# pghysels/STRUMPACK

Measured on AMD Instinct MI355X. Metric: hss_compress_ulv_factor_solve_gflops, higher is better.
Workload: dtype f64

## Files before the change

include/hssk.h:

```cpp
#ifndef HSSK_H
#define HSSK_H

#ifdef __cplusplus
extern "C" {
#endif

typedef struct hssk_ctx hssk_ctx;

int hssk_ctx_create(hssk_ctx** ctx, int device);
void hssk_ctx_destroy(hssk_ctx* ctx);
void* hssk_ctx_stream(hssk_ctx* ctx);
int hssk_sync(hssk_ctx* ctx);
const char* hssk_last_error(void);
typedef struct hssk_plan hssk_plan;
int hssk_plan_begin(hssk_ctx* ctx, hssk_plan** plan);
int hssk_plan_end(hssk_ctx* ctx);
int hssk_plan_replay(hssk_ctx* ctx, hssk_plan* plan);
void hssk_plan_destroy(hssk_plan* plan);
int hssk_plan_size(const hssk_plan* plan);

void* hssk_malloc(long long bytes);
void hssk_free(void* dptr);
long long hssk_device_total_bytes(void);
int hssk_memcpy_h2d(hssk_ctx* ctx, void* dst, const void* src, long long bytes);
int hssk_memcpy_d2h(hssk_ctx* ctx, void* dst, const void* src, long long bytes);
int hssk_upload_async(hssk_ctx* ctx, void* dst, const void* src, long long bytes);
int hssk_memcpy_d2d(hssk_ctx* ctx, void* dst, const void* src, long long bytes);
int hssk_memcpy2d_h2d(hssk_ctx* ctx, void* dst, long long dpitch, const void* src, long long spitch,
                      long long width, long long height);
int hssk_memcpy2d_d2h(hssk_ctx* ctx, void* dst, long long dpitch, const void* src, long long spitch,
                      long long width, long long height);
int hssk_memset_zero(hssk_ctx* ctx, void* dst, long long bytes);
int hssk_h2d_block_async(hssk_ctx* ctx, double* dst, long long ldd, const double* src, long long lds, long long rows,
                         long long cols);
int hssk_h2d_bytes_async(hssk_ctx* ctx, void* dst, long long dpitch, const void* src, long long spitch, long long width,
                         long long cols);
int hssk_copy_fence(hssk_ctx* ctx);
int hssk_compute_fence(hssk_ctx* ctx);
int hssk_compute_mark(hssk_ctx* ctx, int slot);
int hssk_copy_wait(hssk_ctx* ctx, int slot);
int hssk_is_device_pointer(const void* ptr);
typedef struct hssk_aca_desc {
  const double* A;
  int lda, m, n;
  double rtol, atol;
  int max_rank, row0;
  double* U;
  int ldu;
  double* V;
  int ldv;
  int* rank;
} hssk_aca_desc;
int hssk_aca_vbatched(hssk_ctx* ctx, const hssk_aca_desc* descs, int count);
int hssk_side_begin(hssk_ctx* ctx);
int hssk_side_end(hssk_ctx* ctx);
int hssk_side_join(hssk_ctx* ctx);
int hssk_stream_wait(hssk_ctx* waiter, hssk_ctx* on);
int hssk_watch_start(hssk_ctx* ctx, int id);
int hssk_watch_stop(hssk_ctx* ctx, int id);
double hssk_watch_read_ms(hssk_ctx* ctx, int id, int* pairs);
float hssk_last_dgemm_ms(hssk_ctx* ctx);
double hssk_last_dgemm_flops(hssk_ctx* ctx);
int hssk_dgemm_timing_defer(hssk_ctx* ctx);
int hssk_dgemm_timing_collect(hssk_ctx* ctx, double* ms, double* flops, int* launches);
long long hssk_last_dgemm_trace(hssk_ctx* ctx, long long* out, long long max_wgs);
double hssk_last_dgemm_clock_ghz(hssk_ctx* ctx);

int hssk_fill_toeplitz(hssk_ctx* ctx, double* A, int n, long long lda, char kind);
int hssk_fill_toeplitz_block(hssk_ctx* ctx, double* A, int rows, int cols, long long lda, int i0, int j0, char kind);
int hssk_randn(hssk_ctx* ctx, double* P, int rows, long long cols, long long ld, int row0,
               long long stride, unsigned long long seed);

int hssk_dgemm(hssk_ctx* ctx, int transB, int m, long long n, long long k, double alpha,
               const double* A, long long lda, const double* B, long long ldb, double beta,
               double* C, long long ldc);

int hssk_sgemm_sketch(hssk_ctx* ctx, int transB, int m, long long n, long long k, double alpha,
                      const double* A, long long lda,
                      const float* B, long long ldb,
                      double beta, double* C, long long ldc);
int hssk_narrow_f32(hssk_ctx* ctx, float* dst, long long ldd, const double* src, long long lds, long long rows, long long cols);

#define HSSK_GEN_TOEPLITZ 1
#define HSSK_GEN_TOEPLITZ_UPPER 2
typedef struct hssk_gen {
  int kind, reserved;
  double p[4];
} hssk_gen;
int hssk_sketch_gen(hssk_ctx* ctx, const hssk_gen* g, int transG, int m, long long n, long long k, long long j0, double alpha,
                    const double* A, long long lda, double beta, double* C, long long ldc);
int hssk_gen_fill(hssk_ctx* ctx, const hssk_gen* g, double* A, long long rows, long long cols, long long lda, long long i0,
                  long long j0, int trans);

typedef struct hssk_gemm_desc {
  const double* A;
  const double* B;
  double* C;
  int m, n, k;
  int lda, ldb, ldc;
  int transA, transB;
  double alpha, beta;
} hssk_gemm_desc;
int hssk_gemm_vbatched(hssk_ctx* ctx, const hssk_gemm_desc* descs, int count);

typedef struct hssk_leaf_update_desc {
  const double* R;
  const double* D;
  double* Sr;
  double* Sc;
  int d, m, ldr, ldd, lds;
} hssk_leaf_update_desc;
int hssk_leaf_update_vbatched(hssk_ctx* ctx, const hssk_leaf_update_desc* descs, int count);

typedef struct hssk_kernel_spec {
  const double* X;
  long long n;
  int d, type, p;
  double h, lambda;
} hssk_kernel_spec;
typedef struct hssk_keval_desc {
  const int* ri;
  const int* ci;
  double* out;
  int nr, nc, ldo, r0, c0;
} hssk_keval_desc;
int hssk_kernel_eval_vbatched(hssk_ctx* ctx, const hssk_kernel_spec* spec, const hssk_keval_desc* descs, int count);
int hssk_knn(hssk_ctx* ctx, const double* X, int d, int n, int k, int q0, int q1, int* out_idx);
typedef struct hssk_colset_desc {
  const int* src0;
  const int* src1;
  int n0, n1, lo, hi;
  int* out;
  int* count;
  const int* n0_dev;
  const int* n1_dev;
} hssk_colset_desc;
int hssk_colsets(hssk_ctx* ctx, const hssk_colset_desc* descs, int count, int universe);
long long hssk_colsets_max_universe(void);
int hssk_cluster_median(hssk_ctx* ctx, double* X, int d, int n, int algo, int cluster_size, int* perm, int* status);
int hssk_kernel_predict(hssk_ctx* ctx, const hssk_kernel_spec* spec, const double* w, const double* T, int m, double* pred);
#define HSSK_KPREDICT_TAU 1.220703125e-4
int hssk_kernel_predict_f32(hssk_ctx* ctx, const float* X, long long n, int d, int type, int p, double h,
                            const float* w, const float* T, int m, float* pred, long long* stats);
int hssk_kernel_predict_splits(long long n, int m);

typedef struct hssk_colgather_desc {
  const double* src;
  double* dst;
  const int* idx;
  int rows, ncols, lds, ldd;
  int scatter;
} hssk_colgather_desc;
int hssk_gather_cols(hssk_ctx* ctx, const hssk_colgather_desc* descs, int count);
enum { HSSK_DT_F64 = 0, HSSK_DT_F32 = 1, HSSK_DT_C32 = 2, HSSK_DT_C64 = 3 };
int hssk_expand_image(hssk_ctx* ctx, double* dst, long long ldd, const void* src, long long lds, long long rows, long long cols,
                      int dtype);
typedef struct hssk_rowgather_desc {
  const double* src;
  double* dst;
  const int* idx;
  int nrows, cols, lds, ldd;
  int scatter, accumulate;
} hssk_rowgather_desc;
int hssk_gather_rows(hssk_ctx* ctx, const hssk_rowgather_desc* descs, int count);
typedef struct hssk_elem_desc {
  const double* A;
  long long lda;
  const int* I;
  const int* J;
  int i0, j0;
  double* B;
  int m, n, ldb, transpose;
  int rlo, rhi, clo, chi;
} hssk_elem_desc;
int hssk_gather_elems(hssk_ctx* ctx, const hssk_elem_desc* descs, int count);
int hssk_gather_elems_f32(hssk_ctx* ctx, const hssk_elem_desc* descs, int count);
int hssk_gen_elems(hssk_ctx* ctx, const hssk_gen* g, const hssk_elem_desc* descs, int count);
int hssk_sum_slabs(hssk_ctx* ctx, const double* slabs, long long count, long long stride, int nslab, double* out);
typedef struct hssk_transpose_desc {
  const double* src;
  double* dst;
  int rows, cols, lds, ldd;
} hssk_transpose_desc;
int hssk_transpose(hssk_ctx* ctx, const hssk_transpose_desc* descs, int count);

typedef struct hssk_triu_desc {
  const double* src;
  double* dst;
  int rows, cols, lds, ldd;
  int dstride;
} hssk_triu_desc;
int hssk_copy_triu(hssk_ctx* ctx, const hssk_triu_desc* descs, int count);

int hssk_sjlt_dense(hssk_ctx* ctx, double* Rt, int dn, long long K, long long ld, const int* pat, int nnz);
int hssk_sjlt_sketch(hssk_ctx* ctx, int transA, long long n_out, long long K, const double* A, long long lda,
// ... 298 lines not shown
```

include/structured/StructuredMatrix.h:

```cpp
#ifndef STRUCTURED_MATRIX_H
#define STRUCTURED_MATRIX_H

typedef enum {
  SP_TYPE_HSS = 0,
  SP_TYPE_BLR,
  SP_TYPE_HODLR,
  SP_TYPE_HODBF,
  SP_TYPE_BUTTERFLY,
  SP_TYPE_LR,
  SP_TYPE_LOSSY,
  SP_TYPE_LOSSLESS
} SP_STRUCTURED_TYPE;

typedef struct CSPOptions {
  SP_STRUCTURED_TYPE type;
  double rel_tol;
  double abs_tol;
  int leaf_size;
  int max_rank;
  int verbose;
} CSPOptions;

typedef void* CSPStructMat;

// ... 47 lines not shown
void SPX_d_struct_default_hss_options(SPXHSSOptions* h);
int SPX_d_struct_from_dense_hss(CSPStructMat* S, int rows, int cols, const double* A, int ldA,
                                const CSPOptions* opts, const SPXHSSOptions* h);
int SPX_d_struct_from_dense_device(CSPStructMat* S, int rows, int cols, const double* dA, long long ldA,
                                   const CSPOptions* opts, const SPXHSSOptions* h);
int SPX_s_struct_from_dense_device(CSPStructMat* S, int rows, int cols, const float* dA, long long ldA,
                                   const CSPOptions* opts, const SPXHSSOptions* h, int sketch_precision);
int SPX_s_struct_sketch_route(const CSPStructMat S);
int SPX_s_struct_stats(const CSPStructMat S, double* out);
typedef void (*SPXAllGatherFn)(void* user, void* dbuf, long long bytes_per_rank);
int SPX_d_struct_from_dense_device_sharded(CSPStructMat* S, int rows, int cols, const double* dA, long long ldA,
                                           const CSPOptions* opts, const SPXHSSOptions* h, int world, int rank,
                                           SPXAllGatherFn allgather, void* user);
typedef void* SPXComm;
int SPX_comm_unique_id(char id[128]);
int SPX_comm_create(SPXComm* comm, int world, int rank, const char id[128]);
void SPX_comm_destroy(SPXComm* comm);
int SPX_comm_selftest(SPXComm comm);
int SPX_comm_size(const SPXComm comm);
int SPX_comm_rank(const SPXComm comm);
int SPX_struct_shard_range(int n, const CSPOptions* opts, int world, int rank, int* lo, int* hi);
int SPX_d_struct_from_dense_device_comm(CSPStructMat* S, int rows, int cols, const double* dA, long long ldA,
                                        const CSPOptions* opts, const SPXHSSOptions* h, SPXComm comm);
int SPX_d_struct_from_generator(CSPStructMat* S, int n, int kind, const CSPOptions* opts, const SPXHSSOptions* h);
int SPX_d_struct_from_generator_comm(CSPStructMat* S, int n, int kind, const CSPOptions* opts, const SPXHSSOptions* h, SPXComm comm);
int SPX_d_struct_from_generator_sharded(CSPStructMat* S, int n, int kind, const CSPOptions* opts, const SPXHSSOptions* h,
                                        int world, int rank, SPXAllGatherFn allgather, void* user);
int SPX_d_struct_from_blocks_device(CSPStructMat* S, int rows, int cols, const double* dArows, long long ldr,
                                    const double* dAcols, long long ldc, const CSPOptions* opts, const SPXHSSOptions* h,
                                    SPXComm comm);
int SPX_d_struct_from_blocks_device_cb(CSPStructMat* S, int rows, int cols, const double* dArows, long long ldr,
                                       const double* dAcols, long long ldc, const CSPOptions* opts, const SPXHSSOptions* h,
                                       int world, int rank, SPXAllGatherFn allgather, void* user);
int SPX_d_struct_from_kernel(CSPStructMat* S, int n, int d, double* points, int ktype, double h, double lambda, int p,
                             const CSPOptions* opts, int clustering, int neighbors, int* perm);
int SPX_d_struct_from_kernel_sharded(CSPStructMat* S, int n, int d, double* points, int ktype, double h, double lambda, int p,
                                     const CSPOptions* opts, int clustering, int neighbors, int* perm, int world, int rank,
                                     SPXAllGatherFn allgather, void* user);
int SPX_d_struct_from_kernel_comm(CSPStructMat* S, int n, int d, double* points, int ktype, double h, double lambda, int p,
                                  const CSPOptions* opts, int clustering, int neighbors, int* perm, SPXComm comm);
int SPX_d_struct_mult_device(const CSPStructMat S, char trans, int m, const double* dB, long long ldB,
                             double* dC, long long ldC);
int SPX_d_struct_solve_device(const CSPStructMat S, int nrhs, double* dB, long long ldB);
int SPX_d_struct_levels(const CSPStructMat S);
int SPX_d_struct_is_compressed(const CSPStructMat S);
int SPX_d_struct_num_nodes(const CSPStructMat S);
int SPX_d_struct_node_info(const CSPStructMat S, int* out);
int SPX_d_struct_stats(const CSPStructMat S, double* out);
int SPX_d_struct_partial_factor(CSPStructMat S);
int SPX_d_struct_schur_dims(const CSPStructMat S, int* dims);
int SPX_d_struct_schur_update(CSPStructMat S, double* Theta, int ldT, double* DUB01, int ldD, double* Phi, int ldP,
                              double* Vhat, int ldV);
int SPX_d_struct_schur_product_direct(const CSPStructMat S, int c, const double* R, long long ldR, double* Sr,
                                      long long ldSr, double* Sc, long long ldSc, int on_device);
int SPX_d_struct_schur_product_indirect(const CSPStructMat S, int c, const double* R0, long long ldR0, const double* R1,
                                        long long ldR1, const double* Sr1, long long ldSr1, const double* Sc1,
                                        long long ldSc1, double* Sr, long long ldSr, double* Sc, long long ldSc,
                                        int on_device);
int SPX_d_struct_mult_child(const CSPStructMat S, int child, char trans, int m, const double* B, long long ldB, double* C,
                            long long ldC, int on_device);
int SPX_d_struct_extract_blocks(const CSPStructMat S, int nb, const int* rows, const int* roff, const int* cols, const int* coff,
                                double* const* out, const int* ldo, int add, int on_device);
int SPX_d_struct_write(const CSPStructMat S, const char* path);
typedef void* SPXBLRFront;
int SPX_d_blr_front_factor(SPXBLRFront* F, int dsep, int dupd, const double* F11, int ld11, const double* F12, int ld12,
                           const double* F21, int ld21, double* F22, int ld22, int ntiles1, const int* tiles1, int ntiles2,
                           const int* tiles2, const char* admissible, const CSPOptions* opts);
int SPX_d_blr_front_factor_device(SPXBLRFront* F, int dsep, int dupd, const double* dF11, long long ld11, const double* dF12,
                                  long long ld12, const double* dF21, long long ld21, const double* dF22, long long ld22,
                                  int ntiles1, const int* tiles1, int ntiles2, const int* tiles2, const char* admissible,
                                  const CSPOptions* opts);
void SPX_d_blr_front_time_phases(int on);
int SPX_blr_low_rank_algorithm(int algo);
int SPX_d_blr_front_forward(const SPXBLRFront F, int nrhs, double* bsep, int ldb, double* bupd, int ldu);
int SPX_d_blr_front_backward(const SPXBLRFront F, int nrhs, double* ysep, int ldy, const double* yupd, int ldu);
int SPX_d_blr_front_schur(const SPXBLRFront F, double* F22, int ld22);
const double* SPX_d_blr_front_schur_device(const SPXBLRFront F, long long* ld);
int SPX_d_blr_front_tile_ranks(const SPXBLRFront F, int* out);
int SPX_d_blr_front_stats(const SPXBLRFront F, double* out);
void SPX_d_blr_front_destroy(SPXBLRFront* F);
void* SPX_d_struct_hssk_ctx(const CSPStructMat S);
long long SPX_tree_pass_launches(void);
long long SPX_tree_pass_fallbacks(void);
long long SPX_device_pool_cached_bytes(void);
long long SPX_device_pool_limit_bytes(void);
void SPX_device_pool_trim(void);
void SPX_device_pool_set_limit_gb(double gb);

#ifdef __cplusplus
}
#endif
#endif
```

strumpack_amd/capi.py:

```python
import ctypes as C

import numpy as np

SP_TYPE_HSS, SP_TYPE_BLR = 0, 1


class CSPOptions(C.Structure):
    _fields_ = [("type", C.c_int), ("rel_tol", C.c_double), ("abs_tol", C.c_double),
                ("leaf_size", C.c_int), ("max_rank", C.c_int), ("verbose", C.c_int)]


class SPXHSSOptions(C.Structure):
    _fields_ = [("d0", C.c_int), ("dd", C.c_int), ("p", C.c_int), ("compression_algorithm", C.c_int),
                ("random_engine", C.c_int), ("random_distribution", C.c_int),
                ("compression_sketch", C.c_int), ("sjlt_algo", C.c_int), ("nnz0", C.c_int), ("nnz", C.c_int),
                ("factor_ahead", C.c_int), ("symmetric_operand", C.c_int)]


SP_SYMBOLS = [
    "SP_d_struct_default_options", "SP_d_struct_destroy", "SP_d_struct_rows", "SP_d_struct_cols",
    "SP_d_struct_memory", "SP_d_struct_nonzeros", "SP_d_struct_rank", "SP_d_struct_from_dense",
    "SP_d_struct_from_elements", "SP_d_struct_mult", "SP_d_struct_factor", "SP_d_struct_solve",
    "SP_d_struct_shift",
    "SPX_d_struct_default_hss_options", "SPX_d_struct_from_dense_hss",
    "SPX_d_struct_from_dense_device", "SPX_d_struct_from_dense_device_sharded", "SPX_d_struct_mult_device", "SPX_d_struct_solve_device",
    "SPX_d_struct_levels", "SPX_d_struct_is_compressed", "SPX_d_struct_num_nodes",
    "SPX_d_struct_node_info", "SPX_d_struct_stats", "SPX_d_struct_hssk_ctx",
    "SPX_d_struct_from_kernel", "SPX_d_struct_from_kernel_sharded",
    "SPX_d_struct_from_dense_and_factor", "SPX_comm_unique_id", "SPX_comm_create", "SPX_comm_destroy", "SPX_comm_size", "SPX_comm_rank", "SPX_comm_selftest", "SPX_struct_shard_range",
    "SPX_d_struct_from_dense_device_comm", "SPX_d_struct_from_blocks_device", "SPX_d_struct_from_blocks_device_cb",
    "SPX_d_struct_from_kernel_comm",
    "SPX_d_struct_from_generator", "SPX_d_struct_from_generator_comm", "SPX_d_struct_from_generator_sharded",
    "SPX_d_struct_extract_blocks", "SPX_d_struct_write",
    "SPX_d_blr_front_factor", "SPX_d_blr_front_factor_device", "SPX_d_blr_front_time_phases", "SPX_blr_low_rank_algorithm", "SPX_d_blr_front_forward",
    "SPX_d_blr_front_backward", "SPX_d_blr_front_schur", "SPX_d_blr_front_schur_device", "SPX_d_blr_front_tile_ranks",
    "SPX_d_blr_front_stats", "SPX_d_blr_front_destroy",
    "SPX_tree_pass_launches", "SPX_tree_pass_fallbacks",
    "SPX_device_pool_cached_bytes", "SPX_device_pool_limit_bytes", "SPX_device_pool_trim", "SPX_device_pool_set_limit_gb",
    "SPX_s_struct_from_dense_device", "SPX_s_struct_sketch_route", "SPX_s_struct_stats",
]
ELEM_CB = C.CFUNCTYPE(C.c_double, C.c_int, C.c_int)
ALLGATHER_CB = C.CFUNCTYPE(None, C.c_void_p, C.c_void_p, C.c_longlong)
STAT_NAMES = ["t_compress", "t_sketch", "t_random", "t_tree", "t_factor", "t_solve", "t_mult",
              "sketch_kernel_ms", "sketch_launches", "rounds", "d_final", "f_sketch", "f_local",
              "f_reduce", "f_id", "f_ortho", "f_ulv", "f_solve", "factor_memory", "sketch_kernel_flops", "sketch_kernel_bytes",
              "b_solve", "b_mult", "t_comm"]


def load(path):
    L = C.CDLL(path)
    vp, dp = C.c_void_p, C.c_void_p
    L.SP_d_struct_default_options.argtypes = [C.POINTER(CSPOptions)]
    L.SP_d_struct_destroy.argtypes = [C.POINTER(vp)]
    for f in ("SP_d_struct_rows", "SP_d_struct_cols", "SP_d_struct_rank", "SPX_d_struct_levels",
              "SPX_d_struct_is_compressed", "SPX_d_struct_num_nodes", "SP_d_struct_factor"):
        getattr(L, f).argtypes = [vp]
        getattr(L, f).restype = C.c_int
    for f in ("SP_d_struct_memory", "SP_d_struct_nonzeros"):
        getattr(L, f).argtypes = [vp]
        getattr(L, f).restype = C.c_longlong
    L.SP_d_struct_from_dense.argtypes = [C.POINTER(vp), C.c_int, C.c_int, dp, C.c_int, C.POINTER(CSPOptions)]
    L.SP_d_struct_from_elements.argtypes = [C.POINTER(vp), C.c_int, C.c_int, ELEM_CB, C.POINTER(CSPOptions)]
    L.SP_d_struct_mult.argtypes = [vp, C.c_char, C.c_int, dp, C.c_int, dp, C.c_int]
    L.SP_d_struct_solve.argtypes = [vp, C.c_int, dp, C.c_int]
    L.SP_d_struct_shift.argtypes = [vp, C.c_double]
    L.SPX_d_struct_default_hss_options.argtypes = [C.POINTER(SPXHSSOptions)]
    L.SPX_d_struct_from_dense_hss.argtypes = [C.POINTER(vp), C.c_int, C.c_int, dp, C.c_int,
                                              C.POINTER(CSPOptions), C.POINTER(SPXHSSOptions)]
    L.SPX_d_struct_from_dense_device.argtypes = [C.POINTER(vp), C.c_int, C.c_int, dp, C.c_longlong,
                                                 C.POINTER(CSPOptions), C.POINTER(SPXHSSOptions)]
    L.SPX_d_struct_from_dense_device_sharded.argtypes = [C.POINTER(vp), C.c_int, C.c_int, dp, C.c_longlong,
                                                         C.POINTER(CSPOptions), C.POINTER(SPXHSSOptions),
                                                         C.c_int, C.c_int, ALLGATHER_CB, vp]
    L.SPX_d_struct_from_kernel.argtypes = [C.POINTER(vp), C.c_int, C.c_int, dp, C.c_int, C.c_double, C.c_double, C.c_int,
                                           C.POINTER(CSPOptions), C.c_int, C.c_int, vp]
    L.SPX_d_struct_from_kernel_sharded.argtypes = [C.POINTER(vp), C.c_int, C.c_int, dp, C.c_int, C.c_double, C.c_double, C.c_int,
                                                   C.POINTER(CSPOptions), C.c_int, C.c_int, vp, C.c_int, C.c_int, ALLGATHER_CB, vp]
    L.SPX_d_struct_from_dense_and_factor.argtypes = [C.POINTER(vp), C.c_int, C.c_int, dp, C.c_int, C.POINTER(CSPOptions)]
    L.SPX_comm_unique_id.argtypes = [C.c_char_p]
    L.SPX_comm_create.argtypes = [C.POINTER(vp), C.c_int, C.c_int, C.c_char_p]
    L.SPX_comm_destroy.argtypes = [C.POINTER(vp)]
    L.SPX_comm_destroy.restype = None
    L.SPX_comm_selftest.argtypes = [vp]
    L.SPX_comm_size.argtypes = [vp]
    L.SPX_comm_rank.argtypes = [vp]
    L.SPX_struct_shard_range.argtypes = [C.c_int, C.POINTER(CSPOptions), C.c_int, C.c_int, C.POINTER(C.c_int), C.POINTER(C.c_int)]
    L.SPX_d_struct_from_dense_device_comm.argtypes = [C.POINTER(vp), C.c_int, C.c_int, dp, C.c_longlong,
                                                      C.POINTER(CSPOptions), C.POINTER(SPXHSSOptions), vp]
    L.SPX_d_struct_from_blocks_device.argtypes = [C.POINTER(vp), C.c_int, C.c_int, dp, C.c_longlong, dp, C.c_longlong,
                                                  C.POINTER(CSPOptions), C.POINTER(SPXHSSOptions), vp]
    L.SPX_d_struct_from_blocks_device_cb.argtypes = [C.POINTER(vp), C.c_int, C.c_int, dp, C.c_longlong, dp, C.c_longlong,
                                                     C.POINTER(CSPOptions), C.POINTER(SPXHSSOptions), C.c_int, C.c_int,
                                                     ALLGATHER_CB, vp]
    L.SPX_d_struct_from_kernel_comm.argtypes = [C.POINTER(vp), C.c_int, C.c_int, dp, C.c_int, C.c_double, C.c_double, C.c_int,
                                                C.POINTER(CSPOptions), C.c_int, C.c_int, vp, vp]
    L.SPX_d_struct_from_generator.argtypes = [C.POINTER(vp), C.c_int, C.c_int, C.POINTER(CSPOptions), C.POINTER(SPXHSSOptions)]
    L.SPX_d_struct_from_generator_comm.argtypes = [C.POINTER(vp), C.c_int, C.c_int, C.POINTER(CSPOptions), C.POINTER(SPXHSSOptions), vp]
    L.SPX_d_struct_from_generator_sharded.argtypes = [C.POINTER(vp), C.c_int, C.c_int, C.POINTER(CSPOptions), C.POINTER(SPXHSSOptions),
                                                      C.c_int, C.c_int, ALLGATHER_CB, vp]
    L.SPX_d_struct_mult_device.argtypes = [vp, C.c_char, C.c_int, dp, C.c_longlong, dp, C.c_longlong]
    L.SPX_d_struct_solve_device.argtypes = [vp, C.c_int, dp, C.c_longlong]
    L.SPX_d_struct_node_info.argtypes = [vp, C.POINTER(C.c_int)]
    L.SPX_d_struct_stats.argtypes = [vp, C.POINTER(C.c_double)]
    ll = C.c_longlong
    L.SPX_d_struct_partial_factor.argtypes = [vp]
    L.SPX_d_struct_schur_dims.argtypes = [vp, C.POINTER(C.c_int)]
    L.SPX_d_struct_schur_update.argtypes = [vp, dp, C.c_int, dp, C.c_int, dp, C.c_int, dp, C.c_int]
    L.SPX_d_struct_schur_product_direct.argtypes = [vp, C.c_int, dp, ll, dp, ll, dp, ll, C.c_int]
    L.SPX_d_struct_schur_product_indirect.argtypes = [vp, C.c_int, dp, ll, dp, ll, dp, ll, dp, ll, dp, ll, dp, ll, C.c_int]
    L.SPX_d_struct_mult_child.argtypes = [vp, C.c_int, C.c_char, C.c_int, dp, ll, dp, ll, C.c_int]
    L.SPX_d_struct_hssk_ctx.argtypes = [vp]
    L.SPX_d_struct_hssk_ctx.restype = vp
    for f in ("SPX_tree_pass_launches", "SPX_tree_pass_fallbacks", "SPX_device_pool_cached_bytes", "SPX_device_pool_limit_bytes"):
        getattr(L, f).argtypes = []
        getattr(L, f).restype = C.c_longlong
    L.SPX_device_pool_trim.argtypes = []
    L.SPX_device_pool_trim.restype = None
    L.SPX_device_pool_set_limit_gb.argtypes = [C.c_double]
    L.SPX_device_pool_set_limit_gb.restype = None
    ip = C.POINTER(C.c_int)
    L.SPX_d_struct_extract_blocks.argtypes = [vp, C.c_int, ip, ip, ip, ip, C.POINTER(C.c_void_p), ip, C.c_int, C.c_int]
    L.SPX_d_struct_write.argtypes = [vp, C.c_char_p]
    L.SPX_d_blr_front_factor.argtypes = [C.POINTER(vp), C.c_int, C.c_int, dp, C.c_int, dp, C.c_int, dp, C.c_int, dp, C.c_int,
                                         C.c_int, ip, C.c_int, ip, C.c_char_p, C.POINTER(CSPOptions)]
    L.SPX_d_blr_front_factor_device.argtypes = [C.POINTER(vp), C.c_int, C.c_int, dp, ll, dp, ll, dp, ll, dp, ll,
                                                C.c_int, ip, C.c_int, ip, C.c_char_p, C.POINTER(CSPOptions)]
    L.SPX_d_blr_front_time_phases.argtypes = [C.c_int]
    L.SPX_d_blr_front_time_phases.restype = None
    L.SPX_blr_low_rank_algorithm.argtypes = [C.c_int]
    L.SPX_blr_low_rank_algorithm.restype = C.c_int
    L.SPX_d_blr_front_forward.argtypes = [vp, C.c_int, dp, C.c_int, dp, C.c_int]
    L.SPX_d_blr_front_backward.argtypes = [vp, C.c_int, dp, C.c_int, dp, C.c_int]
    L.SPX_d_blr_front_schur.argtypes = [vp, dp, C.c_int]
    L.SPX_d_blr_front_schur_device.argtypes = [vp, C.POINTER(ll)]
    L.SPX_d_blr_front_schur_device.restype = vp
    L.SPX_d_blr_front_tile_ranks.argtypes = [vp, ip]
    L.SPX_d_blr_front_stats.argtypes = [vp, C.POINTER(C.c_double)]
    L.SPX_d_blr_front_destroy.argtypes = [C.POINTER(vp)]
    L.SPX_d_blr_front_destroy.restype = None
    L.SP_s_struct_default_options.argtypes = [C.POINTER(CSPOptions)]
    L.SP_s_struct_default_options.restype = None
    L.SP_s_struct_destroy.argtypes = [C.POINTER(vp)]
    L.SP_s_struct_destroy.restype = None
    for f in ("SP_s_struct_rows", "SP_s_struct_cols", "SP_s_struct_rank", "SP_s_struct_factor", "SPX_s_struct_sketch_route"):
        getattr(L, f).argtypes = [vp]
        getattr(L, f).restype = C.c_int
    for f in ("SP_s_struct_memory", "SP_s_struct_nonzeros"):
        getattr(L, f).argtypes = [vp]
        getattr(L, f).restype = C.c_longlong
    L.SP_s_struct_from_dense.argtypes = [C.POINTER(vp), C.c_int, C.c_int, dp, C.c_int, C.POINTER(CSPOptions)]
    L.SP_s_struct_mult.argtypes = [vp, C.c_char, C.c_int, dp, C.c_int, dp, C.c_int]
    L.SP_s_struct_solve.argtypes = [vp, C.c_int, dp, C.c_int]
    L.SP_s_struct_shift.argtypes = [vp, C.c_float]
    L.SPX_s_struct_from_dense_device.argtypes = [C.POINTER(vp), C.c_int, C.c_int, dp, C.c_longlong,
                                                 C.POINTER(CSPOptions), C.POINTER(SPXHSSOptions), C.c_int]
    L.SPX_s_struct_stats.argtypes = [vp, C.POINTER(C.c_double)]
    return L


class BLRFront:
    STAT_NAMES = ["t_factor", "ms_lu", "ms_compress", "ms_trsm", "ms_schur", "f_schur", "f_total", "nnz11", "nnz12", "nnz21",
                  "max_rank", "schur_launches", "b_schur", "_r13", "_r14", "_r15"]

    def __init__(self, lib, handle, dsep, dupd, nt1, nt2):
        self.L, self.h, self.dsep, self.dupd, self.nt1, self.nt2 = lib, handle, dsep, dupd, nt1, nt2

    @staticmethod
    def _tiles(t):
        a = np.ascontiguousarray(t, dtype=np.int32)
        return a, a.ctypes.data_as(C.POINTER(C.c_int))

    @staticmethod
    def _adm(adm, nt1):
        if adm is None:
            return None
        a = np.asfortranarray(np.asarray(adm).astype(np.int8).reshape(nt1, nt1))
        return a.tobytes(order="F")

    @classmethod
    def factor(cls, lib, F11, F12, F21, F22, tiles1, tiles2, opts, admissible=None):
        ds, du = F11.shape[0], (F12.shape[1] if F12 is not None else 0)
        f = lambda a: None if a is None else np.asfortranarray(a, dtype=np.float64)
        F11, F12, F21 = f(F11), f(F12), f(F21)
        S = np.array(F22, dtype=np.float64, order="F") if F22 is not None else np.zeros((du, du), order="F")
        t1, p1 = cls._tiles(tiles1)
        t2, p2 = cls._tiles(tiles2)
        ptr = lambda a: a.ctypes.data if a is not None and a.size else None
        h = C.c_void_p()
        if lib.SPX_d_blr_front_factor(C.byref(h), ds, du, ptr(F11), max(ds, 1), ptr(F12), max(ds, 1), ptr(F21), max(du, 1),
                                      ptr(S), max(du, 1), len(t1), p1, len(t2), p2, cls._adm(admissible, len(t1)), C.byref(opts)):
            raise RuntimeError("SPX_d_blr_front_factor failed")
        return cls(lib, h, ds, du, len(t1), len(t2)), S

    @classmethod
    def factor_device(cls, lib, dsep, dupd, dF11, ld11, dF12, ld12, dF21, ld21, dF22, ld22, tiles1, tiles2, opts, admissible=None):
        t1, p1 = cls._tiles(tiles1)
# ... 372 lines not shown
```

strumpack_amd/csrc/host/StructuredMatrixC.cpp:

```cpp
#include "DevicePool.hpp"
#include <complex>
#include <cstdlib>
#include <iostream>

#include "BLRMatrix.hpp"
#include "HSSMatrix.hpp"
#include "HSSMatrixPromoted.hpp"
#include "Comm.hpp"
#include "Kernel.hpp"
#include "StructuredMatrix.hpp"
#include "structured/StructuredMatrix.h"

using namespace strumpack;
using namespace strumpack::structured;

namespace {
struct CStructMat {
  std::unique_ptr<StructuredMatrix<double>> S;
};
inline StructuredMatrix<double>* mat(const CSPStructMat S) { return static_cast<CStructMat*>(S)->S.get(); }
inline HSS::HSSMatrix<double>* hss(const CSPStructMat S) { return dynamic_cast<HSS::HSSMatrix<double>*>(mat(S)); }

template <typename T> struct CStructMatT {
  std::unique_ptr<StructuredMatrix<T>> S;
// ... 553 lines not shown
  f->time_phases = g_blr_time_phases;
  return f;
}
inline BLR::DeviceBLR* front(const SPXBLRFront F) {
  if (!F) throw std::invalid_argument("BLR front: null handle");
  return static_cast<BLR::DeviceBLR*>(F);
}
}
}
void SPX_d_blr_front_time_phases(int on) { g_blr_time_phases = on != 0; }
int SPX_blr_low_rank_algorithm(int algo) {
  if (algo != 0 && algo != 1) return 1;
  g_blr_low_rank_algorithm = algo;
  return 0;
}
int SPX_d_blr_front_factor(SPXBLRFront* F, int dsep, int dupd, const double* F11, int ld11, const double* F12, int ld12,
                           const double* F21, int ld21, double* F22, int ld22, int ntiles1, const int* tiles1, int ntiles2,
                           const int* tiles2, const char* admissible, const CSPOptions* opts) {
  SP_TRY
  auto f = make_front(dsep, dupd, ntiles1, tiles1, ntiles2, tiles2, opts);
  f->partial_factor_host(ntiles1, F11, ld11, F12, ld12, F21, ld21, F22, ld22, admissible);
  if (F22 && dupd > 0) f->schur_host(F22, ld22);
  *F = f.release();
  SP_CATCH
}
int SPX_d_blr_front_factor_device(SPXBLRFront* F, int dsep, int dupd, const double* dF11, long long ld11, const double* dF12,
                                  long long ld12, const double* dF21, long long ld21, const double* dF22, long long ld22,
                                  int ntiles1, const int* tiles1, int ntiles2, const int* tiles2, const char* admissible,
                                  const CSPOptions* opts) {
  SP_TRY
  auto f = make_front(dsep, dupd, ntiles1, tiles1, ntiles2, tiles2, opts);
  f->partial_factor_device(ntiles1, dF11, ld11, dF12, ld12, dF21, ld21, dF22, ld22, admissible);
  *F = f.release();
  SP_CATCH
}
int SPX_d_blr_front_forward(const SPXBLRFront F, int nrhs, double* bsep, int ldb, double* bupd, int ldu) {
  SP_TRY
  front(F)->front_forward(nrhs, bsep, ldb, bupd, ldu);
  SP_CATCH
}
int SPX_d_blr_front_backward(const SPXBLRFront F, int nrhs, double* ysep, int ldy, const double* yupd, int ldu) {
  SP_TRY
  front(F)->front_backward(nrhs, ysep, ldy, yupd, ldu);
  SP_CATCH
}
int SPX_d_blr_front_schur(const SPXBLRFront F, double* F22, int ld22) {
  SP_TRY
  front(F)->schur_host(F22, ld22);
  SP_CATCH
}
const double* SPX_d_blr_front_schur_device(const SPXBLRFront F, long long* ld) {
  if (!F) return nullptr;
  auto* f = static_cast<BLR::DeviceBLR*>(F);
  if (ld) *ld = f->schur_ld();
  return f->upd_rows() > 0 ? f->schur_device() : nullptr;
}
int SPX_d_blr_front_tile_ranks(const SPXBLRFront F, int* out) {
  SP_TRY
  front(F)->tile_ranks(out);
  SP_CATCH
}
int SPX_d_blr_front_stats(const SPXBLRFront F, double* out) {
  SP_TRY
  auto* f = front(F);
  long long nz[3];
  f->front_nonzeros(nz);
  out[0] = f->t_factor;
  for (int p = 0; p < 4; p++) out[1 + p] = f->phase_ms[p];
  out[5] = f->f_schur; out[6] = f->f_total;
  out[7] = (double)nz[0]; out[8] = (double)nz[1]; out[9] = (double)nz[2];
  out[10] = f->rank(); out[11] = f->schur_launches; out[12] = f->b_schur;
  SP_CATCH
}
void SPX_d_blr_front_destroy(SPXBLRFront* F) {
  if (!F) return;
  delete static_cast<BLR::DeviceBLR*>(*F);
  *F = nullptr;
}

void* SPX_d_struct_hssk_ctx(const CSPStructMat S) { return hss(S) ? (void*)hss(S)->engine()->ctx() : nullptr; }

long long SPX_tree_pass_launches(void) { return strumpack::HSS::tree_pass_launches(); }
long long SPX_tree_pass_fallbacks(void) { return strumpack::HSS::tree_pass_fallbacks(); }

long long SPX_device_pool_cached_bytes(void) { return (long long)strumpack::DevicePool::get().cached(); }
long long SPX_device_pool_limit_bytes(void) { return (long long)strumpack::DevicePool::get().limit(); }
void SPX_device_pool_trim(void) { strumpack::DevicePool::get().trim(); }
void SPX_device_pool_set_limit_gb(double gb) {
  strumpack::DevicePool::get().set_limit(gb <= 0 ? 0 : (size_t)(gb * 1073741824.0));
}

}
```

strumpack_amd/csrc/host/hss_compress.cpp:

```cpp
#include "hss_engine_internal.hpp"
#include <cstdio>

namespace strumpack {
namespace HSS {

void DeviceHSS::drop_plans() {
  for (auto& kv : plans_) if (kv.second.plan) hssk_plan_destroy(kv.second.plan);
  plans_.clear();
  if (plan_arena_) plan_arena_->reset();
}
bool DeviceHSS::plans_enabled() const {
  static const bool off = [] { const char* e = std::getenv("STRUMPACK_AMD_NO_PLANS"); return e && e[0] == '1'; }();
  return !off;
}

void DeviceHSS::reset_compression() {
  book_ = PendingBook();
  defer_book_ = false;
  drop_plans();
  for (auto& nd : nodes_) {
    int lo = nd.lo, m = nd.m, lvl = nd.lvl, h = nd.height, c0 = nd.c0, c1 = nd.c1, p = nd.parent;
    nd = Node();
    nd.lo = lo; nd.m = m; nd.lvl = lvl; nd.height = h; nd.c0 = c0; nd.c1 = c1; nd.parent = p;
  }
  factor_cancel();
  persist_->reset();
  dev_tree_ = nullptr;
  work_->reset();
  fact_->reset();
  invalidate_factors();
  d_ranks_ = persist_->ints(2 * nodes_.size() + 2);
}

void DeviceHSS::restart_nodes(int d_have) {
  ck(hssk_sync(ctx_));
  factor_cancel();
  for (auto& nd : nodes_) {
    int lo = nd.lo, m = nd.m, lvl = nd.lvl, h = nd.height, c0 = nd.c0, c1 = nd.c1, p = nd.parent;
    nd = Node();
    nd.lo = lo; nd.m = m; nd.lvl = lvl; nd.height = h; nd.c0 = c0; nd.c1 = c1; nd.parent = p;
  }
  persist_->reset();
  dev_tree_ = nullptr;
  invalidate_factors();
  d_ranks_ = persist_->ints(2 * nodes_.size() + 2);
  if (d_have > 0) {
    std::vector<hssk_colgather_desc> cp;
    const int ncols = (int)std::min<long long>(n_, 0x7fffffff);
    cp.push_back(hssk_colgather_desc{Srt0_, Srt_, nullptr, d_have, ncols, dcap_, dcap_, 0});
    cp.push_back(hssk_colgather_desc{Sct0_, Sct_, nullptr, d_have, ncols, dcap_, dcap_, 0});
    ck(hssk_gather_cols(ctx_, cp.data(), 2));
  }
}

void DeviceHSS::free_compress_workspace() {
  ck(hssk_sync(ctx_));
  work_->reset();
  Rt_ = Srt_ = Sct_ = Srt0_ = Sct0_ = nullptr;
  sj_pat_ = nullptr;
  for (auto& nd : nodes_) { nd.Srt = nd.Sct = nd.Rrt = nd.Rct = nd.RrtRed = nd.RctRed = nd.Qr = nd.Qc = nullptr; nd.panels = false; }
}

void DeviceHSS::compress(Source& src) {
  OpGuard op_guard(op_mu_);
  double t0 = now();
  stats_ = PhaseStats();
  int dcap = o_.algorithm != 1 ? o_.d0 + o_.p : o_.d0 + o_.dd;
  dcap = std::max(16, (dcap + 15) / 16 * 16);
  for (;;) {
    if (compress_attempt(src, dcap)) break;
    dcap *= 2;
    if (o_.verbose) std::cout << "# HSS compression: growing the sample capacity to " << dcap << std::endl;
  }
  static const bool trace_host = [] { const char* e = std::getenv("STRUMPACK_AMD_TRACE_HOST"); return e && e[0] == '1'; }();
  const double th0 = now();
  if (dist_subtree_) exchange_node_table();
  free_compress_workspace();
  comm_arena_->reset();
  const double th1 = now();
  {
    const double ms = hssk_watch_read_ms(ctx_, 5, nullptr);
    if (ms > 0.) stats_.t_sketch = ms * 1e-3;
    double kms = 0., kfl = 0.;
    int kn = 0;
    ck(hssk_dgemm_timing_collect(ctx_, &kms, &kfl, &kn));
    stats_.sketch_kernel_ms += kms; stats_.sketch_kernel_flops += kfl; stats_.sketch_launches += kn;
  }
  stats_.t_compress = now() - t0;
  stats_.t_tree = stats_.t_compress - stats_.t_sketch - stats_.t_random;
  stats_.t_mark = now();
  if (trace_host) std::fprintf(stderr, "# host: compress end: free workspace %.1f us, timers %.1f us\n", (th1 - th0) * 1e6, (now() - th1) * 1e6);
}

void DeviceHSS::fill_random(int r0, int dn) {
  if (o_.user_random) { sj_pat_ = nullptr; return; }
  double t0 = now();
  const long long N = n_;
  sj_pat_ = nullptr;
  if (o_.sketch == 1) {
    if (r0 == 0 || !rng_) rng_.reset(new HostRng());
    auto& e = rng_->sj;
    const int nnz = std::max(1, std::min(r0 == 0 ? o_.nnz0 : o_.nnz, dn));
    const bool dense_pat = nnz > 8;
    const int nq = dense_pat ? nnz : (nnz <= 4 ? 4 : 8);
    std::vector<int> pat((size_t)nq * N, dn);
    std::uniform_int_distribution<int> sign(0, 1);
    if (o_.sjlt_algo == 0) {
      const int chunk = dn / nnz;
      std::uniform_int_distribution<int> shift(0, chunk - 1);
      for (long long k = 0; k < N; k++)
        for (int q = 0; q < nnz; q++) {
          const int c = shift(e) + chunk * q;
          pat[(size_t)k * nq + q] = sign(e) == 0 ? c : (c | (int)0x80000000);
        }
    } else {
      std::vector<int> cols(dn);
      for (int j = 0; j < dn; j++) cols[j] = j;
      for (long long k = 0; k < N; k++)
        for (int q = 0; q < nnz; q++) {
          std::uniform_int_distribution<int> pick(q, dn - 1);
          std::swap(cols[q], cols[pick(e)]);
          pat[(size_t)k * nq + q] = sign(e) == 0 ? cols[q] : (cols[q] | (int)0x80000000);
        }
    }
    if (dense_pat) {
      std::vector<double> buf((size_t)dn * N, 0.);
      host_parallel_for((size_t)N, [&](size_t k) {
        for (int q = 0; q < nnz; q++) {
          const int p = pat[k * nq + q];
          buf[(size_t)(p & 0x7fffffff) + k * dn] = p < 0 ? -1. : 1.;
        }
      });
      ck(hssk_memcpy2d_h2d(ctx_, Rt_ + r0, sizeof(double) * dcap_, buf.data(), sizeof(double) * dn, sizeof(double) * dn, N));
      ck(hssk_sync(ctx_));
      stats_.t_random += now() - t0;
      return;
    }
    int* dp = work_->ints((size_t)nq * N);
    ck(hssk_memcpy_h2d(ctx_, dp, pat.data(), (long long)sizeof(int) * nq * N));
    ck(hssk_sjlt_dense(ctx_, Rt_ + r0, dn, N, dcap_, dp, nnz));
    sj_pat_ = dp;
    sj_nnz_ = nnz;
  } else if (o_.random_engine == 2) {
    if (o_.random_dist != 0) throw std::invalid_argument("philox engine implements the normal distribution only");
    ck(hssk_randn(ctx_, Rt_ + r0, dn, N, dcap_, r0, N, 0x5354524dull));
  } else {
    if (r0 == 0 || !rng_) rng_.reset(new HostRng());
    if (o_.random_engine == 0 && o_.random_dist == 0 && N > 0 && dn > 0) {
      std::vector<double> blk((size_t)dn * N);
      rng_->linnorm.fill(blk.data(), blk.size(), [](std::size_t n, const std::function<void(std::size_t)>& fn) { host_parallel_for(n, fn); });
      double* dT = tmp_->dbl((size_t)dn * N);
      ck(hssk_memcpy_h2d(ctx_, dT, blk.data(), (long long)(sizeof(double) * blk.size())));
      hssk_transpose_desc t{dT, Rt_ + r0, (int)N, dn, (int)N, dcap_};
      ck(hssk_transpose(ctx_, &t, 1));
    } else {
      std::minstd_rand* lin = &rng_->lin;
      std::mt19937* mer = &rng_->mer;
      auto& nd = rng_->nd;
      auto& ud = rng_->ud;
      std::vector<double> buf((size_t)dn * N);
      for (int s = 0; s < dn; s++)
        for (long long c = 0; c < N; c++) {
          double v;
          if (o_.random_engine == 0) v = o_.random_dist == 0 ? nd(*lin) : ud(*lin);
          else v = o_.random_dist == 0 ? nd(*mer) : ud(*mer);
          buf[s + (size_t)c * dn] = v;
        }
      ck(hssk_memcpy2d_h2d(ctx_, Rt_ + r0, sizeof(double) * dcap_, buf.data(), sizeof(double) * dn, sizeof(double) * dn, N));
    }
  }
  ck(hssk_sync(ctx_));
  stats_.t_random += now() - t0;
}

bool DeviceHSS::compress_attempt(Source& src, int dcap) {
  reset_compression();
  attempt_++;
  dcap_ = dcap;
  const size_t N = n_;
  cols_per_rank_ = o_.world > 1 ? ((long long)N + o_.world - 1) / o_.world : (long long)N;
  const size_t Npad = o_.world > 1 ? (size_t)cols_per_rank_ * o_.world : N;
  Rt_ = work_->dbl((size_t)dcap * N);
  Srt_ = work_->dbl((size_t)dcap * Npad);
  Sct_ = work_->dbl((size_t)dcap * Npad);
  if (o_.algorithm == 2) { Srt0_ = work_->dbl((size_t)dcap * Npad); Sct0_ = work_->dbl((size_t)dcap * Npad); }
  stats_.rounds = 0;
  stats_.f_sketch = stats_.f_local = stats_.f_reduce = stats_.f_id = stats_.f_ortho = 0;
  const bool original = (o_.algorithm != 1);
  if (!original) {
    int d = o_.d0, dd = o_.dd;
    while (!is_compressed()) {
      int c = (d == o_.d0) ? 0 : d;
      int dnew = (d == o_.d0) ? d + dd : dd;
      if (c + dnew > dcap) return false;
      fill_random(c, dnew);
      if (stats_.rounds == 0 && src.extract_before_sample()) {
        std::vector<int> leaves;
        for (auto& ids : own_by_height_) for (int id : ids) if (nodes_[id].leaf() && nodes_[id].lvl != 0) leaves.push_back(id);
        extract_blocks(src, leaves);
      }
      ck(hssk_watch_start(ctx_, 5));
      src.sample(*this, c, dnew);
      ck(hssk_watch_stop(ctx_, 5));
      stats_.f_sketch += src.sketch_flops(*this, dnew);
      if (o_.verbose) std::cout << "# compressing with d+dd = " << d << "+" << dd << " (stable)" << std::endl;
      stats_.rounds++;
      for (size_t h = 0; h < own_by_height_.size(); h++) {
        if (h == 1 && tree_pass(src, d, dd)) {
          for (size_t hh = 1; hh < own_by_height_.size(); hh++) factor_ahead_level(hh);
          break;
        }
        process_level(src, own_by_height_[h], d, dd, false);
        factor_ahead_level(h);
      }
      if (dist_subtree_) {
        exchange_cut_compress(d + dd);
        for (auto& ids : top_by_height_) process_level(src, ids, d, dd, false);
      }
      stats_.d_final = d + dd;
      if (!is_compressed()) {
        d += dd;
        dd = std::min(dd, o_.max_rank - d);
        if (dd <= 0) break;
      }
    }
  } else {
    int d_old = 0, d = o_.d0 + o_.p;
    while (!is_compressed()) {
      if (d > dcap) return false;
      fill_random(d_old, d - d_old);
      ck(hssk_watch_start(ctx_, 5));
      src.sample(*this, d_old, d - d_old);
      ck(hssk_watch_stop(ctx_, 5));
      stats_.f_sketch += src.sketch_flops(*this, d - d_old);
      if (o_.verbose) std::cout << "# compressing with d = " << d - o_.p << " + " << o_.p << (o_.algorithm == 2 ? " (original, hard restart)" : " (original)") << std::endl;
      if (o_.algorithm == 2) {
        if (dist_subtree_ || o_.world > 1) throw std::invalid_argument("hard restart is a single-GPU option");
        std::vector<hssk_colgather_desc> cp;
        cp.push_back(hssk_colgather_desc{Srt_ + d_old, Srt0_ + d_old, nullptr, d - d_old, (int)N, dcap_, dcap_, 0});
        cp.push_back(hssk_colgather_desc{Sct_ + d_old, Sct0_ + d_old, nullptr, d - d_old, (int)N, dcap_, dcap_, 0});
        ck(hssk_gather_cols(ctx_, cp.data(), 2));
      }
      stats_.rounds++;
      for (auto& ids : own_by_height_) process_level(src, ids, d, d - d_old, true);
      if (dist_subtree_) {
        exchange_cut_compress(d);
        for (auto& ids : top_by_height_) process_level(src, ids, d, d - d_old, true);
      }
      stats_.d_final = d;
      if (!is_compressed()) {
        d_old = d;
        d = 2 * (d_old - o_.p) + o_.p;
        if (d_old >= 4 * n_ + o_.p + 64) break;
        if (o_.algorithm == 2 && d <= dcap) restart_nodes(d_old);
      }
    }
  }
  return true;
}

void DeviceHSS::process_level(Source& src, const std::vector<int>& ids_all, int d, int dd, bool original) {
  const int dtot = original ? d : d + dd;
  const int dnew0 = original ? d - dd : d;
  std::vector<int> ids;
  for (int id : ids_all) {
    Node& nd = nodes_[id];
    if (!nd.leaf() && !(nodes_[nd.c0].compressed() && nodes_[nd.c1].compressed())) continue;
    if (nd.lvl == 0 && nd.compressed()) continue;
    ids.push_back(id);
  }
  if (ids.empty()) return;
  std::vector<int> fresh;
  std::vector<char> was_untouched(nodes_.size(), 0), was_compressed(nodes_.size(), 0);
  for (int id : ids) {
    Node& nd = nodes_[id];
    was_untouched[id] = nd.untouched();
    was_compressed[id] = nd.compressed();
    if (nd.untouched()) fresh.push_back(id);
  }
  extract_blocks(src, fresh);
  std::vector<int> work_ids, r0s, dns;
  for (int id : ids) {
    Node& nd = nodes_[id];
    if (nd.lvl == 0) { nd.Ustate = nd.Vstate = 2; continue; }
    if (!nd.panels) {
      if (nd.leaf()) {
        nd.mU = nd.mV = nd.m;
        nd.Srt = Srt_ + (size_t)nd.lo * dcap_;
        nd.Sct = Sct_ + (size_t)nd.lo * dcap_;
        nd.Rrt = nd.Rct = Rt_ + (size_t)nd.lo * dcap_;
      } else {
        nd.mU = nodes_[nd.c0].rU + nodes_[nd.c1].rU;
        nd.mV = nodes_[nd.c0].rV + nodes_[nd.c1].rV;
        nd.Srt = work_->dbl((size_t)dcap_ * std::max(nd.mU, 1));
        nd.Sct = work_->dbl((size_t)dcap_ * std::max(nd.mV, 1));
        nd.Rrt = work_->dbl((size_t)dcap_ * std::max(nd.mV, 1));
        nd.Rct = work_->dbl((size_t)dcap_ * std::max(nd.mU, 1));
      }
      nd.panels = true;
    }
    work_ids.push_back(id);
    r0s.push_back(was_untouched[id] ? 0 : dnew0);
    dns.push_back(was_untouched[id] ? dtot : dtot - dnew0);
  }
  if (work_ids.empty()) return;
  local_samples(work_ids, r0s, dns);

  std::vector<int> id_nodes, id_which, ot_nodes, ot_which;
  for (int id : work_ids) {
    Node& nd = nodes_[id];
    if (was_compressed[id]) continue;
    for (int w = 0; w < 2; w++) {
      int st = w == 0 ? nd.Ustate : nd.Vstate;
      if (st == 2) continue;
      int rows = w == 0 ? nd.mU : nd.mV;
      if (original || dtot >= o_.max_rank || dtot >= rows) { id_nodes.push_back(id); id_which.push_back(w); }
      else { ot_nodes.push_back(id); ot_which.push_back(w); }
    }
  }
  if (!ot_nodes.empty()) {
    std::vector<char> resolved;
    ortho_test(ot_nodes, ot_which, d, dd, resolved);
    for (size_t i = 0; i < ot_nodes.size(); i++) {
      if (resolved[i]) { id_nodes.push_back(ot_nodes[i]); id_which.push_back(ot_which[i]); }
      else {
        Node& nd = nodes_[ot_nodes[i]];
        (ot_which[i] == 0 ? nd.Ustate : nd.Vstate) = 1;
      }
    }
  }
  defer_book_ = !original;
  run_id(id_nodes, id_which, dtot);
  defer_book_ = false;
  if (original) {
    for (int id : work_ids) {
      Node& nd = nodes_[id];
      if (was_compressed[id]) continue;
      bool ok = (dtot - o_.p >= o_.max_rank) || (nd.rU < dtot - o_.p && nd.rV < dtot - o_.p);
      if (!ok) { nd.Ustate = nd.Vstate = 1; nd.rU = nd.rV = 0; nd.Ir.clear(); nd.Ic.clear(); }
    }
  }
  std::vector<int> rd_ids, rd_r0, rd_dn;
  for (int id : work_ids) {
    Node& nd = nodes_[id];
    if (!nd.compressed()) continue;
    if (!was_compressed[id]) {
      nd.RrtRed = work_->dbl((size_t)dcap_ * std::max(nd.rV, 1));
      nd.RctRed = work_->dbl((size_t)dcap_ * std::max(nd.rU, 1));
      rd_ids.push_back(id); rd_r0.push_back(0); rd_dn.push_back(dtot);
    } else {
      rd_ids.push_back(id); rd_r0.push_back(dnew0); rd_dn.push_back(dtot - dnew0);
    }
  }
  reduce_samples(rd_ids, rd_r0, rd_dn);
  finish_id_bookkeeping();
}

void DeviceHSS::extract_blocks(Source& src, const std::vector<int>& ids) {
  std::vector<ElemReq> reqs;
  for (int id : ids) {
    Node& nd = nodes_[id];
    if (nd.leaf()) {
      if (nd.D) continue;
      nd.D = persist_->dbl((size_t)nd.m * nd.m);
      reqs.push_back(ElemReq{nullptr, nullptr, nullptr, nullptr, nd.lo, nd.lo, nd.m, nd.m, nd.D, nd.m});
    } else {
      Node &a = nodes_[nd.c0], &b = nodes_[nd.c1];
      nd.B01 = persist_->dbl((size_t)std::max(a.rU, 1) * std::max(b.rV, 1));
      nd.B10 = persist_->dbl((size_t)std::max(b.rU, 1) * std::max(a.rV, 1));
      reqs.push_back(ElemReq{a.dIr, b.dIc, &a.Ir, &b.Ic, 0, 0, a.rU, b.rV, nd.B01, std::max(a.rU, 1)});
      reqs.push_back(ElemReq{b.dIr, a.dIc, &b.Ir, &a.Ic, 0, 0, b.rU, a.rV, nd.B10, std::max(b.rU, 1)});
    }
  }
  if (!reqs.empty()) src.extract(*this, reqs);
}

void DeviceHSS::local_samples(const std::vector<int>& ids, const std::vector<int>& r0s, const std::vector<int>& dns) {
  std::vector<hssk_combine_desc> cb;
  std::vector<hssk_gemm_desc> mm;
  std::vector<hssk_leaf_update_desc> lu;
  for (size_t k = 0; k < ids.size(); k++) {
    Node& nd = nodes_[ids[k]];
    const int r0 = r0s[k], dn = dns[k];
    if (dn <= 0) continue;
    if (nd.leaf()) {
      const int m = nd.m;
      if (dn <= 192 && dn % 2 == 0 && r0 % 2 == 0 && nd.Rrt == nd.Rct)
        lu.push_back(hssk_leaf_update_desc{nd.Rrt + r0, nd.D, nd.Srt + r0, nd.Sct + r0, dn, m, dcap_, m, dcap_});
      else {
        mm.push_back(hssk_gemm_desc{nd.Rrt + r0, nd.D, nd.Srt + r0, dn, m, m, dcap_, m, dcap_, 0, 1, -1.0, 1.0});
        mm.push_back(hssk_gemm_desc{nd.Rct + r0, nd.D, nd.Sct + r0, dn, m, m, dcap_, m, dcap_, 0, 0, -1.0, 1.0});
      }
      stats_.f_local += 4.0 * m * (double)m * dn;
    } else {
      Node &a = nodes_[nd.c0], &b = nodes_[nd.c1];
      const int none = 0x7fffffff;
      const int l01 = std::max(a.rU, 1), l10 = std::max(b.rU, 1);
      cb.push_back(hssk_combine_desc{a.Srt + r0, nullptr, dcap_, none, a.permU, b.RrtRed + r0, nullptr, dcap_, none, nullptr,
                                     nd.B01, 1, l01, -1.0, nd.Srt + r0, dcap_, dn, a.rU, b.rV});
      cb.push_back(hssk_combine_desc{b.Srt + r0, nullptr, dcap_, none, b.permU, a.RrtRed + r0, nullptr, dcap_, none, nullptr,
                                     nd.B10, 1, l10, -1.0, nd.Srt + r0 + (size_t)a.rU * dcap_, dcap_, dn, b.rU, a.rV});
      cb.push_back(hssk_combine_desc{a.Sct + r0, nullptr, dcap_, none, a.permV, b.RctRed + r0, nullptr, dcap_, none, nullptr,
                                     nd.B10, l10, 1, -1.0, nd.Sct + r0, dcap_, dn, a.rV, b.rU});
      cb.push_back(hssk_combine_desc{b.Sct + r0, nullptr, dcap_, none, b.permV, a.RctRed + r0, nullptr, dcap_, none, nullptr,
                                     nd.B01, l01, 1, -1.0, nd.Sct + r0 + (size_t)a.rV * dcap_, dcap_, dn, b.rV, a.rU});
      stats_.f_local += 4.0 * ((double)a.rU * b.rV + (double)b.rU * a.rV) * dn;
    }
  }
  if (!cb.empty()) ck(hssk_gather_combine(ctx_, cb.data(), (int)cb.size()));
  if (!lu.empty()) {
    int rc = hssk_leaf_update_vbatched(ctx_, lu.data(), (int)lu.size());
    if (rc == 2) {
      for (auto& u : lu) {
        mm.push_back(hssk_gemm_desc{u.R, u.D, u.Sr, u.d, u.m, u.m, u.ldr, u.ldd, u.lds, 0, 1, -1.0, 1.0});
        mm.push_back(hssk_gemm_desc{u.R, u.D, u.Sc, u.d, u.m, u.m, u.ldr, u.ldd, u.lds, 0, 0, -1.0, 1.0});
      }
    } else ck(rc);
  }
  if (!mm.empty()) ck(hssk_gemm_vbatched(ctx_, mm.data(), (int)mm.size()));
}

void DeviceHSS::reduce_samples(const std::vector<int>& ids, const std::vector<int>& r0s, const std::vector<int>& dns) {
  if (ids.empty()) return;
  std::vector<hssk_combine_desc> cb;
  const int none = 0x7fffffff;
  for (size_t k = 0; k < ids.size(); k++) {
    Node& nd = nodes_[ids[k]];
    const int r0 = r0s[k], dn = dns[k];
    if (dn <= 0) continue;
    const double *rr0, *rr1 = nullptr, *rc0, *rc1 = nullptr;
    int sr = none, sc = none;
    if (nd.leaf()) { rr0 = nd.Rrt + r0; rc0 = nd.Rct + r0; }
    else {
      Node &a = nodes_[nd.c0], &b = nodes_[nd.c1];
      rr0 = a.RrtRed + r0; rr1 = b.RrtRed + r0; sr = a.rV;
      rc0 = a.RctRed + r0; rc1 = b.RctRed + r0; sc = a.rU;
    }
    {
      const int m = nd.mV, r = nd.rV, K = (m > r && r > 0) ? m - r : 0;
      if (r > 0)
        cb.push_back(hssk_combine_desc{rr0, rr1, dcap_, sr, nd.permV, rr0, rr1, dcap_, sr, nd.permV + r, nd.XV, 1, r, 1.0,
                                       nd.RrtRed + r0, dcap_, dn, r, K});
      stats_.f_reduce += 2.0 * r * (double)K * dn;
    }
    {
      const int m = nd.mU, r = nd.rU, K = (m > r && r > 0) ? m - r : 0;
      if (r > 0)
        cb.push_back(hssk_combine_desc{rc0, rc1, dcap_, sc, nd.permU, rc0, rc1, dcap_, sc, nd.permU + r, nd.XU, 1, r, 1.0,
                                       nd.RctRed + r0, dcap_, dn, r, K});
      stats_.f_reduce += 2.0 * r * (double)K * dn;
    }
  }
  if (!cb.empty()) ck(hssk_gather_combine(ctx_, cb.data(), (int)cb.size()));
}

void DeviceHSS::run_id(const std::vector<int>& ids, const std::vector<int>& which, int dtot) {
  if (ids.empty()) return;
  Arena& tmp = *tmp_;
  tmp.rewind();
  const size_t cnt = ids.size();
  std::vector<double*> Ws(cnt, nullptr);
  std::vector<const double*> srcs(cnt, nullptr);
  std::vector<int> ds(cnt, dtot);
  for (size_t k = 0; k < cnt; k++) {
    Node& nd = nodes_[ids[k]];
    const int m = which[k] == 0 ? nd.mU : nd.mV;
    const double* S = which[k] == 0 ? nd.Srt : nd.Sct;
    if (m == 0) continue;
    Ws[k] = tmp.dbl((size_t)dtot * m);
    srcs[k] = S;
  }
  id_panels(ids, which, Ws, ds, &srcs, dcap_);
}

static bool tsqr_staircase() {
  const char* e = std::getenv("STRUMPACK_AMD_TSQR_DENSE");
  return !(e && std::atoi(e));
}

void DeviceHSS::tsqr_reduce(const std::vector<int>& ids, const std::vector<int>& which, std::vector<double*>& Ws,
                            std::vector<int>& ds) {
  Arena& tmp = *tmp_;
  const size_t cnt = ids.size();
  struct Piece { double* p; int ld, rows; };
  std::vector<std::vector<Piece>> pieces(cnt);
  std::vector<int> ms(cnt, 0);
  bool any = false;
  std::vector<hssk_qr_desc> qr;
  for (size_t k = 0; k < cnt; k++) {
    const Node& nd = nodes_[ids[k]];
    const int m = which[k] == 0 ? nd.mU : nd.mV, d = ds[k];
    ms[k] = m;
    if (m <= 0 || !Ws[k] || d <= std::max(256, 2 * m)) continue;
// ... 393 lines not shown
```

strumpack_amd/csrc/host/hss_engine.hpp:

```cpp
#pragma once
#include <functional>
#include <iosfwd>
#include <map>
#include <tuple>
#include <memory>
#include <mutex>
#include <string>
#include <vector>

#include "ClusterTree.hpp"
#include "hssk.h"

namespace strumpack {
namespace HSS {

struct EngineOptions {
  double rel_tol = 1e-2, abs_tol = 1e-8;
  int leaf_size = 512, max_rank = 50000, d0 = 128, dd = 64, p = 10;
  int algorithm = 1;
  int random_engine = 0;
  int random_dist = 0;
  int sketch = 0, sjlt_algo = 0, nnz0 = 4, nnz = 4;
  bool user_random = false;
  bool factor_ahead = false;
  int symmetric = 0;
  bool verbose = false;
  int device = 0;
  int world = 1, rank = 0;
  void (*allgather)(void* user, void* dbuf, long long bytes_per_rank) = nullptr;
  void* comm_user = nullptr;
  void (*allgather_stream)(void* user, void* dbuf, long long bytes_per_rank, void* stream) = nullptr;
  void (*allreduce_stream)(void* user, double* buf, long long count, void* stream) = nullptr;
  void (*reduce_scatter_stream)(void* user, const double* send, const long long* offs, const long long* counts, double* recv,
                                void* stream) = nullptr;
};

struct CommSpec {
  int world = 1, rank = 0;
  void (*allgather)(void*, void*, long long) = nullptr;
  void* user = nullptr;
  bool native = false;
  void apply(EngineOptions& e) const;
};

using host_mult_t = std::function<void(char trans, int n, int nrhs, const double* R, int ldr, double* S, int lds)>;
using host_sample_t = std::function<void(int n, int nrhs, double* R, double* Sr, double* Sc)>;
using host_elem_t = std::function<void(int m, const int* I, int n, const int* J, double* B, int ldb)>;
class DeviceHSS;
long long tree_pass_launches();
long long tree_pass_fallbacks();

struct PhaseStats {
  double t_compress = 0, t_sketch = 0, t_random = 0, t_tree = 0, t_factor = 0, t_solve = 0, t_mult = 0;
  double t_comm = 0;
  double sketch_kernel_ms = 0;
  double sketch_kernel_flops = 0;
  double sketch_kernel_bytes = 0;
  int sketch_launches = 0, rounds = 0, d_final = 0;
  double t_mark = 0;
  double f_sketch = 0, f_local = 0, f_reduce = 0, f_id = 0, f_ortho = 0, f_ulv = 0, f_solve = 0;
  double b_solve = 0, b_mult = 0;
};

class Arena;
struct HostRng;

class Arena;
struct SolveWork {
  std::shared_ptr<Arena> arena;
  std::vector<double*> f, y, zc, xb;
  double* db = nullptr;
  int nrhs = 0, sr = -1;
  bool valid = false, partial = false;
  double* xroot = nullptr;
  double* reduced = nullptr;
  long long ldx = 0, ldr = 0;
};

class DeviceHSS {
 public:
  DeviceHSS(int n, const EngineOptions& opts, const structured::ClusterTree* tree = nullptr);
  ~DeviceHSS();
  DeviceHSS(const DeviceHSS&) = delete;
  DeviceHSS& operator=(const DeviceHSS&) = delete;

  void compress_dense_device(const double* dA, long long lda);
  void compress_dense_device_f32(const float* dA, long long lda, int precision);
  int sketch_route() const { return f32_route_; }
  void compress_dense_host(const double* A, long long lda);
  void compress_dense_host_typed(const void* A, long long lda, int dtype);
  using host_fill_t = std::function<void(long long c0, long long c1, double* dst)>;
  void compress_host_blocks(const host_fill_t& fill, const host_elem_t& elem);
  void compress_dense_device_sharded(const double* dRows, long long ldr, const double* dCols, long long ldc);
  void compress_generator(const hssk_gen& g);
  bool shard_range(int rank, int& lo, int& hi) const;
  void compress_callbacks(const host_mult_t& mult, const host_elem_t& elem);
  void compress_callbacks_user_random(const host_sample_t& sample, const host_elem_t& elem);
  struct KernelSpec {
    const double* X = nullptr;
    const double* dX = nullptr;
    int d = 0, type = 0, p = 1, ann = 64;
    double h = 1., lambda = 0.;
    std::function<void(int k, int* ann)> neighbors;
    std::function<double(int i, int j)> eval;
  };
  void compress_kernel(const KernelSpec& ks, const int* user_ann = nullptr, int user_k = 0);

  void save(std::ostream& os) const;
  static std::unique_ptr<DeviceHSS> load(std::istream& is, const EngineOptions& opts);

  void mult(char trans, int nrhs, const double* x, long long ldx, double* y, long long ldy,
            bool on_device, double beta = 0.0);
  void factor();
  void solve(int nrhs, double* b, long long ldb, bool on_device);
  void shift(double sigma);
  void reset() { OpGuard g(op_mu_); reset_compression(); }
  void shift_cplx(double re, double im);

  struct SchurDims { int n0 = 0, n1 = 0, rV0 = 0, rU0 = 0, rV1 = 0, rU1 = 0, mu0 = 0; };
  void partial_factor();
  void factor_node(int node) { factor_sub(node, false); }
  void solve_node(int node, int nrhs, double* b, long long ldb, bool on_device) { solve_sub(node, nrhs, b, ldb, on_device); }
  bool node_is_factored(int node) const { return node == 0 ? factored_ : sub_factored_ == node; }
  void forward_solve_node(int node, struct SolveWork& w, int nrhs, const double* b, long long ldb, bool partial, double* xroot,
                          long long ldx, double* reduced, long long ldr);
  void backward_solve_node(int node, struct SolveWork& w, const double* xroot, long long ldx, double* x, long long ldxo);
  bool is_partially_factored() const { return partial_factored_; }
  SchurDims schur_dims() const;
  void schur_update(double* Theta, long long ldt, double* DUB01, long long ldd, double* Phi, long long ldp,
                    double* Vhat, long long ldv);
  void schur_product_direct(int c, const double* R, long long ldr, double* Sr, long long ldsr, double* Sc,
                            long long ldsc, bool on_device);
  void schur_product_indirect(int c, const double* R0, long long ldr0, const double* R1, long long ldr1,
// ... 181 lines not shown
```

strumpack_amd/csrc/host/hss_engine_internal.hpp:

```cpp
#pragma once
#include "hss_engine.hpp"
#include "Comm.hpp"
#include "LinearNormal.hpp"
#include "DevicePool.hpp"

#include <unistd.h>
#include <atomic>
#include <functional>
#include <condition_variable>
#include <thread>
#include <exception>
#include <algorithm>
#include <chrono>
#include <cmath>
#include <cstring>
#include <iostream>
#include <istream>
#include <ostream>
#include <map>
#include <mutex>
#include <random>
#include <stdexcept>

namespace strumpack {
namespace HSS {

inline void ck(int rc) {
  if (rc) throw std::runtime_error(std::string("hssk: ") + hssk_last_error());
}
inline double now() {
  return std::chrono::duration<double>(std::chrono::steady_clock::now().time_since_epoch()).count();
}
inline int hybrid_nrhs() {
  static const int v = [] { const char* e = std::getenv("STRUMPACK_AMD_HYBRID_NRHS"); return e ? std::atoi(e) : 12; }();
  return v;
}

inline int fuse_max_nrhs() {
  static const int v = [] { const char* e = std::getenv("STRUMPACK_AMD_FUSE_MAX_NRHS"); return e ? std::atoi(e) : 256; }();
  return v;
}

struct HostRng {
  std::default_random_engine sj{0};
  std::minstd_rand lin{0};
  LinearNormal linnorm{0};
  std::mt19937 mer{0};
  std::normal_distribution<double> nd;
  std::uniform_real_distribution<double> ud;
};

class HostPool {
 public:
  static HostPool& get() { static HostPool p; return p; }
  bool run(const std::function<void()>& body) {
    if (getpid() != pid_) return false;
    static thread_local bool inside = false;
    if (inside) return false;
    std::unique_lock<std::mutex> own(owner_, std::try_to_lock);
    if (!own.owns_lock() || th_.empty()) return false;
    struct Mark { bool& f; Mark(bool& x) : f(x) { f = true; } ~Mark() { f = false; } } mark(inside);
    {
      std::lock_guard<std::mutex> g(mu_);
      body_ = &body; pending_ = th_.size(); gen_++;
    }
    cv_.notify_all();
    body();
    std::unique_lock<std::mutex> lk(mu_);
    done_.wait(lk, [&] { return pending_ == 0; });
    body_ = nullptr;
    return true;
  }
  ~HostPool() {
    if (getpid() != pid_) { for (auto& t : th_) t.detach(); return; }
    { std::lock_guard<std::mutex> g(mu_); stop_ = true; gen_++; }
    cv_.notify_all();
    for (auto& t : th_) t.join();
  }

 private:
  HostPool() : pid_(getpid()) {
    const unsigned n = std::max(1u, std::min(32u, std::thread::hardware_concurrency()));
    for (unsigned t = 1; t < n; t++) th_.emplace_back([this] { loop(); });
  }
  void loop() {
    unsigned long seen = 0;
    for (;;) {
      const std::function<void()>* f;
      {
        std::unique_lock<std::mutex> lk(mu_);
        cv_.wait(lk, [&] { return gen_ != seen; });
        seen = gen_;
        if (stop_) return;
        f = body_;
      }
      (*f)();
      { std::lock_guard<std::mutex> g(mu_); if (--pending_ == 0) done_.notify_all(); }
    }
  }
  const pid_t pid_;
  std::vector<std::thread> th_;
  std::mutex owner_, mu_;
  std::condition_variable cv_, done_;
  const std::function<void()>* body_ = nullptr;
  unsigned long gen_ = 0;
  size_t pending_ = 0;
  bool stop_ = false;
};
template <class F> void host_parallel_for(size_t n, F&& fn) {
  if (n <= 1) { for (size_t i = 0; i < n; i++) fn(i); return; }
  std::atomic<size_t> next{0};
  std::exception_ptr err;
  std::mutex mu;
  const std::function<void()> body = [&] {
    try {
      for (size_t i = next++; i < n; i = next++) fn(i);
    } catch (...) { std::lock_guard<std::mutex> g(mu); err = std::current_exception(); }
  };
  if (!HostPool::get().run(body)) body();
  if (err) std::rethrow_exception(err);
}

// ... 70 lines not shown
```

strumpack_amd/csrc/host/hss_sources.cpp:

```cpp
#include "hss_engine_internal.hpp"

namespace strumpack {
namespace HSS {

double DeviceHSS::Source::sketch_flops(const DeviceHSS& H, int dn) const {
  return 2.0 * products(H) * (double)H.n_ * (double)H.n_ * (H.sj_pat_ ? H.sj_nnz_ : dn);
}

struct DeviceHSS::DenseDeviceSource : DeviceHSS::Source {
  const double* dA;
  long long lda;
  DenseDeviceSource(const double* a, long long l) : dA(a), lda(l) {}
  bool extract_before_sample() const override { return true; }
  bool device_elems(const DeviceHSS&, hssk_elem_src* e) const override { e->A = dA; e->lda = lda; e->use_gen = 0; return true; }
  int done_products_ = 2;
  bool done_sparse_ = false;
  int products(const DeviceHSS&) const override { return done_products_; }
  double sketch_flops(const DeviceHSS& H, int dn) const override {
    return 2.0 * done_products_ * (double)H.n_ * (double)H.n_ * (done_sparse_ ? H.sj_nnz_ : dn);
  }
  void sample(DeviceHSS& H, int r0, int dn) override {
    const long long N = H.n_;
    long long j0 = 0, j1 = N;
    if (H.dist_subtree_) {
      const Node& c = H.nodes_[H.cut_nodes_[H.o_.rank]];
      j0 = c.lo; j1 = c.lo + c.m;
    } else if (H.o_.world > 1) {
      j0 = std::min(N, H.cols_per_rank_ * H.o_.rank); j1 = std::min(N, j0 + H.cols_per_rank_);
    }
    const long long nloc = j1 - j0;
    static const bool sj_dense = std::getenv("STRUMPACK_AMD_SJLT_DENSE") && std::atoi(std::getenv("STRUMPACK_AMD_SJLT_DENSE"));
    done_sparse_ = H.sj_pat_ && dn <= 1024 && !sj_dense;
    done_products_ = (!done_sparse_ && H.o_.symmetric) ? 1 : 2;
    if (nloc > 0 && done_sparse_) {
      for (int t = 0; t < 2; t++) {
        const double* Aop = t == 0 ? dA + j0 : dA + j0 * lda;
        double* St = (t == 0 ? H.Srt_ : H.Sct_) + r0 + j0 * H.dcap_;
        ck(hssk_sjlt_sketch(H.ctx_, t, nloc, N, Aop, lda, H.sj_pat_, H.sj_nnz_, dn, St, H.dcap_));
        ck(hssk_sync(H.ctx_));
        float ms = hssk_last_dgemm_ms(H.ctx_);
        if (ms > 0) {
          H.stats_.sketch_kernel_ms += ms; H.stats_.sketch_launches++;
          H.stats_.sketch_kernel_flops += hssk_last_dgemm_flops(H.ctx_);
          H.stats_.sketch_kernel_bytes += 8.0 * (double)nloc * (double)N;
        }
      }
    } else if (nloc > 0) {
      ck(hssk_dgemm(H.ctx_, 1, dn, nloc, N, 1.0, H.Rt_ + r0, H.dcap_, dA + j0, lda, 0.0, H.Srt_ + r0 + j0 * H.dcap_, H.dcap_));
      ck(hssk_dgemm_timing_defer(H.ctx_));
      if (H.o_.symmetric) {
        hssk_colgather_desc cp{H.Srt_ + r0 + j0 * H.dcap_, H.Sct_ + r0 + j0 * H.dcap_, nullptr, dn, (int)nloc, H.dcap_, H.dcap_, 0};
        ck(hssk_gather_cols(H.ctx_, &cp, 1));
      } else {
        ck(hssk_dgemm(H.ctx_, 0, dn, nloc, N, 1.0, H.Rt_ + r0, H.dcap_, dA + j0 * lda, lda, 0.0, H.Sct_ + r0 + j0 * H.dcap_, H.dcap_));
        ck(hssk_dgemm_timing_defer(H.ctx_));
      }
    }
    if (H.o_.world > 1 && !H.dist_subtree_) {
      const long long bytes = (long long)sizeof(double) * H.dcap_ * H.cols_per_rank_;
      H.comm(H.Srt_, bytes);
      H.comm(H.Sct_, bytes);
    }
  }
  void extract(DeviceHSS& H, const std::vector<ElemReq>& reqs) override {
    std::vector<hssk_elem_desc> d;
    d.reserve(reqs.size());
    for (auto& r : reqs)
      if (r.m > 0 && r.n > 0) d.push_back(hssk_elem_desc{dA, lda, r.dI, r.dJ, r.i0, r.j0, r.dB, r.m, r.n, r.ldb, 0});
    if (!d.empty()) ck(hssk_gather_elems(H.ctx_, d.data(), (int)d.size()));
  }
};

struct DeviceHSS::DenseDeviceSourceF32 : DeviceHSS::Source {
  const float* dA;
  long long lda;
  int route;
  double* dBuf = nullptr;
  long long nb = 0;
  int gen = -1;
  int done_products_ = 2;
  DenseDeviceSourceF32(const float* a, long long l, int r) : dA(a), lda(l), route(r) {}
  bool extract_before_sample() const override { return true; }
  bool device_elems(const DeviceHSS&, hssk_elem_src* e) const override {
    e->A = reinterpret_cast<const double*>(dA); e->lda = lda; e->use_gen = 2;
    return true;
  }
  int products(const DeviceHSS&) const override { return done_products_; }
  double sketch_flops(const DeviceHSS& H, int dn) const override { return 2.0 * done_products_ * (double)H.n_ * (double)H.n_ * dn; }
  void sample(DeviceHSS& H, int r0, int dn) override {
    if (H.o_.world > 1) throw std::invalid_argument("single-precision device operand: single-GPU only (multi-GPU float operands are not supported)");
    if (H.sj_pat_) throw std::invalid_argument("single-precision device operand: the SJLT sketch is not supported; use the Gaussian sketch");
    const long long N = H.n_;
    if (N <= 0 || dn <= 0) return;
    auto timed = [&](double bytes) {
      ck(hssk_dgemm_timing_defer(H.ctx_));
      H.stats_.sketch_kernel_bytes += bytes;
    };
    if (route == 1) {
      done_products_ = H.o_.symmetric ? 1 : 2;
      ck(hssk_sgemm_sketch(H.ctx_, 1, dn, N, N, 1.0, H.Rt_ + r0, H.dcap_, dA, lda, 0.0, H.Srt_ + r0, H.dcap_));
      timed(4.0 * (double)N * (double)N);
      if (H.o_.symmetric) {
        hssk_colgather_desc cp{H.Srt_ + r0, H.Sct_ + r0, nullptr, dn, (int)N, H.dcap_, H.dcap_, 0};
        ck(hssk_gather_cols(H.ctx_, &cp, 1));
      } else {
        ck(hssk_sgemm_sketch(H.ctx_, 0, dn, N, N, 1.0, H.Rt_ + r0, H.dcap_, dA, lda, 0.0, H.Sct_ + r0, H.dcap_));
        timed(4.0 * (double)N * (double)N);
      }
      return;
    }
    done_products_ = 2;
    if (gen != H.attempt_) {
      gen = H.attempt_;
      nb = std::max<long long>(64, (1LL << 30) / (8 * N) / 64 * 64);
      nb = std::min(nb, (N + 63) / 64 * 64);
      dBuf = H.work_->dbl((size_t)N * nb);
    }
    for (long long c0 = 0, b = 0; c0 < N; c0 += nb, b++) {
      const long long c1 = std::min(N, c0 + nb);
      ck(hssk_expand_image(H.ctx_, dBuf, N, dA + c0 * lda, lda, N, c1 - c0, HSSK_DT_F32));
      ck(hssk_dgemm(H.ctx_, 0, dn, c1 - c0, N, 1.0, H.Rt_ + r0, H.dcap_, dBuf, N, 0.0, H.Sct_ + r0 + c0 * H.dcap_, H.dcap_));
      timed(0.);
      ck(hssk_dgemm(H.ctx_, 1, dn, N, c1 - c0, 1.0, H.Rt_ + r0 + c0 * H.dcap_, H.dcap_, dBuf, N, b ? 1.0 : 0.0, H.Srt_ + r0, H.dcap_));
      timed(0.);
    }
  }
  void extract(DeviceHSS& H, const std::vector<ElemReq>& reqs) override {
    std::vector<hssk_elem_desc> d;
    d.reserve(reqs.size());
    for (auto& r : reqs)
      if (r.m > 0 && r.n > 0) d.push_back(hssk_elem_desc{reinterpret_cast<const double*>(dA), lda, r.dI, r.dJ, r.i0, r.j0, r.dB, r.m, r.n, r.ldb, 0});
    if (!d.empty()) ck(hssk_gather_elems_f32(H.ctx_, d.data(), (int)d.size()));
  }
};

struct DeviceHSS::ShardedDenseSource : DeviceHSS::Source {
  const double* dRows;
  long long ldr;
  const double* dCols;
  long long ldc;
  ShardedDenseSource(const double* r, long long lr, const double* c, long long lc) : dRows(r), ldr(lr), dCols(c), ldc(lc) {}
  bool device_elems(const DeviceHSS& H, hssk_elem_src* e) const override {
    const Node& c = H.nodes_[H.o_.world == 1 ? 0 : H.cut_nodes_[H.o_.rank]];
    e->A = dCols - (long long)c.lo * ldc; e->lda = ldc; e->use_gen = 0;
    return true;
  }
  void sample(DeviceHSS& H, int r0, int dn) override {
    const bool single = H.o_.world == 1;
    if (!single && !H.dist_subtree_) throw std::invalid_argument("sharded operand: the tree cannot be cut into one subtree per rank (world must be a power of two and the tree complete down to that depth)");
    if (H.sj_pat_) throw std::invalid_argument("sharded operand: the SJLT sketch needs the replicated-operand interface");
    const long long N = H.n_;
    const Node& c = H.nodes_[single ? 0 : H.cut_nodes_[H.o_.rank]];
    const long long j0 = c.lo, nloc = c.m;
    auto timed = [&] { ck(hssk_dgemm_timing_defer(H.ctx_)); };
    ck(hssk_dgemm(H.ctx_, 0, dn, nloc, N, 1.0, H.Rt_ + r0, H.dcap_, dCols, ldc, 0.0, H.Sct_ + r0 + j0 * H.dcap_, H.dcap_));
    timed();
    if (dRows) {
      ck(hssk_dgemm(H.ctx_, 1, dn, nloc, N, 1.0, H.Rt_ + r0, H.dcap_, dRows, ldr, 0.0, H.Srt_ + r0 + j0 * H.dcap_, H.dcap_));
      timed();
    } else {
      H.tmp_->rewind();
      double* P = H.tmp_->dbl((size_t)dn * N);
      double* mineP = H.tmp_->dbl((size_t)dn * nloc);
      ck(hssk_dgemm(H.ctx_, 1, dn, N, nloc, 1.0, H.Rt_ + r0 + j0 * H.dcap_, H.dcap_, dCols, ldc, 0.0, P, dn));
      timed();
      const double tc = now();
      std::vector<long long> offs(H.o_.world), counts(H.o_.world);
      for (int g = 0; g < H.o_.world; g++) {
        const Node& cg = H.nodes_[single ? 0 : H.cut_nodes_[g]];
        offs[g] = (long long)cg.lo * dn; counts[g] = (long long)cg.m * dn;
      }
      H.reduce_scatter_sum(P, offs, counts, mineP);
      hssk_colgather_desc cp{mineP, H.Srt_ + r0 + j0 * H.dcap_, nullptr, dn, (int)nloc, dn, H.dcap_, 0};
      ck(hssk_gather_cols(H.ctx_, &cp, 1));
      ck(hssk_sync(H.ctx_));
      H.stats_.t_comm += now() - tc;
    }
  }
  void extract(DeviceHSS& H, const std::vector<ElemReq>& reqs) override {
    const Node& c = H.nodes_[H.o_.world == 1 ? 0 : H.cut_nodes_[H.o_.rank]];
    const int j0 = c.lo, j1 = c.lo + c.m;
    auto inside = [&](const std::vector<int>* h, int i0, int cnt) {
      if (!h) return i0 >= j0 && i0 + cnt <= j1;
      for (int i = 0; i < cnt; i++) if ((*h)[i] < j0 || (*h)[i] >= j1) return false;
      return true;
    };
    std::vector<hssk_elem_desc> own, part, back;
    size_t tot = 0;
    for (auto& r : reqs) if (r.m > 0 && r.n > 0 && !(inside(r.hI, r.i0, r.m) && inside(r.hJ, r.j0, r.n))) tot += (size_t)r.m * r.n;
    double* stage = tot ? H.comm_arena_->dbl(tot) : nullptr;
    size_t off = 0;
    for (auto& r : reqs) {
      if (r.m <= 0 || r.n <= 0) continue;
      if (inside(r.hI, r.i0, r.m) && inside(r.hJ, r.j0, r.n)) {
        own.push_back(hssk_elem_desc{dCols - (long long)j0 * ldc, ldc, r.dI, r.dJ, r.i0, r.j0, r.dB, r.m, r.n, r.ldb, 0, 0, 0, 0, 0});
      } else {
        double* T = stage + off;
        off += (size_t)r.m * r.n;
        if (dRows) part.push_back(hssk_elem_desc{dRows - j0, ldr, r.dI, r.dJ, r.i0, r.j0, T, r.m, r.n, r.m, 0, j0, j1, 0, 0});
        else part.push_back(hssk_elem_desc{dCols - (long long)j0 * ldc, ldc, r.dI, r.dJ, r.i0, r.j0, T, r.m, r.n, r.m, 0, 0, 0, j0, j1});
        back.push_back(hssk_elem_desc{T, r.m, nullptr, nullptr, 0, 0, r.dB, r.m, r.n, r.ldb, 0, 0, 0, 0, 0});
      }
    }
    if (!own.empty()) ck(hssk_gather_elems(H.ctx_, own.data(), (int)own.size()));
    if (!part.empty()) {
      const double tc = now();
      ck(hssk_gather_elems(H.ctx_, part.data(), (int)part.size()));
      H.allreduce_sum(stage, (long long)tot);
      ck(hssk_gather_elems(H.ctx_, back.data(), (int)back.size()));
      H.stats_.t_comm += now() - tc;
    }
  }
};

struct DeviceHSS::HostBlockSource : DeviceHSS::Source {
  const void* hA;
  long long lda;
  int dtype = HSSK_DT_F64;
  const host_fill_t* fill;
  const host_elem_t* elem;
  double* dBuf[2] = {nullptr, nullptr};
  double* dNat[2] = {nullptr, nullptr};
  long long nb = 0;
  int gen = -1;
  std::vector<double*> dcache;
  HostBlockSource(const void* a, long long l, const host_fill_t* f, const host_elem_t* e, int dt = HSSK_DT_F64)
      : hA(a), lda(l), dtype(dt), fill(f), elem(e) {}
  long long reals() const { return dtype == HSSK_DT_C32 || dtype == HSSK_DT_C64 ? 2 : 1; }
  size_t esize() const { return dtype == HSSK_DT_F32 ? 4 : dtype == HSSK_DT_C64 ? 16 : 8; }
  double image_at(size_t I, size_t J) const {
    switch (dtype) {
      case HSSK_DT_F32: return (double)((const float*)hA)[I + J * (size_t)lda];
      case HSSK_DT_C32: {
        const float* z = (const float*)hA + 2 * (I / 2 + (J / 2) * (size_t)lda);
        return (I & 1) == (J & 1) ? (double)z[0] : ((I & 1) ? (double)z[1] : -(double)z[1]);
      }
      case HSSK_DT_C64: {
        const double* z = (const double*)hA + 2 * (I / 2 + (J / 2) * (size_t)lda);
        return (I & 1) == (J & 1) ? z[0] : ((I & 1) ? z[1] : -z[1]);
      }
// ... 115 lines not shown
        (*elem)(r.m, I.data(), r.n, J.data(), B, r.m);
      }
    });
    for (size_t k = 0; k < reqs.size(); k++) {
      const ElemReq& r = reqs[k];
      if (r.m <= 0 || r.n <= 0 || hit[k]) continue;
      if (r.ldb == r.m) ck(hssk_upload_async(H.ctx_, r.dB, img.data() + off[k], (long long)(sizeof(double) * (off[k + 1] - off[k]))));
      else ck(hssk_memcpy2d_h2d(H.ctx_, r.dB, sizeof(double) * r.ldb, img.data() + off[k], sizeof(double) * r.m, sizeof(double) * r.m, r.n));
    }
  }
};

struct DeviceHSS::CallbackSource : DeviceHSS::Source {
  const host_mult_t* mult;
  const host_sample_t* usample = nullptr;
  const host_elem_t& elem;
  CallbackSource(const host_mult_t& m, const host_elem_t& e) : mult(&m), elem(e) {}
  CallbackSource(const host_sample_t& s, const host_elem_t& e) : mult(nullptr), usample(&s), elem(e) {}
  void sample(DeviceHSS& H, int r0, int dn) override {
    if (H.o_.world > 1) throw std::invalid_argument("the host-callback interface is single-GPU");
    if (usample) {
      const int N = H.n_;
      if (N == 0 || dn == 0) return;
      std::vector<double> R((size_t)N * dn), Sr((size_t)N * dn), Sc((size_t)N * dn);
      (*usample)(N, dn, R.data(), Sr.data(), Sc.data());
      double* dT = H.tmp_->dbl((size_t)N * dn);
      const double* src[3] = {R.data(), Sr.data(), Sc.data()};
      double* dst[3] = {H.Rt_ + r0, H.Srt_ + r0, H.Sct_ + r0};
      for (int q = 0; q < 3; q++) {
        ck(hssk_memcpy_h2d(H.ctx_, dT, src[q], (long long)(sizeof(double) * (size_t)N * dn)));
        hssk_transpose_desc b{dT, dst[q], N, dn, N, H.dcap_};
        ck(hssk_transpose(H.ctx_, &b, 1));
        ck(hssk_sync(H.ctx_));
      }
      return;
    }
    const int N = H.n_;
    if (N == 0 || dn == 0) return;
    double* dT = H.tmp_->dbl((size_t)N * dn);
    std::vector<double> R((size_t)N * dn), S((size_t)N * dn);
    hssk_transpose_desc t{H.Rt_ + r0, dT, dn, N, H.dcap_, N};
    ck(hssk_transpose(H.ctx_, &t, 1));
    ck(hssk_memcpy_d2h(H.ctx_, R.data(), dT, (long long)(sizeof(double) * R.size())));
    for (int pass = 0; pass < 2; pass++) {
      (*mult)(pass == 0 ? 'N' : 'C', N, dn, R.data(), N, S.data(), N);
      ck(hssk_memcpy_h2d(H.ctx_, dT, S.data(), (long long)(sizeof(double) * S.size())));
      hssk_transpose_desc b{dT, (pass == 0 ? H.Srt_ : H.Sct_) + r0, N, dn, N, H.dcap_};
      ck(hssk_transpose(H.ctx_, &b, 1));
      ck(hssk_sync(H.ctx_));
    }
  }
  void extract(DeviceHSS& H, const std::vector<ElemReq>& reqs) override {
    for (auto& r : reqs) {
      if (r.m <= 0 || r.n <= 0) continue;
      std::vector<int> I(r.m), J(r.n);
      for (int i = 0; i < r.m; i++) I[i] = r.hI ? (*r.hI)[i] : r.i0 + i;
      for (int j = 0; j < r.n; j++) J[j] = r.hJ ? (*r.hJ)[j] : r.j0 + j;
      std::vector<double> B((size_t)r.m * r.n);
      elem(r.m, I.data(), r.n, J.data(), B.data(), r.m);
      ck(hssk_memcpy2d_h2d(H.ctx_, r.dB, sizeof(double) * r.ldb, B.data(), sizeof(double) * r.m, sizeof(double) * r.m, r.n));
    }
  }
};

struct DeviceHSS::GeneratorSource : DeviceHSS::Source {
  hssk_gen g;
  explicit GeneratorSource(const hssk_gen& g_) : g(g_) {}
  bool extract_before_sample() const override { return true; }
  bool device_elems(const DeviceHSS&, hssk_elem_src* e) const override { e->A = nullptr; e->lda = 0; e->gen = g; e->use_gen = 1; return true; }
  int products(const DeviceHSS& H) const override { return H.o_.symmetric ? 1 : 2; }
  void sample(DeviceHSS& H, int r0, int dn) override {
    if (H.sj_pat_) throw std::invalid_argument("generated operand: the SJLT sketch streams a stored matrix; use the Gaussian sketch");
    const long long N = H.n_;
    long long j0 = 0, j1 = N;
    if (H.dist_subtree_) {
      const Node& c = H.nodes_[H.cut_nodes_[H.o_.rank]];
      j0 = c.lo; j1 = c.lo + c.m;
    } else if (H.o_.world > 1) {
      j0 = std::min(N, H.cols_per_rank_ * H.o_.rank); j1 = std::min(N, j0 + H.cols_per_rank_);
    }
    const long long nloc = j1 - j0;
    auto timed = [&] { ck(hssk_dgemm_timing_defer(H.ctx_)); };
    if (nloc > 0) {
      ck(hssk_sketch_gen(H.ctx_, &g, 1, dn, nloc, N, j0, 1.0, H.Rt_ + r0, H.dcap_, 0.0, H.Srt_ + r0 + j0 * H.dcap_, H.dcap_));
      timed();
      if (H.o_.symmetric) {
        hssk_colgather_desc cp{H.Srt_ + r0 + j0 * H.dcap_, H.Sct_ + r0 + j0 * H.dcap_, nullptr, dn, (int)nloc, H.dcap_, H.dcap_, 0};
        ck(hssk_gather_cols(H.ctx_, &cp, 1));
      } else {
        ck(hssk_sketch_gen(H.ctx_, &g, 0, dn, nloc, N, j0, 1.0, H.Rt_ + r0, H.dcap_, 0.0, H.Sct_ + r0 + j0 * H.dcap_, H.dcap_));
        timed();
      }
    }
    if (H.o_.world > 1 && !H.dist_subtree_) {
      const long long bytes = (long long)sizeof(double) * H.dcap_ * H.cols_per_rank_;
      H.comm(H.Srt_, bytes);
      H.comm(H.Sct_, bytes);
    }
  }
  void extract(DeviceHSS& H, const std::vector<ElemReq>& reqs) override {
    std::vector<hssk_elem_desc> d;
    d.reserve(reqs.size());
    for (auto& r : reqs)
      if (r.m > 0 && r.n > 0) d.push_back(hssk_elem_desc{nullptr, 0, r.dI, r.dJ, r.i0, r.j0, r.dB, r.m, r.n, r.ldb, 0});
    if (!d.empty()) ck(hssk_gen_elems(H.ctx_, &g, d.data(), (int)d.size()));
  }
};

void DeviceHSS::compress_generator(const hssk_gen& g) {
  GeneratorSource s(g);
  check_symmetry(s);
  compress(s);
}
void DeviceHSS::check_symmetry(Source& src) {
  if (o_.symmetric != 2 || n_ < 2) return;
  const int q = std::min(512, n_);
  std::vector<int> I(q), J(q);
  std::minstd_rand g(12345);
  for (int i = 0; i < q; i++) { I[i] = (int)(g() % (unsigned)n_); J[i] = (int)(g() % (unsigned)n_); }
  tmp_->rewind();
  int* dI = tmp_->ints(q);
  int* dJ = tmp_->ints(q);
  double* B1 = tmp_->dbl((size_t)q * q);
  double* B2 = tmp_->dbl((size_t)q * q);
  ck(hssk_memcpy_h2d(ctx_, dI, I.data(), (long long)sizeof(int) * q));
  ck(hssk_memcpy_h2d(ctx_, dJ, J.data(), (long long)sizeof(int) * q));
  std::vector<ElemReq> rq{ElemReq{dI, dJ, &I, &J, 0, 0, q, q, B1, q}, ElemReq{dJ, dI, &J, &I, 0, 0, q, q, B2, q}};
  src.extract(*this, rq);
  std::vector<double> h1((size_t)q * q), h2((size_t)q * q);
  ck(hssk_memcpy_d2h(ctx_, h1.data(), B1, (long long)sizeof(double) * q * q));
  ck(hssk_memcpy_d2h(ctx_, h2.data(), B2, (long long)sizeof(double) * q * q));
  double dmax = 0, amax = 0;
  for (int j = 0; j < q; j++)
    for (int i = 0; i < q; i++) {
      dmax = std::max(dmax, std::abs(h1[i + (size_t)j * q] - h2[j + (size_t)i * q]));
      amax = std::max(amax, std::abs(h1[i + (size_t)j * q]));
    }
  if (dmax > 1e-14 * std::max(amax, 1e-300)) throw std::invalid_argument("compress: the operand was declared symmetric and is not (sampled entries differ from their mirror images)");
}

void DeviceHSS::compress_dense_device(const double* dA, long long lda) {
  DenseDeviceSource s(dA, lda);
  check_symmetry(s);
  compress(s);
}
void DeviceHSS::compress_dense_device_f32(const float* dA, long long lda, int precision) {
  if (precision < 0 || precision > 2) throw std::invalid_argument("compress_dense_device_f32: sketch precision must be 0 (auto), 1 (FP32 matrix cores) or 2 (exact)");
  if (o_.world > 1) throw std::invalid_argument("compress_dense_device_f32: single-GPU only (multi-GPU float operands are not supported)");
  if (o_.sketch == 1) throw std::invalid_argument("compress_dense_device_f32: the SJLT sketch is not supported on a float operand; use the Gaussian sketch");
  if (!dA || lda < n_) throw std::invalid_argument("compress_dense_device_f32: bad operand");
  const int route = precision ? precision : (o_.rel_tol >= ((double)n_ + 4.) * std::ldexp(1., -24) ? 1 : 2);
  f32_route_ = route;
  DenseDeviceSourceF32 s(dA, lda, route);
  check_symmetry(s);
  compress(s);
}
void DeviceHSS::compress_dense_host(const double* A, long long lda) {
  HostBlockSource s(A, lda, nullptr, nullptr);
  compress(s);
}
void DeviceHSS::compress_dense_host_typed(const void* A, long long lda, int dtype) {
  if (dtype != HSSK_DT_F32 && dtype != HSSK_DT_C32 && dtype != HSSK_DT_C64) throw std::invalid_argument("compress_dense_host_typed: unknown scalar type");
  HostBlockSource s(A, lda, nullptr, nullptr, dtype);
  compress(s);
}
void DeviceHSS::compress_host_blocks(const host_fill_t& fill, const host_elem_t& elem) {
  HostBlockSource s(nullptr, 0, &fill, &elem);
  compress(s);
}
void DeviceHSS::compress_dense_device_sharded(const double* dRows, long long ldr, const double* dCols, long long ldc) {
  if (!dCols) throw std::invalid_argument("sharded operand: the column block is required");
  ShardedDenseSource s(dRows, ldr, dCols, ldc);
  compress(s);
}
bool DeviceHSS::shard_range(int rank, int& lo, int& hi) const {
  if (o_.world == 1) { lo = 0; hi = n_; return true; }
  if (!dist_subtree_ || rank < 0 || rank >= (int)cut_nodes_.size()) return false;
// ... 17 lines not shown
```

strumpack_amd/csrc/kernels/hssk_ctx.hip:

```cpp
#include "hssk_internal.h"

#include <cstdlib>
#include <unistd.h>

#include <atomic>
#include <condition_variable>
#include <functional>
#include <mutex>
#include <thread>
#include <vector>

static thread_local std::string g_err;
static std::mutex g_pool_mu;
static std::vector<hssk_ctx*> g_pool;
void hssk_set_error(const std::string& msg) { g_err = msg; }

thread_local std::vector<std::function<void()>>* hssk_rec::sink = nullptr;

struct hssk_uploader {
  static constexpr int SLOTS = 4;
  static constexpr size_t CHUNK = size_t(256) << 20;
  hssk_rt::stream_t copy{};
  hssk_rt::event_t ev_copy{}, ev_compute{};
  hssk_rt::event_t ev_mark[2];
  bool marked[2] = {false, false};
  char* pinned[SLOTS] = {nullptr, nullptr, nullptr, nullptr};
  hssk_rt::event_t slot_ev[SLOTS];
  bool slot_busy[SLOTS] = {false, false, false, false};
  int next = 0;
  hssk_uploader() {
    copy = hssk_rt::stream_create();
    ev_copy = hssk_rt::event_create();
    ev_compute = hssk_rt::event_create();
    ev_mark[0] = hssk_rt::event_create();
    ev_mark[1] = hssk_rt::event_create();
    for (int i = 0; i < SLOTS; i++) slot_ev[i] = hssk_rt::event_create();
  }
  char* slot(int s) {
    if (!pinned[s]) pinned[s] = (char*)hssk_rt::pinned_malloc(CHUNK);
    return pinned[s];
  }
  void release_slots() {
    try { hssk_rt::sync(copy); } catch (...) {}
    for (int i = 0; i < SLOTS; i++) {
      if (pinned[i]) hssk_rt::pinned_free(pinned[i]);
      pinned[i] = nullptr;
      slot_busy[i] = false;
    }
  }
  ~hssk_uploader() {
    try { hssk_rt::sync(copy); } catch (...) {}
    for (int i = 0; i < SLOTS; i++) { if (pinned[i]) hssk_rt::pinned_free(pinned[i]); hssk_rt::event_destroy(slot_ev[i]); }
    hssk_rt::event_destroy(ev_copy);
    hssk_rt::event_destroy(ev_compute);
    hssk_rt::event_destroy(ev_mark[0]);
    hssk_rt::event_destroy(ev_mark[1]);
    hssk_rt::stream_destroy(copy);
  }
};
static hssk_uploader* uploader(hssk_ctx* c) {
  if (!c->uploader) c->uploader = new hssk_uploader();
  return c->uploader;
}
class PackPool {
 public:
  explicit PackPool(unsigned n) : n_(n), pid_(getpid()) {
    for (unsigned t = 0; t < n_; t++) th_.emplace_back([this, t] { loop(t); });
  }
  ~PackPool() {
    if (getpid() != pid_) { for (auto& t : th_) t.detach(); return; }
    { std::lock_guard<std::mutex> g(mu_); stop_ = true; gen_++; }
    cv_.notify_all();
    for (auto& t : th_) t.join();
  }
  unsigned size() const { return n_; }
  void run(const std::function<void(unsigned)>& fn) {
    if (getpid() != pid_) { for (unsigned t = 0; t < n_; t++) fn(t); return; }
    std::lock_guard<std::mutex> own(owner_);
    std::unique_lock<std::mutex> lk(mu_);
    fn_ = &fn; pending_ = n_; gen_++;
    cv_.notify_all();
    done_.wait(lk, [&] { return pending_ == 0; });
  }

 private:
  void loop(unsigned t) {
    unsigned long seen = 0;
    for (;;) {
      const std::function<void(unsigned)>* f;
      {
        std::unique_lock<std::mutex> lk(mu_);
        cv_.wait(lk, [&] { return gen_ != seen; });
        seen = gen_;
        if (stop_) return;
        f = fn_;
      }
      (*f)(t);
      { std::lock_guard<std::mutex> g(mu_); if (--pending_ == 0) done_.notify_all(); }
    }
  }
// ... 69 lines not shown
    u->slot_busy[s] = true;
  }
}

extern "C" {

int hssk_h2d_block_async(hssk_ctx* c, double* dst, long long ldd, const double* src, long long lds, long long rows,
                         long long cols) {
  HSSK_API_BEGIN
  if (rows <= 0 || cols <= 0) return 0;
  h2d_bytes(c, (char*)dst, sizeof(double) * (size_t)ldd, (const char*)src, sizeof(double) * (size_t)lds, sizeof(double) * (size_t)rows, cols);
  HSSK_API_END
}
int hssk_h2d_bytes_async(hssk_ctx* c, void* dst, long long dpitch, const void* src, long long spitch, long long width, long long cols) {
  HSSK_API_BEGIN
  if (width <= 0 || cols <= 0) return 0;
  if (dpitch < width || spitch < width) HSSK_UNSUPPORTED("pitch smaller than the row width");
  h2d_bytes(c, (char*)dst, (size_t)dpitch, (const char*)src, (size_t)spitch, (size_t)width, cols);
  HSSK_API_END
}
int hssk_copy_fence(hssk_ctx* c) {
  HSSK_API_BEGIN
  hssk_uploader* u = uploader(c);
  hssk_rt::event_record(u->ev_copy, u->copy);
  hssk_rt::stream_wait_event(c->stream, u->ev_copy);
  HSSK_API_END
}
int hssk_compute_fence(hssk_ctx* c) {
  HSSK_API_BEGIN
  hssk_uploader* u = uploader(c);
  hssk_rt::event_record(u->ev_compute, c->stream);
  hssk_rt::stream_wait_event(u->copy, u->ev_compute);
  HSSK_API_END
}
int hssk_compute_mark(hssk_ctx* c, int slot) {
  HSSK_API_BEGIN
  hssk_uploader* u = uploader(c);
  hssk_rt::event_record(u->ev_mark[slot & 1], c->stream);
  u->marked[slot & 1] = true;
  HSSK_API_END
}
int hssk_copy_wait(hssk_ctx* c, int slot) {
  HSSK_API_BEGIN
  hssk_uploader* u = uploader(c);
  if (u->marked[slot & 1]) hssk_rt::stream_wait_event(u->copy, u->ev_mark[slot & 1]);
  HSSK_API_END
}

const char* hssk_last_error(void) { return g_err.c_str(); }

int hssk_ctx_create(hssk_ctx** out, int device) {
  HSSK_API_BEGIN
  if (hssk_rt::device_count() <= device)
    throw std::runtime_error("hssk_ctx_create: no HIP device " + std::to_string(device) +
                             " (this library has no CPU fallback)");
  hssk_rt::set_device(device);
  {
    std::lock_guard<std::mutex> g(g_pool_mu);
    for (size_t i = 0; i < g_pool.size(); i++)
      if (g_pool[i]->device == device) {
        *out = g_pool[i];
        g_pool.erase(g_pool.begin() + i);
        return 0;
      }
  }
  hssk_ctx* c = new hssk_ctx;
  c->device = device;
  c->stream = hssk_rt::stream_create();
  c->ring_bytes = size_t(64) << 20;
  c->h_ring = (char*)hssk_rt::pinned_malloc(c->ring_bytes);
  c->zero_copy_bytes = hssk_rt::pinned_is_device_visible() ? 65536 : 0;
  if (const char* e = std::getenv("HSSK_ZERO_COPY_BYTES")) c->zero_copy_bytes = (size_t)std::atoll(e);
  c->d_ring = (char*)hssk_rt::dev_malloc(c->ring_bytes);
  c->ev0 = hssk_rt::event_create();
  c->ev1 = hssk_rt::event_create();
  c->ev_sync = hssk_rt::event_create();
  *out = c;
  HSSK_API_END
}

void hssk_ctx_destroy(hssk_ctx* c) {
  if (!c) return;
  try { hssk_rt::sync(c->stream); } catch (...) {}
  {
    std::lock_guard<std::mutex> g(g_pool_mu);
    if (g_pool.size() < 8) {
      if (c->uploader) c->uploader->release_slots();
      c->ring_off = 0;
      c->dgemm_timed = false;
      if (c->on_side) { c->stream = c->main_saved; c->on_side = false; }
      for (int i = 0; i < 8; i++) {
        for (auto& p : c->watch[i]) { c->watch_free.push_back(p.first); c->watch_free.push_back(p.second); }
        c->watch[i].clear();
        c->watch_open[i] = false;
      }
      c->recording = nullptr;
      c->require_mma = false;
      g_pool.push_back(c);
      return;
    }
  }
  hssk_rt::pinned_free(c->h_ring);
  hssk_rt::dev_free(c->d_ring);
  hssk_rt::dev_free(c->d_scratch);
  hssk_rt::dev_free(c->d_aux);
  hssk_rt::dev_free(c->d_gen);
  delete c->uploader;
  hssk_rt::pinned_free(c->h_sweep_err);
  for (auto& w : c->watch) for (auto& p : w) { hssk_rt::event_destroy(p.first); hssk_rt::event_destroy(p.second); }
  for (auto& b : c->dgemm_deferred) { hssk_rt::event_destroy(b.a); hssk_rt::event_destroy(b.b); }
  for (auto e : c->watch_free) hssk_rt::event_destroy(e);
  hssk_rt::event_destroy(c->ev0);
  hssk_rt::event_destroy(c->ev_sync);
  if (c->side_made) { hssk_rt::event_destroy(c->ev_fork); hssk_rt::event_destroy(c->ev_join); hssk_rt::stream_destroy(c->side); }
  hssk_rt::event_destroy(c->ev1);
  hssk_rt::stream_destroy(c->stream);
  delete c;
}

void* hssk_ctx_stream(hssk_ctx* c) { return (void*)c->stream; }

int hssk_stream_wait(hssk_ctx* waiter, hssk_ctx* on) {
  HSSK_API_BEGIN
  if (!waiter || !on) throw std::invalid_argument("hssk_stream_wait: null context");
  if (waiter == on) return 0;
  hssk_rt::event_record(on->ev_sync, on->stream);
  hssk_rt::stream_wait_event(waiter->stream, on->ev_sync);
  HSSK_API_END
}
int hssk_side_begin(hssk_ctx* c) {
  HSSK_API_BEGIN
  if (c->on_side) throw std::logic_error("hssk_side_begin: already on the side stream");
  if (!c->side_made) {
    c->side = hssk_rt::stream_create();
    c->ev_fork = hssk_rt::event_create();
    c->ev_join = hssk_rt::event_create();
    c->side_made = true;
  }
  auto f = [c]() {
    hssk_rt::event_record(c->ev_fork, c->stream);
    hssk_rt::stream_wait_event(c->side, c->ev_fork);
    c->main_saved = c->stream;
    c->stream = c->side;
    c->on_side = true;
  };
  f();
  if (hssk_rec::sink) hssk_rec::sink->push_back(f);
  HSSK_API_END
}
int hssk_side_end(hssk_ctx* c) {
  HSSK_API_BEGIN
  if (!c->on_side) throw std::logic_error("hssk_side_end: not on the side stream");
  auto f = [c]() { c->stream = c->main_saved; c->on_side = false; };
  f();
  if (hssk_rec::sink) hssk_rec::sink->push_back(f);
  HSSK_API_END
}
int hssk_side_join(hssk_ctx* c) {
  HSSK_API_BEGIN
  if (c->on_side) throw std::logic_error("hssk_side_join: still on the side stream");
  if (!c->side_made) return 0;
  auto f = [c]() {
    hssk_rt::event_record(c->ev_join, c->side);
    hssk_rt::stream_wait_event(c->stream, c->ev_join);
  };
  f();
// ... 200 lines not shown
```

strumpack_amd/csrc/kernels/hssk_dgemm.hip:

```cpp
#include "hssk_device.h"
#include "hssk_internal.h"
#include "hssk_gen.h"

#include <algorithm>
#include <cstdlib>
#include <type_traits>

namespace {

constexpr int BN = 64, BK = 16;

template <int BM, bool TRANSB, bool FULL, int TAG = 0>
__global__ __launch_bounds__(256, 2) void dgemm_kernel(int m, long long n, long long k, const double* __restrict__ A,
                                                       long long lda, const double* __restrict__ B, long long ldb,
                                                       double* __restrict__ P, long long ldp, long long pstride,
                                                       long long kchunk, int jtile0, long long* __restrict__ clk) {
  const long long t0_ = clk ? hssk_clock() : 0, w0_ = clk ? hssk_wallclock() : 0;
  constexpr int LDA_S = BM + 16, LDB_S = BN + 16;
  constexpr int WM = BM / 2;
  constexpr int MT = WM / 16;
  constexpr int NT = 2;
  constexpr int A_PER_THREAD = BM * BK / 256;
  constexpr int B_PER_THREAD = BN * BK / 256;
  constexpr int A2 = A_PER_THREAD / 2, B2 = B_PER_THREAD / 2;
// ... 339 lines not shown
      lds[SLOT + A_DBL + tid] = gen_tau(16 + tid);
    }
    hssk_wait_glds<2 * NCH>();
    hssk_wg_barrier();
    frags(0, 0, 0);
    int st = 0;
    for (; st + 3 <= nst; st += 3) {
      stage(st, std::integral_constant<int, 0>());
      stage(st + 1, std::integral_constant<int, 1>());
      stage(st + 2, std::integral_constant<int, 2>());
    }
    if (st < nst) stage(st, std::integral_constant<int, 0>());
    if (st + 1 < nst) stage(st + 1, std::integral_constant<int, 1>());
    hssk_wait_glds<0>();
  }
  double* Pz = P + (long long)blockIdx.z * pstride;
#pragma unroll
  for (int a = 0; a < MT; a++)
#pragma unroll
    for (int b = 0; b < NT; b++)
#pragma unroll
      for (int r = 0; r < 4; r++) {
        const int gi = i0 + wm + a * 16 + l15;
        const long long gj = j0 + wn + b * 16 + l4 + 4 * r;
        Pz[gi + gj * ldp] = acc[a][b][r];
      }
  if (clk && threadIdx.x == 0) {
    const long long w1 = hssk_wallclock();
    if (blockIdx.x == 0 && blockIdx.y == 0 && blockIdx.z == 0) {
      clk[0] = hssk_clock() - t0_;
      clk[1] = w1 - w0_;
    }
    const long long fid = blockIdx.x + (long long)gridDim.x * (blockIdx.y + (long long)gridDim.y * blockIdx.z);
    long long* rec = clk + 4 + 4 * fid;
    rec[0] = w0_; rec[1] = w1; rec[2] = hssk_hwid(); rec[3] = bx;
  }
}

__global__ void dgemm_reduce_kernel(int m, long long n, const double* __restrict__ P, long long ldp,
                                    long long pstride, int nz, double alpha, double beta,
                                    double* __restrict__ C, long long ldc) {
  long long total = (long long)m * n;
  for (long long e = (long long)blockIdx.x * blockDim.x + threadIdx.x; e < total;
       e += (long long)gridDim.x * blockDim.x) {
    int i = (int)(e % m);
    long long j = e / m;
    double s = 0.;
    for (int z = 0; z < nz; z++) s += P[i + j * ldp + z * pstride];
    double* c = C + i + j * ldc;
    double v = alpha * s;
    if (beta != 0.) v += beta * (*c);
    *c = v;
  }
}

__global__ void dgemm_reduce_wide_kernel(int m, long long n, const double* __restrict__ P, long long ldp,
                                         long long pstride, int nz, double alpha, double beta,
                                         double* __restrict__ C, long long ldc) {
  HSSK_SHARED double s_part[256];
  const int el = threadIdx.x & 15, zl = threadIdx.x >> 4;
  const long long total = (long long)m * n;
  for (long long e0 = (long long)blockIdx.x * 16; e0 < total; e0 += (long long)gridDim.x * 16) {
    const long long e = e0 + el;
    const int i = (int)(e % m);
    const long long j = e / m;
    double s = 0.;
    if (e < total) {
      const double* p = P + i + j * ldp;
      for (int z = zl; z < nz; z += 16) s += p[z * pstride];
    }
    s_part[threadIdx.x] = s;
    __syncthreads();
    if (zl == 0 && e < total) {
      double t = 0.;
      for (int q = 0; q < 16; q++) t += s_part[el + 16 * q];
      double* c = C + i + j * ldc;
      double v = alpha * t;
      if (beta != 0.) v += beta * (*c);
      *c = v;
    }
    __syncthreads();
  }
}

template <int BM, bool FULL, int TAG>
void launch_dgemm(hssk_ctx* ctx, int transB, dim3 grid, int m, long long n, long long k, const double* A,
                  long long lda, const double* B, long long ldb, double* P, long long ldp, long long pstride,
                  long long kchunk, int jtile0, long long* clk) {
  if (grid.x == 0) return;
  if (transB)
    HSSK_LAUNCH((dgemm_kernel<BM, true, FULL, TAG>), grid, dim3(256), 0, ctx->stream, m, n, k, A, lda, B, ldb, P, ldp, pstride, kchunk, jtile0, clk);
  else
    HSSK_LAUNCH((dgemm_kernel<BM, false, FULL, TAG>), grid, dim3(256), 0, ctx->stream, m, n, k, A, lda, B, ldb, P, ldp, pstride, kchunk, jtile0, clk);
}

}

namespace {
template <bool FULL, int TAG>
void launch_bm(int BM, hssk_ctx* ctx, int transB, dim3 grid, int m, long long n, long long k, const double* A,
               long long lda, const double* B, long long ldb, double* P, long long ldp, long long pstride,
               long long kchunk, int jtile0, long long* clk) {
  if (BM == 192) launch_dgemm<192, FULL, TAG>(ctx, transB, grid, m, n, k, A, lda, B, ldb, P, ldp, pstride, kchunk, jtile0, clk);
  else if (BM == 128) launch_dgemm<128, FULL, TAG>(ctx, transB, grid, m, n, k, A, lda, B, ldb, P, ldp, pstride, kchunk, jtile0, clk);
  else launch_dgemm<64, FULL, TAG>(ctx, transB, grid, m, n, k, A, lda, B, ldb, P, ldp, pstride, kchunk, jtile0, clk);
}

constexpr int BN2 = 128;
inline size_t sketch_lds_bytes(int mblk) { return sizeof(double) * 3 * (size_t)(64 * mblk + BN2) * BK; }
template <int MBLK, int TAG>
void launch_sketch_m(hssk_ctx* ctx, int transB, dim3 grid, long long n, long long k, const double* A, long long lda,
                     const double* B, long long ldb, double* P, long long ldp, long long pstride, long long kchunk,
                     int jtile0, long long* clk, const hssk_gen* gen, long long jg0) {
  const size_t shm = sketch_lds_bytes(MBLK);
  const hssk_gen g0{0, 0, {0., 0., 0., 0.}};
  if (gen) {
    if (transB) HSSK_LAUNCH((sketch_kernel<MBLK, true, TAG, true>), grid, dim3(512), shm, ctx->stream, n, k, A, lda, B, ldb, P, ldp, pstride, kchunk, jtile0, clk, *gen, jg0);
    else HSSK_LAUNCH((sketch_kernel<MBLK, false, TAG, true>), grid, dim3(512), shm, ctx->stream, n, k, A, lda, B, ldb, P, ldp, pstride, kchunk, jtile0, clk, *gen, jg0);
  } else {
    if (transB) HSSK_LAUNCH((sketch_kernel<MBLK, true, TAG, false>), grid, dim3(512), shm, ctx->stream, n, k, A, lda, B, ldb, P, ldp, pstride, kchunk, jtile0, clk, g0, jg0);
    else HSSK_LAUNCH((sketch_kernel<MBLK, false, TAG, false>), grid, dim3(512), shm, ctx->stream, n, k, A, lda, B, ldb, P, ldp, pstride, kchunk, jtile0, clk, g0, jg0);
  }
}
template <int MBLK>
bool sketch_prepare_m() {
  static const bool ok = [] {
    try {
      const size_t b = sketch_lds_bytes(MBLK);
      if (b > hssk_rt::max_lds_per_workgroup()) return false;
      hssk_rt::allow_dynamic_lds(sketch_kernel<MBLK, true, 0, false>, b);
      hssk_rt::allow_dynamic_lds(sketch_kernel<MBLK, false, 0, false>, b);
      hssk_rt::allow_dynamic_lds(sketch_kernel<MBLK, true, 1, false>, b);
      hssk_rt::allow_dynamic_lds(sketch_kernel<MBLK, false, 1, false>, b);
      hssk_rt::allow_dynamic_lds(sketch_kernel<MBLK, true, 0, true>, b);
      hssk_rt::allow_dynamic_lds(sketch_kernel<MBLK, false, 0, true>, b);
      hssk_rt::allow_dynamic_lds(sketch_kernel<MBLK, true, 1, true>, b);
      hssk_rt::allow_dynamic_lds(sketch_kernel<MBLK, false, 1, true>, b);
      return true;
    } catch (const std::exception&) {
      return false;
    }
  }();
  return ok;
}
inline bool sketch_prepare(int BM) {
  return BM == 192 ? sketch_prepare_m<3>() : (BM == 128 ? sketch_prepare_m<2>() : sketch_prepare_m<1>());
}
template <int TAG>
void launch_sketch(int BM, hssk_ctx* ctx, int transB, dim3 grid, long long n, long long k, const double* A, long long lda,
                   const double* B, long long ldb, double* P, long long ldp, long long pstride, long long kchunk,
                   int jtile0, long long* clk, const hssk_gen* gen, long long jg0) {
  if (grid.x == 0) return;
  if (BM == 192) launch_sketch_m<3, TAG>(ctx, transB, grid, n, k, A, lda, B, ldb, P, ldp, pstride, kchunk, jtile0, clk, gen, jg0);
  else if (BM == 128) launch_sketch_m<2, TAG>(ctx, transB, grid, n, k, A, lda, B, ldb, P, ldp, pstride, kchunk, jtile0, clk, gen, jg0);
  else launch_sketch_m<1, TAG>(ctx, transB, grid, n, k, A, lda, B, ldb, P, ldp, pstride, kchunk, jtile0, clk, gen, jg0);
}
}

static void dgemm_impl(hssk_ctx* ctx, int transB, int m, long long n, long long k, double alpha, const double* A, long long lda,
                       const double* B, long long ldb, const hssk_gen* gen, long long jg0, double beta, double* C, long long ldc) {
  if (m <= 0 || n <= 0) return;
  const int BM = m > 128 ? 192 : (m > 64 ? 128 : 64);
  const unsigned gm = (unsigned)((m + BM - 1) / BM);
  const long long ksteps = (k + BK - 1) / BK;
  const bool aligned = (m % BM == 0) && (k % BK == 0) && (lda % 2 == 0) && (gen || ldb % 2 == 0) &&
                       (((size_t)A | (gen ? (size_t)0 : (size_t)B)) % 16 == 0);
  static const int cus = hssk_rt::cu_count();
  const bool force_v1 = [] { const char* e = std::getenv("HSSK_DGEMM_V1"); return e && std::atoi(e) != 0; }();
  const bool v2 = aligned && (gen || !force_v1) && k > 0 && n >= BN2 && sketch_prepare(BM);
  if (gen && !v2) {
    const long long nb_max = std::max<long long>(64, std::min<long long>(1024, (long long)(size_t(1) << 28) / std::max<long long>(k, 1)));
    const long long ldg = k + (k & 1);
    for (long long c0 = 0; c0 < n; c0 += nb_max) {
      const long long nb = std::min(nb_max, n - c0);
      double* G = ctx->gen_block(sizeof(double) * (size_t)ldg * nb);
      if (hssk_gen_fill(ctx, gen, G, k, nb, ldg, 0, jg0 + c0, transB)) throw std::runtime_error(hssk_last_error());
      dgemm_impl(ctx, 0, m, nb, k, alpha, A, lda, G, ldg, nullptr, 0, beta, C + c0 * ldc, ldc);
    }
    return;
  }
  const int BNt = v2 ? BN2 : BN;
  static const bool no_fold = [] { const char* e = std::getenv("HSSK_DGEMM_NO_FOLD"); return e && std::atoi(e) != 0; }();
  const bool fold_edge = v2 && !no_fold && n % BNt != 0 && n % 2 == 0;
  const unsigned gn_full = aligned ? (unsigned)(n / BNt) + (fold_edge ? 1u : 0u) : 0u;
  const long long edge_col0 = std::min<long long>(n, (long long)gn_full * BNt);
  const unsigned gn_edge = (unsigned)((n - edge_col0 + BN - 1) / BN);
  const long long slots = v2 ? cus : 2LL * cus;
  struct Group { long long col0 = 0, ntiles = 0; int split = 1; long long kchunk = BK; int nz = 0; double* P = nullptr; long long cols = 0, vcols = 0; };
  auto chunk_of = [&](int split) {
    long long c = ((ksteps + split - 1) / split) * BK;
    return c > 0 ? c : (long long)BK;
  };
  auto max_split = [&]() { return (int)std::max<long long>(1, std::min<long long>(256, ksteps / 24)); };
  auto one_round_split = [&](long long tiles) {
    if (tiles <= 0 || k <= 0) return 1;
    return (int)std::max<long long>(1, std::min<long long>(max_split(), slots / tiles));
  };
  Group gmain, gtail, gedge;
  if (gn_full) {
    const long long T = (long long)gm * gn_full;
    const double epi = 3.0, red = 0.0067 * (BNt / BN);
    double best = 1e300;
    int best_s = 1;
    long long best_main = T;
    const int sp_min = (int)std::min<long long>(std::min(max_split(), 64), (ksteps + 1023) / 1024);
    for (int sp = std::max(1, sp_min); sp <= std::min(max_split(), 64); sp++) {
      const long long r = (T * sp) / slots;
      long long tm = r > 0 ? std::min<long long>(T, (r * slots) / sp) : 0;
      if (gm > 1) tm = T;
      const long long tt = T - tm;
      double cost = 0.;
      if (tm) cost += (double)((tm * sp + slots - 1) / slots) * ((double)(ksteps + sp - 1) / sp + epi) + red * sp * (double)tm;
      if (tt) {
        const int st = one_round_split(tt);
        cost += (double)((tt * st + slots - 1) / slots) * ((double)(ksteps + st - 1) / st + epi) + red * st * (double)tt + 2.0;
      }
      if (cost < best - 1e-9) { best = cost; best_s = sp; best_main = tm; }
    }
    if (k <= 0) { best_s = 1; best_main = T; }
    if (const char* e = std::getenv("HSSK_DGEMM_SPLIT")) {
      const int sp = std::max(1, std::min(max_split(), std::atoi(e)));
      const long long r = (T * sp) / slots;
      best_s = sp;
      best_main = (gm > 1 || r == 0) ? T : std::min<long long>(T, (r * slots) / sp);
    }
    gmain.col0 = 0; gmain.ntiles = gm > 1 ? gn_full : best_main; gmain.split = best_s; gmain.cols = gmain.ntiles * BNt;
    gtail.col0 = gmain.cols; gtail.ntiles = gn_full - gmain.ntiles; gtail.split = one_round_split(gtail.ntiles); gtail.cols = gtail.ntiles * BNt;
  }
  gedge.col0 = edge_col0; gedge.ntiles = gn_edge; gedge.split = one_round_split((long long)gm * gn_edge); gedge.cols = n - edge_col0;
  const long long ldp = m;
  size_t ptot = 0;
  for (Group* g : {&gmain, &gtail, &gedge}) {
    if (!g->ntiles) continue;
    g->vcols = std::min(g->cols, n - g->col0);
    g->kchunk = chunk_of(g->split);
    g->nz = (int)std::max<long long>(1, (k + g->kchunk - 1) / g->kchunk);
    ptot += (size_t)ldp * g->cols * g->nz;
  }
  const size_t ntrace = gmain.ntiles ? (size_t)gmain.ntiles * gm * gmain.nz : 0;
  double* P = ctx->scratch(sizeof(double) * (ptot + 4 + 4 * ntrace));
  long long* clk = (long long*)(P + ptot);
  {
    double* q = P;
    for (Group* g : {&gmain, &gtail, &gedge}) {
      if (!g->ntiles) continue;
      g->P = q;
      q += (size_t)ldp * g->cols * g->nz;
    }
  }
  auto shifted = [&](const Group& g) { return g.P - g.col0 * ldp; };
  const Group* timed = gmain.ntiles ? &gmain : (gtail.ntiles ? &gtail : &gedge);
  auto bracket = [&](const Group* g, auto&& launch) {
    if (!g->ntiles) return;
    if (g == timed) hssk_rt::event_record(ctx->ev0, ctx->stream);
    launch();
    if (g == timed) hssk_rt::event_record(ctx->ev1, ctx->stream);
  };
  auto grid_of = [&](const Group& g) { return dim3((unsigned)g.ntiles, gm, (unsigned)g.nz); };
  if (gen && gedge.ntiles) {
    const long long ldg = k + (k & 1);
    double* G = ctx->gen_block(sizeof(double) * (size_t)ldg * gedge.cols);
    if (hssk_gen_fill(ctx, gen, G, k, gedge.cols, ldg, 0, jg0 + gedge.col0, transB)) throw std::runtime_error(hssk_last_error());
    const double* Gs = G - gedge.col0 * ldg;
    bracket(&gedge, [&] { launch_bm<false, 0>(BM, ctx, 0, grid_of(gedge), m, n, k, A, lda, Gs, ldg, shifted(gedge), ldp, ldp * gedge.cols, gedge.kchunk, (int)(gedge.col0 / BN), nullptr); });
  } else
  bracket(&gedge, [&] { launch_bm<false, 0>(BM, ctx, transB, grid_of(gedge), m, n, k, A, lda, B, ldb, shifted(gedge), ldp, ldp * gedge.cols, gedge.kchunk, (int)(gedge.col0 / BN), nullptr); });
  if (v2) {
    bracket(&gtail, [&] { launch_sketch<1>(BM, ctx, transB, grid_of(gtail), n, k, A, lda, B, ldb, shifted(gtail), ldp, ldp * gtail.cols, gtail.kchunk, (int)(gtail.col0 / BN2), nullptr, gen, jg0); });
    bracket(&gmain, [&] { launch_sketch<0>(BM, ctx, transB, grid_of(gmain), n, k, A, lda, B, ldb, shifted(gmain), ldp, ldp * gmain.cols, gmain.kchunk, (int)(gmain.col0 / BN2), clk, gen, jg0); });
  } else {
    bracket(&gtail, [&] { launch_bm<true, 1>(BM, ctx, transB, grid_of(gtail), m, n, k, A, lda, B, ldb, shifted(gtail), ldp, ldp * gtail.cols, gtail.kchunk, (int)(gtail.col0 / BN), nullptr); });
    bracket(&gmain, [&] { launch_bm<true, 0>(BM, ctx, transB, grid_of(gmain), m, n, k, A, lda, B, ldb, shifted(gmain), ldp, ldp * gmain.cols, gmain.kchunk, (int)(gmain.col0 / BN), clk); });
  }
  ctx->d_clk = gmain.ntiles ? clk : nullptr;
  ctx->dgemm_trace_wgs = (long long)ntrace;
  ctx->dgemm_timed = true;
  ctx->dgemm_timed_flops = 2.0 * (double)m * (double)timed->vcols * (double)k;
  for (const Group* g : {&gmain, &gtail, &gedge}) {
    if (!g->ntiles) continue;
    long long total = (long long)m * g->vcols;
    unsigned rb = (unsigned)std::min<long long>((total + 255) / 256, 4096);
    if (g->nz >= 32 && total <= 65536)
      HSSK_LAUNCH(dgemm_reduce_wide_kernel, dim3((unsigned)((total + 15) / 16)), dim3(256), 0, ctx->stream, m, g->vcols, (const double*)g->P, ldp, ldp * g->cols, g->nz, alpha, beta, C + g->col0 * ldc, ldc);
    else
      HSSK_LAUNCH(dgemm_reduce_kernel, dim3(rb), dim3(256), 0, ctx->stream, m, g->vcols, (const double*)g->P, ldp, ldp * g->cols, g->nz, alpha, beta, C + g->col0 * ldc, ldc);
  }
  hssk_rt::check_launch();
}

extern "C" int hssk_dgemm(hssk_ctx* ctx, int transB, int m, long long n, long long k, double alpha,
                          const double* A, long long lda, const double* B, long long ldb, double beta,
                          double* C, long long ldc) {
  HSSK_API_BEGIN
  dgemm_impl(ctx, transB, m, n, k, alpha, A, lda, B, ldb, nullptr, 0, beta, C, ldc);
  HSSK_API_END
}

extern "C" int hssk_sketch_gen(hssk_ctx* ctx, const hssk_gen* g, int transG, int m, long long n, long long k, long long j0,
                               double alpha, const double* A, long long lda, double beta, double* C, long long ldc) {
  HSSK_API_BEGIN
  if (!g || (g->kind != HSSK_GEN_TOEPLITZ && g->kind != HSSK_GEN_TOEPLITZ_UPPER)) throw std::invalid_argument("hssk_sketch_gen: unknown generator kind");
  if (k > 0x7fffffffLL || j0 + n > 0x7fffffffLL) throw std::invalid_argument("hssk_sketch_gen: indices beyond 2^31");
  dgemm_impl(ctx, transG, m, n, k, alpha, A, lda, nullptr, 0, g, j0, beta, C, ldc);
  HSSK_API_END
}
```

strumpack_amd/csrc/kernels/hssk_gemm_vbatched.hip:

```cpp
#include "hssk_device.h"
#include "hssk_internal.h"

#include <algorithm>
#include <cstdlib>
#include <vector>

namespace {

constexpr int TM = 64, TN = 64, TK = 16;
constexpr int LDS_LD = 80;

struct Tile {
  int prob, tm, tn;
};

__global__ __launch_bounds__(256) void gemm_vbatched_kernel(const hssk_gemm_desc* __restrict__ descs,
                                                            const Tile* __restrict__ tiles) {
  HSSK_SHARED double As[TK * LDS_LD];
  HSSK_SHARED double Bs[TK * LDS_LD];
  const Tile t = tiles[blockIdx.x];
  const hssk_gemm_desc p = descs[t.prob];
  const int tid = threadIdx.x, lane = tid & 63, wave = tid >> 6;
  const int i0 = t.tm * TM, j0 = t.tn * TN;
  const int wm = (wave & 1) * 32, wn = (wave >> 1) * 32;
// ... 137 lines not shown
      const bool ok = (iA[r] < m) && (k0 + kkA[r] < k);
      const hssk_d2 v = hssk_gload2(A, min(iA[r], m - 2) + (size_t)min(k0 + kkA[r], k - 1) * p.lda);
      ra[r] = ok ? v : hssk_d2{0., 0.};
    }
#pragma unroll
    for (int r = 0; r < 2; r++) {
      const int gj = j0 + jB[r], gk = k0 + kkB[r];
      const bool ok = gj < n && gk < k;
      const int cj = min(gj, n - 1), ck = min(gk, k - 1);
      const double v = TRANSB ? hssk_gload(B, cj + (size_t)ck * p.ldb) : hssk_gload(B, ck + (size_t)cj * p.ldb);
      rb[r] = ok ? v : 0.;
    }
  };
  auto store = [&](int buf, const hssk_d2 (&ra)[6], const double (&rb)[2]) {
    double* as = As + buf * PBK * PLDA;
    double* bs = Bs + buf * PBK * PLDB;
#pragma unroll
    for (int r = 0; r < 6; r++) *reinterpret_cast<hssk_d2*>(as + ldsA[r]) = ra[r];
#pragma unroll
    for (int r = 0; r < 2; r++) bs[kkB[r] * PLDB + jB[r]] = rb[r];
  };
  auto compute = [&](int buf) {
    const double* as = As + buf * PBK * PLDA + wm + l15;
    const double* bs = Bs + buf * PBK * PLDB + l15;
#pragma unroll
    for (int ks = 0; ks < PBK; ks += 4) {
      double af[3], bf[2];
#pragma unroll
      for (int a = 0; a < 3; a++) af[a] = as[(ks + l4) * PLDA + a * 16];
#pragma unroll
      for (int b = 0; b < 2; b++) bf[b] = bs[(ks + l4) * PLDB + b * 16];
#pragma unroll
      for (int a = 0; a < 3; a++)
#pragma unroll
        for (int b = 0; b < 2; b++) acc[a][b] = hssk_mfma_f64_16x16x4(bf[b], af[a], acc[a][b]);
    }
  };
  const int nst = (k + PBK - 1) / PBK;
  load(0, ra0, rb0);
  store(0, ra0, rb0);
  if (nst > 1) load(PBK, ra1, rb1);
  __syncthreads();
  int st = 0;
  for (; st + 2 < nst; st += 2) {
    load((st + 2) * PBK, ra0, rb0);
    compute(0);
    store(1, ra1, rb1);
    __syncthreads();
    if (st + 3 < nst) load((st + 3) * PBK, ra1, rb1);
    compute(1);
    store(0, ra0, rb0);
    __syncthreads();
  }
  compute(0);
  if (st + 1 < nst) {
    store(1, ra1, rb1);
    __syncthreads();
    compute(1);
  }
  double cv[3][2][4];
  if (p.beta != 0.) {
#pragma unroll
    for (int a = 0; a < 3; a++)
#pragma unroll
      for (int b = 0; b < 2; b++)
#pragma unroll
        for (int r = 0; r < 4; r++)
          cv[a][b][r] = hssk_gload(p.C, min(wm + a * 16 + l15, m - 1) + (size_t)min(j0 + b * 16 + l4 + 4 * r, n - 1) * p.ldc);
  }
#pragma unroll
  for (int a = 0; a < 3; a++)
#pragma unroll
    for (int b = 0; b < 2; b++)
#pragma unroll
      for (int r = 0; r < 4; r++) {
        const int gi = wm + a * 16 + l15;
        const int gj = j0 + b * 16 + l4 + 4 * r;
        double v = p.alpha * acc[a][b][r];
        if (p.beta != 0.) v += p.beta * cv[a][b][r];
        if (gi < m && gj < n) hssk_gstore(p.C, gi + (size_t)gj * p.ldc, v);
      }
}

__global__ __launch_bounds__(256, 2) void leaf_update_kernel(const hssk_leaf_update_desc* __restrict__ descs,
                                                             const Tile* __restrict__ tiles) {
  HSSK_SHARED double As[2 * PBK * PLDA];
  HSSK_SHARED double Bs[2 * 2 * PBK * PLDB];
  const Tile t = tiles[blockIdx.x];
  if (t.prob < 0) return;
  const hssk_leaf_update_desc p = descs[t.prob];
  const int tid = threadIdx.x, lane = tid & 63, wave = tid >> 6;
  const int l15 = lane & 15, l4 = lane >> 4;
  const int j0 = t.tn * PBN;
  const int wm = wave * 48;
  const int d = p.d, m = p.m;
  const double* __restrict__ A = p.R;
  const double* __restrict__ D = p.D;

  hssk_d4 acc[2][3][2];
#pragma unroll
  for (int q = 0; q < 2; q++)
#pragma unroll
    for (int a = 0; a < 3; a++)
#pragma unroll
      for (int b = 0; b < 2; b++) acc[q][a][b] = hssk_d4{0., 0., 0., 0.};

  int ldsA[6], kkA[6], iA[6];
#pragma unroll
  for (int r = 0; r < 6; r++) {
    const int e = tid + 256 * r;
    iA[r] = 2 * (e % (PBM / 2));
    kkA[r] = e / (PBM / 2);
    ldsA[r] = kkA[r] * PLDA + iA[r];
  }
  int j1[2], k1[2], j2[2], k2[2];
#pragma unroll
  for (int r = 0; r < 2; r++) {
    const int e = tid + 256 * r;
    j1[r] = e % PBN; k1[r] = e / PBN;
    k2[r] = e % PBK; j2[r] = e / PBK;
  }
  hssk_d2 ra[6];
  double rb1[2], rb2[2];
  auto load = [&](int k0) {
#pragma unroll
    for (int r = 0; r < 6; r++) {
      const bool ok = (iA[r] < d) && (k0 + kkA[r] < m);
      const hssk_d2 v = hssk_gload2(A, min(iA[r], d - 2) + (size_t)min(k0 + kkA[r], m - 1) * p.ldr);
      ra[r] = ok ? v : hssk_d2{0., 0.};
    }
#pragma unroll
    for (int r = 0; r < 2; r++) {
      const int gj = j0 + j1[r], gk = k0 + k1[r];
      const double v1 = hssk_gload(D, min(gj, m - 1) + (size_t)min(gk, m - 1) * p.ldd);
      rb1[r] = (gj < m && gk < m) ? v1 : 0.;
      const int hj = j0 + j2[r], hk = k0 + k2[r];
      const double v2 = hssk_gload(D, min(hk, m - 1) + (size_t)min(hj, m - 1) * p.ldd);
      rb2[r] = (hj < m && hk < m) ? v2 : 0.;
    }
  };
  auto store = [&](int buf) {
    double* as = As + buf * PBK * PLDA;
    double* b1 = Bs + (buf * 2 + 0) * PBK * PLDB;
    double* b2 = Bs + (buf * 2 + 1) * PBK * PLDB;
#pragma unroll
    for (int r = 0; r < 6; r++) *reinterpret_cast<hssk_d2*>(as + ldsA[r]) = ra[r];
#pragma unroll
    for (int r = 0; r < 2; r++) {
      b1[k1[r] * PLDB + j1[r]] = rb1[r];
      b2[k2[r] * PLDB + j2[r]] = rb2[r];
    }
  };
  auto compute = [&](int buf) {
    const double* as = As + buf * PBK * PLDA + wm + l15;
    const double* b1 = Bs + (buf * 2 + 0) * PBK * PLDB + l15;
    const double* b2 = Bs + (buf * 2 + 1) * PBK * PLDB + l15;
#pragma unroll
    for (int ks = 0; ks < PBK; ks += 4) {
      double af[3], bf[2][2];
#pragma unroll
      for (int a = 0; a < 3; a++) af[a] = as[(ks + l4) * PLDA + a * 16];
#pragma unroll
      for (int b = 0; b < 2; b++) { bf[0][b] = b1[(ks + l4) * PLDB + b * 16]; bf[1][b] = b2[(ks + l4) * PLDB + b * 16]; }
#pragma unroll
      for (int q = 0; q < 2; q++)
#pragma unroll
        for (int a = 0; a < 3; a++)
#pragma unroll
          for (int b = 0; b < 2; b++) acc[q][a][b] = hssk_mfma_f64_16x16x4(bf[q][b], af[a], acc[q][a][b]);
    }
  };
  const int nst = (m + PBK - 1) / PBK;
  load(0);
  store(0);
  __syncthreads();
  int buf = 0;
  for (int st = 0; st + 1 < nst; st++) {
    load((st + 1) * PBK);
    compute(buf);
    store(buf ^ 1);
    __syncthreads();
    buf ^= 1;
  }
  compute(buf);
#pragma unroll
  for (int q = 0; q < 2; q++) {
    double* C = q == 0 ? p.Sr : p.Sc;
    double cv[3][2][4];
#pragma unroll
    for (int a = 0; a < 3; a++)
#pragma unroll
      for (int b = 0; b < 2; b++)
#pragma unroll
        for (int r = 0; r < 4; r++)
          cv[a][b][r] = hssk_gload(C, min(wm + a * 16 + l15, d - 1) + (size_t)min(j0 + b * 16 + l4 + 4 * r, m - 1) * p.lds);
#pragma unroll
    for (int a = 0; a < 3; a++)
#pragma unroll
      for (int b = 0; b < 2; b++)
#pragma unroll
        for (int r = 0; r < 4; r++) {
          const int gi = wm + a * 16 + l15;
          const int gj = j0 + b * 16 + l4 + 4 * r;
          if (gi < d && gj < m) hssk_gstore(C, gi + (size_t)gj * p.lds, cv[a][b][r] - acc[q][a][b][r]);
        }
  }
}

inline bool panel_eligible(const hssk_gemm_desc& d) {
  return d.transA == 0 && d.m > 64 && d.m <= PBM && (d.m % 2 == 0) && (d.lda % 2 == 0) &&
         ((size_t)d.A % 16 == 0) && d.k > 0 && d.n > 0;
}


constexpr int TALL_T = 512, TALL_M = 256, TALL_N = 64, TALL_LDB = TALL_N + 1, TALL_CH = 8, TALL_KMAX = 256, TALL_KH = 128;

__global__ __launch_bounds__(TALL_T) HSSK_WAVES_PER_SIMD(4) void gemm_tall_kernel(const hssk_gemm_desc* __restrict__ descs, const Tile* __restrict__ tiles) {
  HSSK_DYN_SHARED(double, Bs);
  const Tile t = tiles[blockIdx.x];
  const hssk_gemm_desc p = descs[t.prob];
  const int tid = threadIdx.x, lane = tid & 63, wave = hssk_uniform(tid >> 6);
  const int l15 = lane & 15, l4 = lane >> 4;
  const int m = p.m, n = p.n, k = p.k;
  const int nh = (k + TALL_KH - 1) / TALL_KH;
  const int kc = (((k + nh - 1) / nh) + 3) & ~3;
  const int r0 = t.tm * TALL_M;
  constexpr int NW = TALL_T / 64, NTL = TALL_M / 16 / NW;
  hssk_d4 acc[NTL][4];
#pragma unroll
  for (int q = 0; q < NTL; q++)
#pragma unroll
    for (int ct = 0; ct < 4; ct++) acc[q][ct] = hssk_d4{0., 0., 0., 0.};
  for (int kb = 0; kb < k; kb += kc) {
    const int kn = min(kc, k - kb);
    if (kb) __syncthreads();
    {
      const int cs = TALL_T / kn, kk = tid % kn, jq = tid / kn;
      if (jq < cs)
        for (int j = jq; j < TALL_N; j += 8 * cs) {
          double v[8];
#pragma unroll
          for (int u = 0; u < 8; u++) v[u] = hssk_gload(p.B, (size_t)(kb + kk) + (size_t)min(j + u * cs, n - 1) * p.ldb);
#pragma unroll
          for (int u = 0; u < 8; u++)
            if (j + u * cs < TALL_N) Bs[kk * TALL_LDB + j + u * cs] = j + u * cs < n ? v[u] : 0.;
        }
    }
    __syncthreads();
    const int nks = (kn + 3) >> 2;
    const int nch = hssk_uniform((nks + TALL_CH - 1) / TALL_CH);
#pragma unroll
    for (int q = 0; q < NTL; q++) {
      const int tl = wave + q * NW;
      if (r0 + tl * 16 >= m) continue;
      const int i = r0 + tl * 16 + l15;
      auto aload = [&](int kk) -> double {
        const int ic = min(i, m - 1), kg = kb + min(kk, kn - 1);
        return p.transA ? hssk_gload(p.A, (size_t)kg + (size_t)ic * p.lda) : hssk_gload(p.A, (size_t)ic + (size_t)kg * p.lda);
      };
      auto chunk = [&](int k0, const double (&a)[TALL_CH]) {
#pragma unroll
        for (int u = 0; u < TALL_CH; u++) {
          const int kk = k0 + 4 * u;
          const double* xr = Bs + min(kk, kn - 1) * TALL_LDB + l15;
#pragma unroll
          for (int ct = 0; ct < 4; ct++) acc[q][ct] = hssk_mfma_f64_16x16x4(kk < kn ? xr[ct * 16] : 0., a[u], acc[q][ct]);
        }
      };
      double a0[TALL_CH], a1[TALL_CH];
#pragma unroll
// ... 124 lines not shown
    }
    if (tall_eligible(d)) {
      for (int tm = 0; tm * TALL_M < d.m; tm++) ttiles.push_back(Tile{p, tm, 0});
      {
        const int nh = (d.k + TALL_KH - 1) / TALL_KH;
        kmax_tall = std::max(kmax_tall, (((d.k + nh - 1) / nh) + 3) & ~3);
      }
      continue;
    }
    if (panel_eligible(d)) {
      std::vector<Tile>& dst = d.transB ? ptilesT : ptilesN;
      for (int tn = 0; tn * PBN < d.n; tn++) dst.push_back(Tile{p, 0, tn});
      continue;
    }
    int ntm = (d.m + TM - 1) / TM, ntn = (d.n + TN - 1) / TN;
    std::vector<Tile>& dst = (d.k > 0) ? tiles : ztiles;
    for (int tn = 0; tn < ntn; tn++)
      for (int tm = 0; tm < ntm; tm++) dst.push_back(Tile{p, tm, tn});
  }
  if (tiles.empty() && ztiles.empty() && ptilesN.empty() && ptilesT.empty() && ttiles.empty() && vtiles.empty()) return 0;
  auto* d_descs = (const hssk_gemm_desc*)ctx->stage(descs, sizeof(hssk_gemm_desc) * count);
  auto xcd_order = [](std::vector<Tile>& v) {
    if (v.size() < 16) return;
    std::vector<std::vector<Tile>> lanes(8);
    int cur = -1, lane = -1;
    for (const Tile& t : v) {
      if (t.prob != cur) { cur = t.prob; lane = (lane + 1) & 7; }
      lanes[lane].push_back(t);
    }
    std::vector<Tile> out;
    out.reserve(v.size() + 64);
    size_t longest = 0;
    for (auto& l : lanes) longest = std::max(longest, l.size());
    for (size_t i = 0; i < longest; i++)
      for (int x = 0; x < 8; x++)
        out.push_back(i < lanes[x].size() ? lanes[x][i] : Tile{-1, 0, 0});
    v.swap(out);
  };
  xcd_order(ptilesN);
  xcd_order(ptilesT);
  if (!ptilesN.empty()) {
    auto* d_tiles = (const Tile*)ctx->stage(ptilesN.data(), sizeof(Tile) * ptilesN.size());
    HSSK_LAUNCH((gemm_panel_kernel<false>), dim3((unsigned)ptilesN.size()), dim3(256), 0, ctx->stream, d_descs, d_tiles);
  }
  if (!ptilesT.empty()) {
    auto* d_tiles = (const Tile*)ctx->stage(ptilesT.data(), sizeof(Tile) * ptilesT.size());
    HSSK_LAUNCH((gemm_panel_kernel<true>), dim3((unsigned)ptilesT.size()), dim3(256), 0, ctx->stream, d_descs, d_tiles);
  }
  if (!vtiles.empty()) {
    auto* d_tiles = (const Tile*)ctx->stage(vtiles.data(), sizeof(Tile) * vtiles.size());
    HSSK_LAUNCH(gemv_small_kernel, dim3((unsigned)vtiles.size()), dim3(GV_T), 0, ctx->stream, d_descs, d_tiles);
  }
  if (!ttiles.empty()) {
    auto* d_tiles = (const Tile*)ctx->stage(ttiles.data(), sizeof(Tile) * ttiles.size());
    const size_t lds = sizeof(double) * (size_t)kmax_tall * TALL_LDB;
    hssk_rt::allow_dynamic_lds(gemm_tall_kernel, lds);
    HSSK_LAUNCH(gemm_tall_kernel, dim3((unsigned)ttiles.size()), dim3(TALL_T), lds, ctx->stream, d_descs, d_tiles);
  }
  if (!tiles.empty()) {
    auto* d_tiles = (const Tile*)ctx->stage(tiles.data(), sizeof(Tile) * tiles.size());
    HSSK_LAUNCH(gemm_vbatched_kernel, dim3((unsigned)tiles.size()), dim3(256), 0, ctx->stream, d_descs, d_tiles);
  }
  if (!ztiles.empty()) {
    auto* d_tiles = (const Tile*)ctx->stage(ztiles.data(), sizeof(Tile) * ztiles.size());
    HSSK_LAUNCH(gemm_scale_kernel, dim3((unsigned)ztiles.size()), dim3(256), 0, ctx->stream, d_descs, d_tiles);
  }
  hssk_rt::check_launch();
  HSSK_API_END
}

extern "C" int hssk_leaf_update_vbatched(hssk_ctx* ctx, const hssk_leaf_update_desc* descs, int count) {
  HSSK_API_BEGIN
  if (count <= 0) return 0;
  std::vector<Tile> tiles;
  for (int p = 0; p < count; p++) {
    const hssk_leaf_update_desc& d = descs[p];
    if (d.d <= 0 || d.m <= 0) continue;
    if (d.d > PBM || (d.d % 2) || (d.ldr % 2) || ((size_t)d.R % 16)) HSSK_UNSUPPORTED("panel shape outside the fused leaf update");
    for (int tn = 0; tn * PBN < d.m; tn++) tiles.push_back(Tile{p, 0, tn});
  }
  if (tiles.empty()) return 0;
  auto* dd = (const hssk_leaf_update_desc*)ctx->stage(descs, sizeof(*descs) * count);
  auto* dt = (const Tile*)ctx->stage(tiles.data(), sizeof(Tile) * tiles.size());
  HSSK_LAUNCH(leaf_update_kernel, dim3((unsigned)tiles.size()), dim3(256), 0, ctx->stream, dd, dt);
  hssk_rt::check_launch();
  HSSK_API_END
}
```

strumpack_amd/csrc/kernels/hssk_internal.h:

```cpp
#pragma once
#include <functional>
#include <vector>
#include <algorithm>
#include <utility>
#include <cstring>
#include <stdexcept>
#include <string>

#include "hssk.h"
#include "hssk_rt.h"

namespace hssk_rec {
extern thread_local std::vector<std::function<void()>>* sink;
}

struct hssk_plan {
  std::vector<std::function<void()>> launches;
  struct Block { char* dev; char* shadow; size_t size; };
  std::vector<Block> blocks;
  size_t off = 0;
  char* alloc(size_t bytes, char** shadow) {
    const size_t need = (bytes + 255) & ~size_t(255);
    if (blocks.empty() || off + need > blocks.back().size) {
      const size_t sz = std::max<size_t>(need, size_t(1) << 20);
      blocks.push_back(Block{(char*)hssk_rt::dev_malloc(sz), (char*)hssk_rt::pinned_malloc(sz), sz});
      off = 0;
    }
    char* p = blocks.back().dev + off;
    *shadow = blocks.back().shadow + off;
    off += need;
    return p;
  }
  ~hssk_plan() { for (auto& b : blocks) { hssk_rt::dev_free(b.dev); hssk_rt::pinned_free(b.shadow); } }
};

struct hssk_uploader;
struct hssk_ctx {
  int device = 0;
  hssk_rt::stream_t stream{};
  char* h_ring = nullptr;
  char* d_ring = nullptr;
  size_t ring_bytes = 0, ring_off = 0;
  size_t zero_copy_bytes = 0;
  hssk_rt::event_t ev0{}, ev1{};
  hssk_rt::event_t ev_sync{};
  hssk_rt::stream_t side{}, main_saved{};
  hssk_rt::event_t ev_fork{}, ev_join{};
  bool on_side = false, side_made = false;
  bool require_mma = false;
  bool dgemm_timed = false;
  double dgemm_timed_flops = 0.;
  struct TimedBracket { hssk_rt::event_t a, b; double flops; };
  std::vector<TimedBracket> dgemm_deferred;
  long long dgemm_trace_wgs = 0;
  long long* d_clk = nullptr;
  double* d_scratch = nullptr;
  struct hssk_uploader* uploader = nullptr;
  int* d_sweep_flags = nullptr;
  int* h_sweep_err = nullptr;
  std::vector<std::pair<hssk_rt::event_t, hssk_rt::event_t>> watch[8];
  std::vector<hssk_rt::event_t> watch_free;
  bool watch_open[8] = {false, false, false, false, false, false, false, false};
  size_t sweep_cap = size_t(1) << 20;
  size_t scratch_bytes = 0;

  hssk_plan* recording = nullptr;
  void* stage(const void* host, size_t bytes) {
    if (recording) {
      char* shadow = nullptr;
      char* p = recording->alloc(bytes, &shadow);
      std::memcpy(shadow, host, bytes);
      hssk_rt::h2d(p, shadow, bytes, stream);
      return p;
    }
    size_t need = (bytes + 255) & ~size_t(255);
    if (need > ring_bytes) throw std::runtime_error("hssk: descriptor batch exceeds staging ring");
    if (ring_off + need > ring_bytes) {
      hssk_rt::sync(stream);
      if (side_made) {
        hssk_rt::sync(side);
        if (on_side) hssk_rt::sync(main_saved);
      }
      ring_off = 0;
    }
    std::memcpy(h_ring + ring_off, host, bytes);
    void* d;
    if (bytes <= zero_copy_bytes) {
      d = h_ring + ring_off;
    } else {
      hssk_rt::h2d(d_ring + ring_off, h_ring + ring_off, bytes, stream);
      d = d_ring + ring_off;
    }
    ring_off += need;
    return d;
  }
  double* d_aux = nullptr;
  size_t aux_bytes = 0;
  void sync_all() {
    hssk_rt::sync(stream);
    if (side_made) {
      hssk_rt::sync(side);
      if (on_side) hssk_rt::sync(main_saved);
    }
  }
  double* aux(size_t bytes) {
    if (bytes > aux_bytes) {
      sync_all();
      hssk_rt::dev_free(d_aux);
      d_aux = (double*)hssk_rt::dev_malloc(bytes);
      aux_bytes = bytes;
    }
    return d_aux;
  }
  double* d_gen = nullptr;
  size_t gen_bytes = 0;
  double* gen_block(size_t bytes) {
    if (bytes > gen_bytes) {
      sync_all();
      hssk_rt::dev_free(d_gen);
      d_gen = (double*)hssk_rt::dev_malloc(bytes);
      gen_bytes = bytes;
    }
    return d_gen;
  }
  double* scratch(size_t bytes) {
    if (bytes > scratch_bytes) {
      sync_all();
      hssk_rt::dev_free(d_scratch);
      d_scratch = (double*)hssk_rt::dev_malloc(bytes);
      scratch_bytes = bytes;
    }
    return d_scratch;
  }
};

void hssk_set_error(const std::string& msg);

#define HSSK_UNSUPPORTED(msg) do { hssk_set_error(std::string(__func__) + ": " + (msg)); return 2; } while (0)
#define HSSK_API_BEGIN try {
#define HSSK_API_END                 \
  return 0;                          \
  }                                  \
  catch (const std::exception& e) {  \
    hssk_set_error(e.what());        \
    return 1;                        \
  }
```

strumpack_amd/hssk.py:

```python
import ctypes as C

import numpy as np

c_dp = C.POINTER(C.c_double)
c_ip = C.POINTER(C.c_int)


class GemmDesc(C.Structure):
    _fields_ = [("A", C.c_void_p), ("B", C.c_void_p), ("C", C.c_void_p),
                ("m", C.c_int), ("n", C.c_int), ("k", C.c_int),
                ("lda", C.c_int), ("ldb", C.c_int), ("ldc", C.c_int),
                ("transA", C.c_int), ("transB", C.c_int),
                ("alpha", C.c_double), ("beta", C.c_double)]


class LeafUpdateDesc(C.Structure):
    _fields_ = [("R", C.c_void_p), ("D", C.c_void_p), ("Sr", C.c_void_p), ("Sc", C.c_void_p),
                ("d", C.c_int), ("m", C.c_int), ("ldr", C.c_int), ("ldd", C.c_int), ("lds", C.c_int)]


class KernelSpec(C.Structure):
    _fields_ = [("X", C.c_void_p), ("n", C.c_longlong), ("d", C.c_int), ("type", C.c_int), ("p", C.c_int),
                ("h", C.c_double), ("lam", C.c_double)]

# ... 54 lines not shown
class TpqrDesc(C.Structure):
    _fields_ = [("R1", C.c_void_p), ("ld1", C.c_int), ("R2", C.c_void_p), ("ld2", C.c_int), ("m", C.c_int)]


class XsolveDesc(C.Structure):
    _fields_ = [("W", C.c_void_p), ("ldw", C.c_int), ("rank", C.c_int), ("m", C.c_int),
                ("X", C.c_void_p), ("ldx", C.c_int), ("solved", C.c_int)]


class PcholDesc(C.Structure):
    _fields_ = [("G", C.c_void_p), ("ldg", C.c_int), ("m", C.c_int), ("rtol", C.c_double), ("atol", C.c_double),
                ("max_rank", C.c_int), ("perm", C.c_void_p), ("rank", C.c_void_p), ("R", C.c_void_p), ("ldr", C.c_int)]


class SumDesc(C.Structure):
    _fields_ = [("P", C.c_void_p), ("stride", C.c_longlong), ("n", C.c_longlong), ("count", C.c_int), ("out", C.c_void_p)]


class GramDesc(C.Structure):
    _fields_ = [("W", C.c_void_p), ("ldw", C.c_int), ("rows", C.c_int), ("m", C.c_int), ("G", C.c_void_p), ("ldg", C.c_int)]


class GramGenDesc(C.Structure):
    _fields_ = [("ri", C.c_void_p), ("r0", C.c_int), ("ci", C.c_void_p), ("c0", C.c_int), ("rows", C.c_int), ("m", C.c_int),
                ("G", C.c_void_p), ("ldg", C.c_int)]


class QrDesc(C.Structure):
    _fields_ = [("A", C.c_void_p), ("lda", C.c_int), ("rows", C.c_int), ("cols", C.c_int),
                ("Q", C.c_void_p), ("ldq", C.c_int), ("nq", C.c_int),
                ("rdiag", C.c_void_p), ("work", C.c_void_p), ("stair", C.c_int),
                ("stop_rel", C.c_double), ("stop_abs", C.c_double), ("r_only", C.c_int)]


class TrsmDesc(C.Structure):
    _fields_ = [("T", C.c_void_p), ("B", C.c_void_p), ("n", C.c_int), ("nrhs", C.c_int),
                ("ldt", C.c_int), ("ldb", C.c_int), ("lower", C.c_int), ("transT", C.c_int),
                ("unit", C.c_int), ("Tinv", C.c_void_p)]


class TrtriDesc(C.Structure):
    _fields_ = [("R", C.c_void_p), ("Tinv", C.c_void_p), ("n", C.c_int), ("ldr", C.c_int), ("mode", C.c_int)]


class LuDesc(C.Structure):
    _fields_ = [("A", C.c_void_p), ("n", C.c_int), ("lda", C.c_int), ("piv", C.c_void_p),
                ("info", C.c_void_p)]


class LuSolveDesc(C.Structure):
    _fields_ = [("LU", C.c_void_p), ("piv", C.c_void_p), ("B", C.c_void_p),
                ("n", C.c_int), ("nrhs", C.c_int), ("lda", C.c_int), ("ldb", C.c_int)]


class NormDesc(C.Structure):
    _fields_ = [("P", C.c_void_p), ("rows", C.c_int), ("cols", C.c_int), ("ld", C.c_int),
                ("out", C.c_void_p)]


class ShiftDesc(C.Structure):
    _fields_ = [("A", C.c_void_p), ("n", C.c_int), ("lda", C.c_int)]


class Gen(C.Structure):
    _fields_ = [("kind", C.c_int), ("reserved", C.c_int), ("p", C.c_double * 4)]


HSSK_SYMBOLS = [
    "hssk_ctx_create", "hssk_ctx_destroy", "hssk_ctx_stream", "hssk_sync", "hssk_last_error",
    "hssk_malloc", "hssk_free", "hssk_memcpy_h2d", "hssk_memcpy_d2h", "hssk_last_dgemm_ms", "hssk_last_dgemm_flops", "hssk_last_dgemm_trace",
    "hssk_fill_toeplitz", "hssk_randn", "hssk_dgemm", "hssk_gemm_vbatched", "hssk_gather_cols",
    "hssk_gather_rows", "hssk_gather_elems", "hssk_transpose", "hssk_id_vbatched",
    "hssk_qr_vbatched", "hssk_trsm_vbatched", "hssk_getrf_vbatched", "hssk_getrs_vbatched",
    "hssk_sumsq_vbatched", "hssk_shift_diag", "hssk_mfma_f64_peak_tflops", "hssk_memcpy_d2d",
    "hssk_memcpy2d_h2d", "hssk_memcpy2d_d2h", "hssk_memset_zero", "hssk_is_device_pointer",
    "hssk_basis_dense", "hssk_mfma_f64_probe", "hssk_last_dgemm_clock_ghz", "hssk_leaf_update_vbatched", "hssk_formq_vbatched",
    "hssk_kernel_eval_vbatched", "hssk_knn", "hssk_kernel_predict", "hssk_copy_triu",
    "hssk_laswp_vbatched", "hssk_shift_diag_cplx", "hssk_upload_async", "hssk_h2d_block_async", "hssk_h2d_bytes_async", "hssk_expand_image", "hssk_copy_fence", "hssk_compute_fence", "hssk_compute_mark", "hssk_copy_wait", "hssk_id_xsolve_vbatched", "hssk_id_solves_inline", "hssk_gather_combine", "hssk_ulv_split", "hssk_tpqr_vbatched", "hssk_fill_toeplitz_block", "hssk_sum_slabs", "hssk_ulv_fwd_sweep", "hssk_ulv_bwd_sweep", "hssk_apply_sweep", "hssk_sweep_status", "hssk_sweep_arm", "hssk_trtri_diag_vbatched", "hssk_sjlt_dense", "hssk_sjlt_sketch",
    "hssk_plan_begin", "hssk_plan_end", "hssk_plan_replay", "hssk_plan_destroy", "hssk_plan_size",
    "hssk_sketch_gen", "hssk_gen_elems", "hssk_gen_fill", "hssk_colsets", "hssk_colsets_max_universe",
    "hssk_cluster_median", "hssk_pchol_id_vbatched", "hssk_pchol_id_max_m", "hssk_pchol_id_rank_cap", "hssk_sum_partials", "hssk_gram_vbatched", "hssk_gram_gen_vbatched", "hssk_gram_gen_supported",
    "hssk_sgemm_sketch", "hssk_narrow_f32", "hssk_gather_elems_f32",
    "hssk_kernel_predict_f32", "hssk_kernel_predict_splits",
]


class DevArray:

    def __init__(self, hk, shape, dtype=np.float64):
        self.hk, self.shape, self.dtype = hk, tuple(shape), np.dtype(dtype)
        self.nbytes = int(np.prod(self.shape)) * self.dtype.itemsize
        self.ptr = hk.lib.hssk_malloc(max(self.nbytes, 8))
        if not self.ptr:
            raise MemoryError(hk.error())

    def free(self):
        if self.ptr:
            self.hk.lib.hssk_free(self.ptr)
            self.ptr = None

    def __del__(self):
        try:
            self.free()
        except Exception:
            pass

    def get(self):
        out = np.empty(self.shape, dtype=self.dtype, order="F")
        if self.nbytes:
            self.hk.check(self.hk.lib.hssk_memcpy_d2h(self.hk.ctx, out.ctypes.data, self.ptr, self.nbytes))
        return out

    def set(self, arr):
        a = np.asfortranarray(arr, dtype=self.dtype)
        assert a.shape == self.shape
        if self.nbytes:
            self.hk.check(self.hk.lib.hssk_memcpy_h2d(self.hk.ctx, self.ptr, a.ctypes.data, self.nbytes))
        return self

    def at(self, *idx):
        off, stride = 0, 1
        for i, n in zip(idx, self.shape):
            off += i * stride
            stride *= n
        return self.ptr + off * self.dtype.itemsize


class Hssk:
    def __init__(self, path, device=0):
        self.lib = L = C.CDLL(path)
        L.hssk_malloc.restype = C.c_void_p
        L.hssk_malloc.argtypes = [C.c_longlong]
        L.hssk_free.argtypes = [C.c_void_p]
        L.hssk_last_error.restype = C.c_char_p
        L.hssk_ctx_create.argtypes = [C.POINTER(C.c_void_p), C.c_int]
        L.hssk_ctx_destroy.argtypes = [C.c_void_p]
        L.hssk_ctx_stream.restype = C.c_void_p
        L.hssk_ctx_stream.argtypes = [C.c_void_p]
        L.hssk_sync.argtypes = [C.c_void_p]
        L.hssk_memcpy_h2d.argtypes = [C.c_void_p, C.c_void_p, C.c_void_p, C.c_longlong]
        L.hssk_memcpy_d2h.argtypes = [C.c_void_p, C.c_void_p, C.c_void_p, C.c_longlong]
        L.hssk_memcpy_d2d.argtypes = [C.c_void_p, C.c_void_p, C.c_void_p, C.c_longlong]
        L.hssk_memset_zero.argtypes = [C.c_void_p, C.c_void_p, C.c_longlong]
        for f in ("hssk_memcpy2d_h2d", "hssk_memcpy2d_d2h"):
            getattr(L, f).argtypes = [C.c_void_p, C.c_void_p, C.c_longlong, C.c_void_p, C.c_longlong,
                                      C.c_longlong, C.c_longlong]
        L.hssk_is_device_pointer.argtypes = [C.c_void_p]
        L.hssk_last_dgemm_clock_ghz.restype = C.c_double
        L.hssk_last_dgemm_clock_ghz.argtypes = [C.c_void_p]
        L.hssk_last_dgemm_ms.restype = C.c_float
        L.hssk_last_dgemm_ms.argtypes = [C.c_void_p]
        L.hssk_last_dgemm_trace.restype = C.c_longlong
        L.hssk_last_dgemm_trace.argtypes = [C.c_void_p, C.c_void_p, C.c_longlong]
        L.hssk_last_dgemm_flops.restype = C.c_double
        L.hssk_last_dgemm_flops.argtypes = [C.c_void_p]
        L.hssk_fill_toeplitz.argtypes = [C.c_void_p, C.c_void_p, C.c_int, C.c_longlong, C.c_char]
        L.hssk_fill_toeplitz_block.argtypes = [C.c_void_p, C.c_void_p, C.c_int, C.c_int, C.c_longlong, C.c_int, C.c_int, C.c_char]
        L.hssk_sum_slabs.argtypes = [C.c_void_p, C.c_void_p, C.c_longlong, C.c_longlong, C.c_int, C.c_void_p]
        L.hssk_upload_async.argtypes = [C.c_void_p, C.c_void_p, C.c_void_p, C.c_longlong]
        L.hssk_h2d_block_async.argtypes = [C.c_void_p, C.c_void_p, C.c_longlong, C.c_void_p, C.c_longlong, C.c_longlong, C.c_longlong]
        L.hssk_copy_fence.argtypes = [C.c_void_p]
        L.hssk_compute_fence.argtypes = [C.c_void_p]
        L.hssk_h2d_bytes_async.argtypes = [C.c_void_p, C.c_void_p, C.c_longlong, C.c_void_p, C.c_longlong, C.c_longlong, C.c_longlong]
        L.hssk_expand_image.argtypes = [C.c_void_p, C.c_void_p, C.c_longlong, C.c_void_p, C.c_longlong, C.c_longlong, C.c_longlong, C.c_int]
        L.hssk_compute_mark.argtypes = [C.c_void_p, C.c_int]
        L.hssk_copy_wait.argtypes = [C.c_void_p, C.c_int]
        L.hssk_sweep_status.argtypes = [C.c_void_p]
        L.hssk_randn.argtypes = [C.c_void_p, C.c_void_p, C.c_int, C.c_longlong, C.c_longlong,
                                 C.c_int, C.c_longlong, C.c_ulonglong]
        L.hssk_dgemm.argtypes = [C.c_void_p, C.c_int, C.c_int, C.c_longlong, C.c_longlong,
                                 C.c_double, C.c_void_p, C.c_longlong, C.c_void_p, C.c_longlong,
                                 C.c_double, C.c_void_p, C.c_longlong]
        L.hssk_sgemm_sketch.argtypes = [C.c_void_p, C.c_int, C.c_int, C.c_longlong, C.c_longlong,
                                        C.c_double, C.c_void_p, C.c_longlong, C.c_void_p, C.c_longlong,
                                        C.c_double, C.c_void_p, C.c_longlong]
        L.hssk_narrow_f32.argtypes = [C.c_void_p, C.c_void_p, C.c_longlong, C.c_void_p, C.c_longlong, C.c_longlong, C.c_longlong]
        for name in ("hssk_gemm_vbatched", "hssk_gather_cols", "hssk_gather_rows",
                     "hssk_gather_elems", "hssk_gather_elems_f32", "hssk_transpose", "hssk_id_vbatched", "hssk_qr_vbatched",
                     "hssk_trsm_vbatched", "hssk_getrf_vbatched", "hssk_getrs_vbatched",
                     "hssk_sumsq_vbatched", "hssk_leaf_update_vbatched", "hssk_formq_vbatched",
                     "hssk_id_xsolve_vbatched", "hssk_gather_combine", "hssk_ulv_split", "hssk_tpqr_vbatched"):
            getattr(L, name).argtypes = [C.c_void_p, C.c_void_p, C.c_int]
        L.hssk_sketch_gen.argtypes = [C.c_void_p, C.c_void_p, C.c_int, C.c_int, C.c_longlong, C.c_longlong, C.c_longlong,
                                      C.c_double, C.c_void_p, C.c_longlong, C.c_double, C.c_void_p, C.c_longlong]
        L.hssk_gen_elems.argtypes = [C.c_void_p, C.c_void_p, C.c_void_p, C.c_int]
        L.hssk_gen_fill.argtypes = [C.c_void_p, C.c_void_p, C.c_void_p, C.c_longlong, C.c_longlong, C.c_longlong, C.c_longlong,
                                    C.c_longlong, C.c_int]
        L.hssk_id_solves_inline.argtypes = [C.c_int, C.c_int]
        L.hssk_shift_diag.argtypes = [C.c_void_p, C.c_void_p, C.c_int, C.c_double]
        L.hssk_kernel_eval_vbatched.argtypes = [C.c_void_p, C.c_void_p, C.c_void_p, C.c_int]
        L.hssk_knn.argtypes = [C.c_void_p, C.c_void_p, C.c_int, C.c_int, C.c_int, C.c_int, C.c_int, C.c_void_p]
        L.hssk_kernel_predict.argtypes = [C.c_void_p, C.c_void_p, C.c_void_p, C.c_void_p, C.c_int, C.c_void_p]
        L.hssk_kernel_predict_f32.argtypes = [C.c_void_p, C.c_void_p, C.c_longlong, C.c_int, C.c_int, C.c_int, C.c_double,
                                              C.c_void_p, C.c_void_p, C.c_int, C.c_void_p, C.c_void_p]
        L.hssk_kernel_predict_splits.argtypes = [C.c_longlong, C.c_int]
        L.hssk_colsets.argtypes = [C.c_void_p, C.c_void_p, C.c_int, C.c_int]
        L.hssk_cluster_median.argtypes = [C.c_void_p, C.c_void_p, C.c_int, C.c_int, C.c_int, C.c_int, C.c_void_p, C.c_void_p]
        for fn in ("hssk_pchol_id_vbatched", "hssk_sum_partials", "hssk_gram_vbatched"):
            getattr(L, fn).argtypes = [C.c_void_p, C.c_void_p, C.c_int]
        L.hssk_pchol_id_rank_cap.argtypes = [C.c_int]
        L.hssk_gram_gen_vbatched.argtypes = [C.c_void_p, C.c_void_p, C.c_void_p, C.c_int]
        L.hssk_gram_gen_supported.argtypes = [C.c_void_p, C.c_int]
        L.hssk_colsets_max_universe.argtypes = []
        L.hssk_colsets_max_universe.restype = C.c_longlong
        L.hssk_sjlt_dense.argtypes = [C.c_void_p, C.c_void_p, C.c_int, C.c_longlong, C.c_longlong, C.c_void_p, C.c_int]
        L.hssk_sjlt_sketch.argtypes = [C.c_void_p, C.c_int, C.c_longlong, C.c_longlong, C.c_void_p, C.c_longlong,
                                       C.c_void_p, C.c_int, C.c_int, C.c_void_p, C.c_longlong]
        L.hssk_mfma_f64_peak_tflops.restype = C.c_double
        L.hssk_mfma_f64_peak_tflops.argtypes = [C.c_void_p, C.c_int]
        L.hssk_mfma_f64_probe.argtypes = [C.c_void_p, C.c_int, C.c_int, C.c_int, C.POINTER(C.c_double)]
        ctx = C.c_void_p()
        if L.hssk_ctx_create(C.byref(ctx), device):
            raise RuntimeError(self.error())
        self.ctx = ctx

    def error(self):
        return self.lib.hssk_last_error().decode()

    def check(self, rc):
        if rc:
            raise RuntimeError(self.error())

    def close(self):
        if self.ctx:
            self.lib.hssk_ctx_destroy(self.ctx)
            self.ctx = None

    def sync(self):
        self.check(self.lib.hssk_sync(self.ctx))

    def empty(self, shape, dtype=np.float64):
        return DevArray(self, shape, dtype)

    def array(self, arr, dtype=None):
        a = np.asarray(arr)
        d = DevArray(self, a.shape, dtype or a.dtype)
        return d.set(a)

    def kernel_predict_f32(self, X, w, T, ktype, h, p=1, stats=False):
        X = np.ascontiguousarray(X, dtype=np.float32)
        T = np.ascontiguousarray(T, dtype=np.float32)
        w = np.ascontiguousarray(w, dtype=np.float32)
        (n, d), m = X.shape, T.shape[0]
        dX, dT, dw, dp = (self.array(X.ravel()), self.array(T.ravel()), self.array(w), self.empty((m,), np.float32))
        st = np.zeros(6, dtype=np.int64)
        self.check(self.lib.hssk_kernel_predict_f32(self.ctx, dX.ptr, n, d, ktype, p, h, dw.ptr, dT.ptr, m, dp.ptr,
                                                    st.ctypes.data if stats else None))
        out = dp.get()
        for a in (dX, dT, dw, dp):
            a.free()
        return (out, st) if stats else out

    def batch(self, fn_name, descs):
        if not descs:
            return
        arr = (type(descs[0]) * len(descs))(*descs)
        self.check(getattr(self.lib, fn_name)(self.ctx, arr, len(descs)))
```

Before: 69510.

## Fold deferred split-K sketch reductions into the leaf update kernel

The two sketch GEMMs (row and column samples) can now leave their split-K partial sums pending in dedicated per-slot buffers instead of reducing them immediately. The leaf update kernel then reads and sums those partials directly and applies the -R*D correction in one pass, avoiding a separate reduce launch and a write/read round trip of the sample matrices. Flushes are added wherever the samples are needed elsewhere (multi-rank exchange, hard restart, later levels, workspace teardown). The change costs extra persistent device memory for the partial buffers and adds coverage checks that fall back to the normal path when the shapes do not match.

```diff
diff --git a/include/hssk.h b/include/hssk.h
--- a/include/hssk.h
+++ b/include/hssk.h
@@ -75,6 +75,10 @@
                const double* A, long long lda, const double* B, long long ldb, double beta,
                double* C, long long ldc);
 
+int hssk_dgemm_defer(hssk_ctx* ctx, int slot);
+int hssk_dgemm_flush(hssk_ctx* ctx);
+int hssk_dgemm_pending(hssk_ctx* ctx, int slot);
+
 int hssk_sgemm_sketch(hssk_ctx* ctx, int transB, int m, long long n, long long k, double alpha,
                       const double* A, long long lda,
                       const float* B, long long ldb,
@@ -111,6 +115,7 @@
   int d, m, ldr, ldd, lds;
 } hssk_leaf_update_desc;
 int hssk_leaf_update_vbatched(hssk_ctx* ctx, const hssk_leaf_update_desc* descs, int count);
+int hssk_leaf_update_pending(hssk_ctx* ctx, const hssk_leaf_update_desc* descs, int count);
 
 typedef struct hssk_kernel_spec {
   const double* X;
diff --git a/include/structured/StructuredMatrix.h b/include/structured/StructuredMatrix.h
--- a/include/structured/StructuredMatrix.h
+++ b/include/structured/StructuredMatrix.h
@@ -153,6 +153,7 @@
 void* SPX_d_struct_hssk_ctx(const CSPStructMat S);
 long long SPX_tree_pass_launches(void);
 long long SPX_tree_pass_fallbacks(void);
+long long SPX_sketch_folds(void);
 long long SPX_device_pool_cached_bytes(void);
 long long SPX_device_pool_limit_bytes(void);
 void SPX_device_pool_trim(void);
diff --git a/strumpack_amd/capi.py b/strumpack_amd/capi.py
--- a/strumpack_amd/capi.py
+++ b/strumpack_amd/capi.py
@@ -35,7 +35,7 @@
     "SPX_d_blr_front_factor", "SPX_d_blr_front_factor_device", "SPX_d_blr_front_time_phases", "SPX_blr_low_rank_algorithm", "SPX_d_blr_front_forward",
     "SPX_d_blr_front_backward", "SPX_d_blr_front_schur", "SPX_d_blr_front_schur_device", "SPX_d_blr_front_tile_ranks",
     "SPX_d_blr_front_stats", "SPX_d_blr_front_destroy",
-    "SPX_tree_pass_launches", "SPX_tree_pass_fallbacks",
+    "SPX_tree_pass_launches", "SPX_tree_pass_fallbacks", "SPX_sketch_folds",
     "SPX_device_pool_cached_bytes", "SPX_device_pool_limit_bytes", "SPX_device_pool_trim", "SPX_device_pool_set_limit_gb",
     "SPX_s_struct_from_dense_device", "SPX_s_struct_sketch_route", "SPX_s_struct_stats",
 ]
@@ -111,7 +111,7 @@
     L.SPX_d_struct_mult_child.argtypes = [vp, C.c_int, C.c_char, C.c_int, dp, ll, dp, ll, C.c_int]
     L.SPX_d_struct_hssk_ctx.argtypes = [vp]
     L.SPX_d_struct_hssk_ctx.restype = vp
-    for f in ("SPX_tree_pass_launches", "SPX_tree_pass_fallbacks", "SPX_device_pool_cached_bytes", "SPX_device_pool_limit_bytes"):
+    for f in ("SPX_tree_pass_launches", "SPX_tree_pass_fallbacks", "SPX_sketch_folds", "SPX_device_pool_cached_bytes", "SPX_device_pool_limit_bytes"):
         getattr(L, f).argtypes = []
         getattr(L, f).restype = C.c_longlong
     L.SPX_device_pool_trim.argtypes = []
diff --git a/strumpack_amd/csrc/host/StructuredMatrixC.cpp b/strumpack_amd/csrc/host/StructuredMatrixC.cpp
--- a/strumpack_amd/csrc/host/StructuredMatrixC.cpp
+++ b/strumpack_amd/csrc/host/StructuredMatrixC.cpp
@@ -659,6 +659,7 @@
 
 long long SPX_tree_pass_launches(void) { return strumpack::HSS::tree_pass_launches(); }
 long long SPX_tree_pass_fallbacks(void) { return strumpack::HSS::tree_pass_fallbacks(); }
+long long SPX_sketch_folds(void) { return strumpack::HSS::sketch_folds(); }
 
 long long SPX_device_pool_cached_bytes(void) { return (long long)strumpack::DevicePool::get().cached(); }
 long long SPX_device_pool_limit_bytes(void) { return (long long)strumpack::DevicePool::get().limit(); }
diff --git a/strumpack_amd/csrc/host/hss_compress.cpp b/strumpack_amd/csrc/host/hss_compress.cpp
--- a/strumpack_amd/csrc/host/hss_compress.cpp
+++ b/strumpack_amd/csrc/host/hss_compress.cpp
@@ -3,6 +3,9 @@
 
 namespace strumpack {
 namespace HSS {
+
+static std::atomic<long long> g_sketch_folds{0};
+long long sketch_folds() { return g_sketch_folds; }
 
 void DeviceHSS::drop_plans() {
   for (auto& kv : plans_) if (kv.second.plan) hssk_plan_destroy(kv.second.plan);
@@ -15,6 +18,7 @@
 }
 
 void DeviceHSS::reset_compression() {
+  hssk_dgemm_flush(ctx_);
   book_ = PendingBook();
   defer_book_ = false;
   drop_plans();
@@ -54,6 +58,7 @@
 }
 
 void DeviceHSS::free_compress_workspace() {
+  ck(hssk_dgemm_flush(ctx_));
   ck(hssk_sync(ctx_));
   work_->reset();
   Rt_ = Srt_ = Sct_ = Srt0_ = Sct0_ = nullptr;
@@ -211,6 +216,7 @@
           break;
         }
         process_level(src, own_by_height_[h], d, dd, false);
+        if (h == 0) ck(hssk_dgemm_flush(ctx_));
         factor_ahead_level(h);
       }
       if (dist_subtree_) {
@@ -235,6 +241,7 @@
       stats_.f_sketch += src.sketch_flops(*this, d - d_old);
       if (o_.verbose) std::cout << "# compressing with d = " << d - o_.p << " + " << o_.p << (o_.algorithm == 2 ? " (original, hard restart)" : " (original)") << std::endl;
       if (o_.algorithm == 2) {
+        ck(hssk_dgemm_flush(ctx_));
         if (dist_subtree_ || o_.world > 1) throw std::invalid_argument("hard restart is a single-GPU option");
         std::vector<hssk_colgather_desc> cp;
         cp.push_back(hssk_colgather_desc{Srt_ + d_old, Srt0_ + d_old, nullptr, d - d_old, (int)N, dcap_, dcap_, 0});
@@ -242,7 +249,10 @@
         ck(hssk_gather_cols(ctx_, cp.data(), 2));
       }
       stats_.rounds++;
-      for (auto& ids : own_by_height_) process_level(src, ids, d, d - d_old, true);
+      for (size_t h = 0; h < own_by_height_.size(); h++) {
+        process_level(src, own_by_height_[h], d, d - d_old, true);
+        if (h == 0) ck(hssk_dgemm_flush(ctx_));
+      }
       if (dist_subtree_) {
         exchange_cut_compress(d);
         for (auto& ids : top_by_height_) process_level(src, ids, d, d - d_old, true);
@@ -379,6 +389,7 @@
   std::vector<hssk_combine_desc> cb;
   std::vector<hssk_gemm_desc> mm;
   std::vector<hssk_leaf_update_desc> lu;
+  bool leaves_plain = false;
   for (size_t k = 0; k < ids.size(); k++) {
     Node& nd = nodes_[ids[k]];
     const int r0 = r0s[k], dn = dns[k];
@@ -388,6 +399,7 @@
       if (dn <= 192 && dn % 2 == 0 && r0 % 2 == 0 && nd.Rrt == nd.Rct)
         lu.push_back(hssk_leaf_update_desc{nd.Rrt + r0, nd.D, nd.Srt + r0, nd.Sct + r0, dn, m, dcap_, m, dcap_});
       else {
+        leaves_plain = true;
         mm.push_back(hssk_gemm_desc{nd.Rrt + r0, nd.D, nd.Srt + r0, dn, m, m, dcap_, m, dcap_, 0, 1, -1.0, 1.0});
         mm.push_back(hssk_gemm_desc{nd.Rct + r0, nd.D, nd.Sct + r0, dn, m, m, dcap_, m, dcap_, 0, 0, -1.0, 1.0});
       }
@@ -408,7 +420,13 @@
     }
   }
   if (!cb.empty()) ck(hssk_gather_combine(ctx_, cb.data(), (int)cb.size()));
-  if (!lu.empty()) {
+  bool folded = false;
+  if (!lu.empty() && !leaves_plain && hssk_dgemm_pending(ctx_, 0) && hssk_dgemm_pending(ctx_, 1)) {
+    const int rc = hssk_leaf_update_pending(ctx_, lu.data(), (int)lu.size());
+    if (rc != 2) { ck(rc); folded = true; g_sketch_folds++; }
+  }
+  ck(hssk_dgemm_flush(ctx_));
+  if (!lu.empty() && !folded) {
     int rc = hssk_leaf_update_vbatched(ctx_, lu.data(), (int)lu.size());
     if (rc == 2) {
       for (auto& u : lu) {
diff --git a/strumpack_amd/csrc/host/hss_engine.hpp b/strumpack_amd/csrc/host/hss_engine.hpp
--- a/strumpack_amd/csrc/host/hss_engine.hpp
+++ b/strumpack_amd/csrc/host/hss_engine.hpp
@@ -49,6 +49,7 @@
 class DeviceHSS;
 long long tree_pass_launches();
 long long tree_pass_fallbacks();
+long long sketch_folds();
 
 struct PhaseStats {
   double t_compress = 0, t_sketch = 0, t_random = 0, t_tree = 0, t_factor = 0, t_solve = 0, t_mult = 0;
diff --git a/strumpack_amd/csrc/host/hss_engine_internal.hpp b/strumpack_amd/csrc/host/hss_engine_internal.hpp
--- a/strumpack_amd/csrc/host/hss_engine_internal.hpp
+++ b/strumpack_amd/csrc/host/hss_engine_internal.hpp
@@ -38,6 +38,11 @@
 
 inline int fuse_max_nrhs() {
   static const int v = [] { const char* e = std::getenv("STRUMPACK_AMD_FUSE_MAX_NRHS"); return e ? std::atoi(e) : 256; }();
+  return v;
+}
+
+inline bool sketch_fold() {
+  static const bool v = [] { const char* e = std::getenv("STRUMPACK_AMD_SKETCH_FOLD"); return !(e && e[0] == '0'); }();
   return v;
 }
 
diff --git a/strumpack_amd/csrc/host/hss_sources.cpp b/strumpack_amd/csrc/host/hss_sources.cpp
--- a/strumpack_amd/csrc/host/hss_sources.cpp
+++ b/strumpack_amd/csrc/host/hss_sources.cpp
@@ -46,17 +46,21 @@
         }
       }
     } else if (nloc > 0) {
+      const bool fold = sketch_fold() && !H.o_.symmetric && !(H.o_.world > 1 && !H.dist_subtree_);
+      if (fold) ck(hssk_dgemm_defer(H.ctx_, 0));
       ck(hssk_dgemm(H.ctx_, 1, dn, nloc, N, 1.0, H.Rt_ + r0, H.dcap_, dA + j0, lda, 0.0, H.Srt_ + r0 + j0 * H.dcap_, H.dcap_));
       ck(hssk_dgemm_timing_defer(H.ctx_));
       if (H.o_.symmetric) {
         hssk_colgather_desc cp{H.Srt_ + r0 + j0 * H.dcap_, H.Sct_ + r0 + j0 * H.dcap_, nullptr, dn, (int)nloc, H.dcap_, H.dcap_, 0};
         ck(hssk_gather_cols(H.ctx_, &cp, 1));
       } else {
+        if (fold) ck(hssk_dgemm_defer(H.ctx_, 1));
         ck(hssk_dgemm(H.ctx_, 0, dn, nloc, N, 1.0, H.Rt_ + r0, H.dcap_, dA + j0 * lda, lda, 0.0, H.Sct_ + r0 + j0 * H.dcap_, H.dcap_));
         ck(hssk_dgemm_timing_defer(H.ctx_));
       }
     }
     if (H.o_.world > 1 && !H.dist_subtree_) {
+      ck(hssk_dgemm_flush(H.ctx_));
       const long long bytes = (long long)sizeof(double) * H.dcap_ * H.cols_per_rank_;
       H.comm(H.Srt_, bytes);
       H.comm(H.Sct_, bytes);
@@ -153,9 +157,12 @@
     const Node& c = H.nodes_[single ? 0 : H.cut_nodes_[H.o_.rank]];
     const long long j0 = c.lo, nloc = c.m;
     auto timed = [&] { ck(hssk_dgemm_timing_defer(H.ctx_)); };
+    const bool fold = sketch_fold() && dRows;
+    if (fold) ck(hssk_dgemm_defer(H.ctx_, 1));
     ck(hssk_dgemm(H.ctx_, 0, dn, nloc, N, 1.0, H.Rt_ + r0, H.dcap_, dCols, ldc, 0.0, H.Sct_ + r0 + j0 * H.dcap_, H.dcap_));
     timed();
     if (dRows) {
+      if (fold) ck(hssk_dgemm_defer(H.ctx_, 0));
       ck(hssk_dgemm(H.ctx_, 1, dn, nloc, N, 1.0, H.Rt_ + r0, H.dcap_, dRows, ldr, 0.0, H.Srt_ + r0 + j0 * H.dcap_, H.dcap_));
       timed();
     } else {
@@ -437,17 +444,21 @@
     const long long nloc = j1 - j0;
     auto timed = [&] { ck(hssk_dgemm_timing_defer(H.ctx_)); };
     if (nloc > 0) {
+      const bool fold = sketch_fold() && !H.o_.symmetric && !(H.o_.world > 1 && !H.dist_subtree_);
+      if (fold) ck(hssk_dgemm_defer(H.ctx_, 0));
       ck(hssk_sketch_gen(H.ctx_, &g, 1, dn, nloc, N, j0, 1.0, H.Rt_ + r0, H.dcap_, 0.0, H.Srt_ + r0 + j0 * H.dcap_, H.dcap_));
       timed();
       if (H.o_.symmetric) {
         hssk_colgather_desc cp{H.Srt_ + r0 + j0 * H.dcap_, H.Sct_ + r0 + j0 * H.dcap_, nullptr, dn, (int)nloc, H.dcap_, H.dcap_, 0};
         ck(hssk_gather_cols(H.ctx_, &cp, 1));
       } else {
+        if (fold) ck(hssk_dgemm_defer(H.ctx_, 1));
         ck(hssk_sketch_gen(H.ctx_, &g, 0, dn, nloc, N, j0, 1.0, H.Rt_ + r0, H.dcap_, 0.0, H.Sct_ + r0 + j0 * H.dcap_, H.dcap_));
         timed();
       }
     }
     if (H.o_.world > 1 && !H.dist_subtree_) {
+      ck(hssk_dgemm_flush(H.ctx_));
       const long long bytes = (long long)sizeof(double) * H.dcap_ * H.cols_per_rank_;
       H.comm(H.Srt_, bytes);
       H.comm(H.Sct_, bytes);
diff --git a/strumpack_amd/csrc/kernels/hssk_ctx.hip b/strumpack_amd/csrc/kernels/hssk_ctx.hip
--- a/strumpack_amd/csrc/kernels/hssk_ctx.hip
+++ b/strumpack_amd/csrc/kernels/hssk_ctx.hip
@@ -1,4 +1,5 @@
 #include "hssk_internal.h"
+#include "DevicePool.hpp"
 
 #include <cstdlib>
 #include <unistd.h>
@@ -16,6 +17,29 @@
 void hssk_set_error(const std::string& msg) { g_err = msg; }
 
 thread_local std::vector<std::function<void()>>* hssk_rec::sink = nullptr;
+
+double* hssk_ctx::slot_buf(int s, size_t bytes) {
+  if (bytes > slot_bytes[s]) {
+    const size_t need = (bytes + (size_t(64) << 20) - 1) & ~((size_t(64) << 20) - 1);
+    sync_all();
+    if (d_slot[s]) strumpack::DevicePool::get().release(d_slot[s], slot_bytes[s]);
+    d_slot[s] = nullptr;
+    slot_bytes[s] = 0;
+    d_slot[s] = (double*)strumpack::DevicePool::get().acquire(need);
+    if (!d_slot[s]) throw std::runtime_error("hssk: out of device memory for the deferred K-partials (" + std::to_string(need) + " bytes)");
+    slot_bytes[s] = need;
+  }
+  return d_slot[s];
+}
+void hssk_ctx::release_slots() {
+  for (int s = 0; s < 2; s++) {
+    pending[s] = hssk_pending();
+    if (d_slot[s]) strumpack::DevicePool::get().release(d_slot[s], slot_bytes[s]);
+    d_slot[s] = nullptr;
+    slot_bytes[s] = 0;
+  }
+  defer_armed = -1;
+}
 
 struct hssk_uploader {
   static constexpr int SLOTS = 4;
@@ -251,6 +275,7 @@
 void hssk_ctx_destroy(hssk_ctx* c) {
   if (!c) return;
   try { hssk_rt::sync(c->stream); } catch (...) {}
+  c->release_slots();
   {
     std::lock_guard<std::mutex> g(g_pool_mu);
     if (g_pool.size() < 8) {
diff --git a/strumpack_amd/csrc/kernels/hssk_dgemm.hip b/strumpack_amd/csrc/kernels/hssk_dgemm.hip
--- a/strumpack_amd/csrc/kernels/hssk_dgemm.hip
+++ b/strumpack_amd/csrc/kernels/hssk_dgemm.hip
@@ -445,6 +445,8 @@
     __syncthreads();
   }
 }
+
+inline bool reduce_is_wide(int nz, long long total) { return nz >= 32 && total <= 65536; }
 
 template <int BM, bool FULL, int TAG>
 void launch_dgemm(hssk_ctx* ctx, int transB, dim3 grid, int m, long long n, long long k, const double* A,
@@ -520,8 +522,29 @@
 }
 }
 
+static void launch_reduce(hssk_ctx* ctx, int m, long long vcols, const double* P, long long ldp, long long pstride, int nz,
+                          double alpha, double beta, double* C, long long ldc) {
+  const long long total = (long long)m * vcols;
+  const unsigned rb = (unsigned)std::min<long long>((total + 255) / 256, 4096);
+  if (reduce_is_wide(nz, total))
+    HSSK_LAUNCH(dgemm_reduce_wide_kernel, dim3((unsigned)((total + 15) / 16)), dim3(256), 0, ctx->stream, m, vcols, P, ldp, pstride, nz, alpha, beta, C, ldc);
+  else
+    HSSK_LAUNCH(dgemm_reduce_kernel, dim3(rb), dim3(256), 0, ctx->stream, m, vcols, P, ldp, pstride, nz, alpha, beta, C, ldc);
+}
+static void flush_slot(hssk_ctx* ctx, int slot) {
+  hssk_pending& p = ctx->pending[slot];
+  if (!p.live) return;
+  p.live = false;
+  for (int g = 0; g < p.ngroups; g++) {
+    const hssk_pending_group& q = p.g[g];
+    if (q.nz > 0) launch_reduce(ctx, p.m, q.vcols, (const double*)q.P, p.ldp, q.pstride, q.nz, p.alpha, 0., p.C + q.col0 * p.ldc, p.ldc);
+  }
+  hssk_rt::check_launch();
+}
+
 static void dgemm_impl(hssk_ctx* ctx, int transB, int m, long long n, long long k, double alpha, const double* A, long long lda,
-                       const double* B, long long ldb, const hssk_gen* gen, long long jg0, double beta, double* C, long long ldc) {
+                       const double* B, long long ldb, const hssk_gen* gen, long long jg0, double beta, double* C, long long ldc,
+                       int defer_slot = -1) {
   if (m <= 0 || n <= 0) return;
   const int BM = m > 128 ? 192 : (m > 64 ? 128 : 64);
   const unsigned gm = (unsigned)((m + BM - 1) / BM);
@@ -601,7 +624,9 @@
     ptot += (size_t)ldp * g->cols * g->nz;
   }
   const size_t ntrace = gmain.ntiles ? (size_t)gmain.ntiles * gm * gmain.nz : 0;
-  double* P = ctx->scratch(sizeof(double) * (ptot + 4 + 4 * ntrace));
+  const bool defer = defer_slot >= 0 && defer_slot < 2 && beta == 0.;
+  if (defer) flush_slot(ctx, defer_slot);
+  double* P = defer ? ctx->slot_buf(defer_slot, sizeof(double) * (ptot + 4 + 4 * ntrace)) : ctx->scratch(sizeof(double) * (ptot + 4 + 4 * ntrace));
   long long* clk = (long long*)(P + ptot);
   {
     double* q = P;
@@ -639,14 +664,20 @@
   ctx->dgemm_trace_wgs = (long long)ntrace;
   ctx->dgemm_timed = true;
   ctx->dgemm_timed_flops = 2.0 * (double)m * (double)timed->vcols * (double)k;
+  hssk_pending pend;
   for (const Group* g : {&gmain, &gtail, &gedge}) {
     if (!g->ntiles) continue;
-    long long total = (long long)m * g->vcols;
-    unsigned rb = (unsigned)std::min<long long>((total + 255) / 256, 4096);
-    if (g->nz >= 32 && total <= 65536)
-      HSSK_LAUNCH(dgemm_reduce_wide_kernel, dim3((unsigned)((total + 15) / 16)), dim3(256), 0, ctx->stream, m, g->vcols, (const double*)g->P, ldp, ldp * g->cols, g->nz, alpha, beta, C + g->col0 * ldc, ldc);
-    else
-      HSSK_LAUNCH(dgemm_reduce_kernel, dim3(rb), dim3(256), 0, ctx->stream, m, g->vcols, (const double*)g->P, ldp, ldp * g->cols, g->nz, alpha, beta, C + g->col0 * ldc, ldc);
+    const bool now = !defer || reduce_is_wide(g->nz, (long long)m * g->vcols);
+    if (now) launch_reduce(ctx, m, g->vcols, g->P, ldp, ldp * g->cols, g->nz, alpha, beta, C + g->col0 * ldc, ldc);
+    if (defer) {
+      hssk_pending_group& q = pend.g[pend.ngroups++];
+      q.P = g->P; q.pstride = ldp * g->cols; q.col0 = g->col0; q.vcols = g->vcols; q.nz = now ? 0 : g->nz;
+    }
+  }
+  if (defer) {
+    pend.live = true;
+    pend.ldp = ldp; pend.alpha = alpha; pend.C = C; pend.ldc = ldc; pend.n = n; pend.m = m;
+    ctx->pending[defer_slot] = pend;
   }
   hssk_rt::check_launch();
 }
@@ -655,15 +686,34 @@
                           const double* A, long long lda, const double* B, long long ldb, double beta,
                           double* C, long long ldc) {
   HSSK_API_BEGIN
-  dgemm_impl(ctx, transB, m, n, k, alpha, A, lda, B, ldb, nullptr, 0, beta, C, ldc);
+  const int slot = ctx->defer_armed;
+  ctx->defer_armed = -1;
+  dgemm_impl(ctx, transB, m, n, k, alpha, A, lda, B, ldb, nullptr, 0, beta, C, ldc, slot);
   HSSK_API_END
 }
+
+extern "C" int hssk_dgemm_defer(hssk_ctx* ctx, int slot) {
+  HSSK_API_BEGIN
+  if (slot < 0 || slot > 1) throw std::invalid_argument("hssk_dgemm_defer: slot must be 0 (row product) or 1 (column product)");
+  ctx->defer_armed = slot;
+  HSSK_API_END
+}
+extern "C" int hssk_dgemm_flush(hssk_ctx* ctx) {
+  HSSK_API_BEGIN
+  ctx->defer_armed = -1;
+  flush_slot(ctx, 0);
+  flush_slot(ctx, 1);
+  HSSK_API_END
+}
+extern "C" int hssk_dgemm_pending(hssk_ctx* ctx, int slot) { return ctx && slot >= 0 && slot < 2 && ctx->pending[slot].live ? 1 : 0; }
 
 extern "C" int hssk_sketch_gen(hssk_ctx* ctx, const hssk_gen* g, int transG, int m, long long n, long long k, long long j0,
                                double alpha, const double* A, long long lda, double beta, double* C, long long ldc) {
   HSSK_API_BEGIN
   if (!g || (g->kind != HSSK_GEN_TOEPLITZ && g->kind != HSSK_GEN_TOEPLITZ_UPPER)) throw std::invalid_argument("hssk_sketch_gen: unknown generator kind");
   if (k > 0x7fffffffLL || j0 + n > 0x7fffffffLL) throw std::invalid_argument("hssk_sketch_gen: indices beyond 2^31");
-  dgemm_impl(ctx, transG, m, n, k, alpha, A, lda, nullptr, 0, g, j0, beta, C, ldc);
+  const int slot = ctx->defer_armed;
+  ctx->defer_armed = -1;
+  dgemm_impl(ctx, transG, m, n, k, alpha, A, lda, nullptr, 0, g, j0, beta, C, ldc, slot);
   HSSK_API_END
 }
diff --git a/strumpack_amd/csrc/kernels/hssk_gemm_vbatched.hip b/strumpack_amd/csrc/kernels/hssk_gemm_vbatched.hip
--- a/strumpack_amd/csrc/kernels/hssk_gemm_vbatched.hip
+++ b/strumpack_amd/csrc/kernels/hssk_gemm_vbatched.hip
@@ -243,8 +243,66 @@
       }
 }
 
+struct FoldGroup {
+  const double* P;
+  long long pstride;
+  long long col0;
+  int nz;
+};
+struct FoldProd {
+  FoldGroup g[3];
+  const double* C;
+  long long ldc, ldp;
+  double alpha;
+};
+struct FoldArgs { FoldProd q[2]; };
+
+__device__ __forceinline__ void fold_half(const FoldProd& f, const double* Cq, int lds, long long jt, int j0, int b, int d, int m,
+                                          int wm, int l15, int l4, int ga, int gb, double (&s)[3][4], unsigned& direct) {
+  direct = 0;
+#pragma unroll
+  for (int a = 0; a < 3; a++)
+#pragma unroll
+    for (int r = 0; r < 4; r++) s[a][r] = 0.;
+  const long long J0 = jt + j0, J1 = jt + min(j0 + PBN, m) - 1;
+  for (int g = ga; g <= gb; g++) {
+    const FoldGroup grp = f.g[g];
+    const bool dir = grp.nz == 0;
+    const long long c0 = max(J0, grp.col0), c1 = g < 2 ? min(J1, f.g[g + 1].col0 - 1) : J1;
+    if (c0 > c1) continue;
+    const double* base = dir ? Cq : grp.P;
+    const long long ld = dir ? (long long)lds : f.ldp, cs = dir ? jt : 0;
+    unsigned off[3][4], mine = 0;
+#pragma unroll
+    for (int r = 0; r < 4; r++) {
+      const long long J = jt + j0 + b * 16 + l4 + 4 * r;
+      if (J >= c0 && J <= c1) mine |= 1u << r;
+      const long long Jc = min(max(J, c0), c1);
+#pragma unroll
+      for (int a = 0; a < 3; a++) off[a][r] = (unsigned)((Jc - cs) * ld + min(wm + a * 16 + l15, d - 1));
+    }
+    if (dir) direct |= mine;
+    const int nz = dir ? 1 : grp.nz;
+#pragma unroll 2
+    for (int z = 0; z < nz; z++) {
+      double v[3][4];
+#pragma unroll
+      for (int a = 0; a < 3; a++)
+#pragma unroll
+        for (int r = 0; r < 4; r++) v[a][r] = hssk_gload(base, off[a][r]);
+#pragma unroll
+      for (int a = 0; a < 3; a++)
+#pragma unroll
+        for (int r = 0; r < 4; r++)
+          if ((mine >> r) & 1u) s[a][r] = dir ? v[a][r] : s[a][r] + v[a][r];
+      base += grp.pstride;
+    }
+  }
+}
+
+template <bool FOLD>
 __global__ __launch_bounds__(256, 2) void leaf_update_kernel(const hssk_leaf_update_desc* __restrict__ descs,
-                                                             const Tile* __restrict__ tiles) {
+                                                             const Tile* __restrict__ tiles, const FoldArgs fold) {
   HSSK_SHARED double As[2 * PBK * PLDA];
   HSSK_SHARED double Bs[2 * 2 * PBK * PLDB];
   const Tile t = tiles[blockIdx.x];
@@ -347,6 +405,31 @@
 #pragma unroll
   for (int q = 0; q < 2; q++) {
     double* C = q == 0 ? p.Sr : p.Sc;
+    if (FOLD) {
+      const FoldProd& f = fold.q[q];
+      const long long jt = (long long)(C - f.C) / f.ldc;
+      const long long J0 = jt + j0, J1 = jt + min(j0 + PBN, m) - 1;
+      const int ga = J0 >= f.g[2].col0 ? 2 : (J0 >= f.g[1].col0 ? 1 : 0), gb = J1 >= f.g[2].col0 ? 2 : (J1 >= f.g[1].col0 ? 1 : 0);
+#pragma unroll
+      for (int b = 0; b < 2; b++) {
+        double s[3][4];
+        unsigned direct;
+        fold_half(f, C, p.lds, jt, j0, b, d, m, wm, l15, l4, ga, gb, s, direct);
+#pragma unroll
+        for (int a = 0; a < 3; a++)
+#pragma unroll
+          for (int r = 0; r < 4; r++) {
+#if defined(__clang__)
+#pragma clang fp contract(off)
+#endif
+            const int gi = wm + a * 16 + l15;
+            const int gj = j0 + b * 16 + l4 + 4 * r;
+            const double cv = ((direct >> r) & 1u) ? s[a][r] : f.alpha * s[a][r];
+            if (gi < d && gj < m) hssk_gstore(C, gi + (size_t)gj * p.lds, cv - acc[q][a][b][r]);
+          }
+      }
+      continue;
+    }
     double cv[3][2][4];
 #pragma unroll
     for (int a = 0; a < 3; a++)
@@ -637,7 +720,58 @@
   if (tiles.empty()) return 0;
   auto* dd = (const hssk_leaf_update_desc*)ctx->stage(descs, sizeof(*descs) * count);
   auto* dt = (const Tile*)ctx->stage(tiles.data(), sizeof(Tile) * tiles.size());
-  HSSK_LAUNCH(leaf_update_kernel, dim3((unsigned)tiles.size()), dim3(256), 0, ctx->stream, dd, dt);
+  HSSK_LAUNCH(leaf_update_kernel<false>, dim3((unsigned)tiles.size()), dim3(256), 0, ctx->stream, dd, dt, FoldArgs{});
   hssk_rt::check_launch();
   HSSK_API_END
 }
+
+extern "C" int hssk_leaf_update_pending(hssk_ctx* ctx, const hssk_leaf_update_desc* descs, int count) {
+  HSSK_API_BEGIN
+  if (count <= 0) return 0;
+  const hssk_pending* pd[2] = {&ctx->pending[0], &ctx->pending[1]};
+  for (int q = 0; q < 2; q++)
+    if (!pd[q]->live || pd[q]->elem_bytes != 8 || pd[q]->ldc <= 0) HSSK_UNSUPPORTED("the reduce passes of both sketch products must be pending");
+  for (int q = 0; q < 2; q++)
+    if ((unsigned long long)pd[q]->n * (unsigned long long)std::max(pd[q]->ldp, pd[q]->ldc) >= (1ull << 32)) HSSK_UNSUPPORTED("product too large for the folding epilogue");
+  std::vector<Tile> tiles;
+  std::vector<std::pair<long long, long long>> cover[2];
+  for (int p = 0; p < count; p++) {
+    const hssk_leaf_update_desc& d = descs[p];
+    if (d.d <= 0 || d.m <= 0) continue;
+    if (d.d > PBM || (d.d % 2) || (d.ldr % 2) || ((size_t)d.R % 16)) HSSK_UNSUPPORTED("panel shape outside the fused leaf update");
+    for (int q = 0; q < 2; q++) {
+      const double* S = q == 0 ? d.Sr : d.Sc;
+      const long long off = S - pd[q]->C;
+      if (d.d != pd[q]->m || d.lds != pd[q]->ldc || S < pd[q]->C || off % pd[q]->ldc) HSSK_UNSUPPORTED("a sample panel is not a column range of the pending product");
+      cover[q].push_back({off / pd[q]->ldc, (long long)d.m});
+    }
+    for (int tn = 0; tn * PBN < d.m; tn++) tiles.push_back(Tile{p, 0, tn});
+  }
+  for (int q = 0; q < 2; q++) {
+    std::sort(cover[q].begin(), cover[q].end());
+    long long next = 0;
+    for (auto& c : cover[q]) {
+      if (c.first != next) HSSK_UNSUPPORTED("the sample panels do not tile the pending product's columns");
+      next += c.second;
+    }
+    if (next != pd[q]->n) HSSK_UNSUPPORTED("the sample panels do not cover the pending product's columns");
+  }
+  FoldArgs fa;
+  for (int q = 0; q < 2; q++) {
+    FoldProd& f = fa.q[q];
+    for (int g = 0; g < 3; g++) {
+      if (g < pd[q]->ngroups) {
+        const hssk_pending_group& s = pd[q]->g[g];
+        f.g[g] = FoldGroup{(const double*)s.P - s.col0 * pd[q]->ldp, s.pstride, s.col0, s.nz};
+      } else f.g[g] = FoldGroup{nullptr, 0, 0x7fffffffffffffffLL, 0};
+    }
+    if (pd[q]->ngroups == 0 || pd[q]->g[0].col0 != 0) HSSK_UNSUPPORTED("pending product without a first group");
+    f.C = pd[q]->C; f.ldc = pd[q]->ldc; f.ldp = pd[q]->ldp; f.alpha = pd[q]->alpha;
+  }
+  auto* dd = (const hssk_leaf_update_desc*)ctx->stage(descs, sizeof(*descs) * count);
+  auto* dt = (const Tile*)ctx->stage(tiles.data(), sizeof(Tile) * tiles.size());
+  HSSK_LAUNCH(leaf_update_kernel<true>, dim3((unsigned)tiles.size()), dim3(256), 0, ctx->stream, dd, dt, fa);
+  hssk_rt::check_launch();
+  ctx->pending[0].live = ctx->pending[1].live = false;
+  HSSK_API_END
+}
diff --git a/strumpack_amd/csrc/kernels/hssk_internal.h b/strumpack_amd/csrc/kernels/hssk_internal.h
--- a/strumpack_amd/csrc/kernels/hssk_internal.h
+++ b/strumpack_amd/csrc/kernels/hssk_internal.h
@@ -32,6 +32,24 @@
     return p;
   }
   ~hssk_plan() { for (auto& b : blocks) { hssk_rt::dev_free(b.dev); hssk_rt::pinned_free(b.shadow); } }
+};
+
+struct hssk_pending_group {
+  const void* P = nullptr;
+  long long pstride = 0;
+  long long col0 = 0, vcols = 0;
+  int nz = 0;
+};
+struct hssk_pending {
+  bool live = false;
+  int elem_bytes = 8;
+  int ngroups = 0;
+  hssk_pending_group g[3];
+  long long ldp = 0;
+  double alpha = 1.;
+  double* C = nullptr;
+  long long ldc = 0, n = 0;
+  int m = 0;
 };
 
 struct hssk_uploader;
@@ -123,6 +141,12 @@
     }
     return d_gen;
   }
+  int defer_armed = -1;
+  hssk_pending pending[2];
+  double* d_slot[2] = {nullptr, nullptr};
+  size_t slot_bytes[2] = {0, 0};
+  double* slot_buf(int s, size_t bytes);
+  void release_slots();
   double* scratch(size_t bytes) {
     if (bytes > scratch_bytes) {
       sync_all();
diff --git a/strumpack_amd/hssk.py b/strumpack_amd/hssk.py
--- a/strumpack_amd/hssk.py
+++ b/strumpack_amd/hssk.py
@@ -160,6 +160,7 @@
     "hssk_cluster_median", "hssk_pchol_id_vbatched", "hssk_pchol_id_max_m", "hssk_pchol_id_rank_cap", "hssk_sum_partials", "hssk_gram_vbatched", "hssk_gram_gen_vbatched", "hssk_gram_gen_supported",
     "hssk_sgemm_sketch", "hssk_narrow_f32", "hssk_gather_elems_f32",
     "hssk_kernel_predict_f32", "hssk_kernel_predict_splits",
+    "hssk_dgemm_defer", "hssk_dgemm_flush", "hssk_dgemm_pending", "hssk_leaf_update_pending",
 ]
 
 
@@ -256,9 +257,12 @@
         for name in ("hssk_gemm_vbatched", "hssk_gather_cols", "hssk_gather_rows",
                      "hssk_gather_elems", "hssk_gather_elems_f32", "hssk_transpose", "hssk_id_vbatched", "hssk_qr_vbatched",
                      "hssk_trsm_vbatched", "hssk_getrf_vbatched", "hssk_getrs_vbatched",
-                     "hssk_sumsq_vbatched", "hssk_leaf_update_vbatched", "hssk_formq_vbatched",
+                     "hssk_sumsq_vbatched", "hssk_leaf_update_vbatched", "hssk_leaf_update_pending", "hssk_formq_vbatched",
                      "hssk_id_xsolve_vbatched", "hssk_gather_combine", "hssk_ulv_split", "hssk_tpqr_vbatched"):
             getattr(L, name).argtypes = [C.c_void_p, C.c_void_p, C.c_int]
+        L.hssk_dgemm_defer.argtypes = [C.c_void_p, C.c_int]
+        L.hssk_dgemm_flush.argtypes = [C.c_void_p]
+        L.hssk_dgemm_pending.argtypes = [C.c_void_p, C.c_int]
         L.hssk_sketch_gen.argtypes = [C.c_void_p, C.c_void_p, C.c_int, C.c_int, C.c_longlong, C.c_longlong, C.c_longlong,
                                       C.c_double, C.c_void_p, C.c_longlong, C.c_double, C.c_void_p, C.c_longlong]
         L.hssk_gen_elems.argtypes = [C.c_void_p, C.c_void_p, C.c_void_p, C.c_int]
```

Result: no change. 69470 (-0.1%).
